# teaghan/sky_embeddings

Measured on AMD Instinct MI355X. Metric: MAE pretrain images/sec (5x64x64, ViT-B), higher is better.
Workload: dtype f16; 1 GPU; mim_32.ini-as-BASELINE configs[1]: MAE ViT-Base/16, 5x64x64, mask_ratio=0.75, bs=256/GPU, AdamW+cosine, norm_pix mse; global_batch=256, parallelism=dp1, rccl_ranks=1, graph=True, adamw_in_wgrad_epilogue=True

## Files before the change

### include/skyemb.h

```cpp
#ifndef SKYEMB_H
#define SKYEMB_H

#include <stdint.h>

#ifdef __cplusplus
extern "C" {
#endif

#define SKYEMB_BF16 0
#define SKYEMB_F32 1
#define SKYEMB_F16 2

#define SKYEMB_KC 0
#define SKYEMB_RC 1

#define SKYEMB_ACT_NONE 0
#define SKYEMB_ACT_GELU 1
#define SKYEMB_ACT_DGELU 2

const char *skyemb_last_error(void);
int skyemb_version(void);
int skyemb_debug_skip(int mask);
#define SKYEMB_GEMM_COUNT_FALLBACK 0
#define SKYEMB_GEMM_COUNT_PIPE 1
#define SKYEMB_GEMM_COUNT_256 2
#define SKYEMB_GEMM_COUNT_GROUP 3
#define SKYEMB_GEMM_COUNT_GROUP256 4
#define SKYEMB_GEMM_COUNT_SPLITK 5
#define SKYEMB_GEMM_COUNT_SLOTS 8
int skyemb_gemm_launch_counts(long long *out, int n, int reset);

typedef struct skyemb_gemm_args {
    const void *A;
    const void *B;
    int64_t lda, ldb;
    int32_t a_layout, b_layout;
    int32_t M, N, K;
    int32_t dtype;
    float alpha;
    const float *bias;
    const float *table;
    const int32_t *tab_row;
    int64_t ldt;
    const int32_t *dst_row;
    const float *resid;
    int64_t ldr;
    const void *aux;
    int64_t ldaux;
    int32_t act;
    float *out_f32;
    int64_t ldo32;
    void *out;
    int64_t ldo;
    void *out2;
    int64_t ldo2;
    int32_t tile;
    float *colsum_a;
    void *ws;
    int64_t ws_bytes;
    int32_t split_k;
    int32_t prefetch_wgs;
    const void *prefetch;
    int64_t prefetch_bytes;
} skyemb_gemm_args;

int skyemb_gemm(const skyemb_gemm_args *args, void *stream);

typedef struct skyemb_gemm_group_info {
    int32_t total_blocks;
    int32_t tile;
    int32_t class_mask;
    int32_t reserved;
} skyemb_gemm_group_info;
int64_t skyemb_gemm_group_blob_bytes(int n);
int skyemb_gemm_group_plan(const skyemb_gemm_args *args, int n, int tile, void *blob_host, int64_t blob_bytes,
                           skyemb_gemm_group_info *info);
int skyemb_gemm_group_launch(const void *blob_dev, const skyemb_gemm_group_info *info, void *stream);
typedef struct skyemb_adamw_desc {
    float *g_base, *p, *m, *v;
    void *p_lp;
    const float *hyper;
    int64_t n_decay;
    float beta1, beta2, eps, weight_decay, grad_scale;
    int32_t enabled;
} skyemb_adamw_desc;
int skyemb_gemm_group_plan_adamw(const skyemb_gemm_args *args, int n, int tile, const skyemb_adamw_desc *adamw, void *blob_host,
                                 int64_t blob_bytes, skyemb_gemm_group_info *info);
int skyemb_gemm_group_plan_side_adamw(const skyemb_gemm_args *args, int n, int tile, const skyemb_adamw_desc *adamw, int own_step,
                                      int64_t side_lo, int64_t side_hi, int side_blocks, void *blob_host, int64_t blob_bytes,
                                      skyemb_gemm_group_info *info);
typedef struct skyemb_ln_bwd_side {
    const void *dy;
    const float *x, *gamma, *mean, *rstd;
    const float *g_in;
    float *g_out;
    void *g_lp;
    float *part;
    int32_t M, D;
} skyemb_ln_bwd_side;
int skyemb_gemm_group_attach_ln_bwd(void *blob_host, int64_t blob_bytes, skyemb_gemm_group_info *info, const skyemb_ln_bwd_side *ln);

int skyemb_colsum(const void *X, int dtype, int64_t ldx, int M, int N, float *out, void *stream);

int skyemb_random_mask_from_noise(const float *noise, int B, int L, int keep, int64_t *ids_restore, float *mask,
                                  int32_t *ids_keep, int32_t *dec_dst, int32_t *dec_tab, int n_extra, void *stream);
int skyemb_simmim_mask_from_noise(const float *noise, const float *ratio_u, double max_ratio, int B, int C, int L, int grid, int p,
                                  float *out_mask, void *stream);

int skyemb_patch_gather(const float *imgs, const float *pmv, const int32_t *ids_keep, void *out, int dtype, int B,
                        int C, int H, int W, int p, int keep, float pixel_mean, float pixel_std, void *stream);

int skyemb_patch_gather_blend(const float *imgs, const float *pmv, const int32_t *ids_keep, const float *pixel_mask, void *out,
                              int dtype, int B, int C, int H, int W, int p, int keep, float pixel_mean, float pixel_std,
                              void *stream);
int skyemb_patch_gather_bwd_pmv_blend(const float *imgs, const int32_t *ids_keep, const float *pixel_mask, const float *drows,
                                      float *partial, float *dpmv, int B, int C, int H, int W, int p, int keep, void *stream);

int skyemb_radec_token_fwd(const float *ra_dec, const float *W0, const float *b0, const float *W1, const float *b1,
                           const float *pos_row, float *x, int64_t row_stride, int B, int D, float *sh, float *z, void *stream);
int skyemb_radec_token_bwd(const float *g, int64_t row_stride, const float *W1, const float *sh, const float *z, float *dz_ws,
                           float *dW0, float *db0, float *dW1, float *db1, int B, int D, void *stream);

int skyemb_patch_gather_bwd_pmv(const float *imgs, const int32_t *ids_keep, const float *drows, float *partial,
                                float *dpmv, int B, int C, int H, int W, int p, int keep, void *stream);

int skyemb_layernorm_fwd(const float *x, const float *gamma, const float *beta, void *y, float *y32, int dtype,
                         float *mean, float *rstd, int M, int D, float eps, void *stream);

int skyemb_layernorm_bwd_blocks(int M);
typedef struct {
    const float *part;
    float *dgamma, *dbeta;
    int32_t nblk, D;
} skyemb_ln_reduce_item;
int skyemb_layernorm_bwd_reduce_batch(const skyemb_ln_reduce_item *items, const int32_t *blocks, int n_blocks, void *stream);
int skyemb_layernorm_bwd(const void *dy, int dy_is_f32, int dtype, const float *x, const float *gamma,
                         const float *mean, const float *rstd, const float *g_in, float *g_out, void *g_lp,
                         float *part, float *dgamma, float *dbeta, int M, int D, void *stream);

#define SKYEMB_MHA_MAX_N 4098
int skyemb_mha_fwd(const void *qkv, void *out, int dtype, int B, int N, int H, int hd, void *stream);
int skyemb_mha_bwd(const void *qkv, const void *dout, void *dqkv, int dtype, int B, int N, int H, int hd,
                   void *stream);

int skyemb_fill_mask_tokens(float *x, const float *mask, const float *mask_token, const float *dec_pos, int B,
                            int L, int Dd, int n_extra, void *stream);
int skyemb_gather_rows(const float *src, const int32_t *idx, float *out, void *out_lp, int dtype, int n_rows,
                       int D, void *stream);
int skyemb_rowsum_select(const float *src, int64_t ld, const float *sel, int row0, int inner, int outer_stride,
                         int n_rows, int D, float *partial, float *out, void *stream);

int skyemb_masked_patch_loss(const float *imgs, const float *pred, const float *mask, float *loss, void *dpred,
                             float *dpred32, int dtype, float *ws, int B, int C, int H, int W, int p, int extra,
                             float pixel_mean, float pixel_std, int norm_pix, int loss_l1, float dscale, void *stream);

int skyemb_simmim_pixel_loss(const float *imgs, const float *pred_tok, const float *pixel_mask, float *loss, void *dpred_tok,
                             int dtype, float *pred_img, float *ws, int B, int C, int H, int W, int p, int extra,
                             float pixel_mean, float pixel_std, int norm_pix, int loss_l1, int pooled, float dscale, void *stream);

int skyemb_set_scalars(float *dst, float a, float b, float c, float d, void *stream);
int skyemb_adamw(float *p, void *g, float *m, float *v, void *p_lp, int dtype, int64_t n, int64_t n_decay,
                 const float *hyper, float lr, float bc1, float bc2, float beta1, float beta2, float eps, float wd,
                 float grad_scale, int zero_grad, int grad_dtype, void *stream);
int skyemb_cast(const float *src, void *dst, int dtype, int64_t n, void *stream);

int skyemb_gather_rows_host(const void *src, int64_t row_bytes, const int64_t *idx, int64_t n, int64_t src_rows, void *dst,
                            int nthreads);
int skyemb_h5_unchunk_host(const void *file_base, int64_t file_bytes, const int64_t *chunk_addr, const int64_t *chunk_off,
                           int64_t nchunks, int rank, const int64_t *chunk_dims, const int64_t *dset_dims, int elem_size, void *dst,
                           int nthreads);
int skyemb_fits_decode_tiles_host(int codec, const void *base, int64_t base_bytes, const int64_t *off, const int64_t *len,
                                  const int64_t *npix, const int64_t *dst_off, int64_t ntiles, int bytepix, int blocksize, void *dst,
                                  int64_t dst_pixels, int nthreads);
int skyemb_fits_dequantise_tiles_host(const int32_t *q, const int64_t *q_off, const int64_t *y0, const int64_t *x0, const int64_t *h,
                                      const int64_t *w, const int64_t *table_row, int64_t ntiles, const double *zscale, const double *zzero,
                                      const int32_t *blank, const uint8_t *has_blank, const float *rand, int method, int zdither0,
                                      float *out, int64_t H, int64_t W, int big_endian_out, int nthreads);
int skyemb_tile_cutouts(const void *tile, const int *big_endian, int C, int H, int W, const int *h0, const int *w0, int n, int S,
                        float lo, float hi, int use_lo, int use_hi, float *out, void *stream);
int skyemb_clip_crop(const float *src, float *dst, int64_t n_planes, int Hs, int Ws, int size, float lo, float hi,
                     int use_lo, int use_hi, void *stream);

int skyemb_augment(const float *imgs, float *out, const float *params, const int32_t *nan_mask, const float *noise, int B, int C,
                   int S, int A, void *stream);

int skyemb_standardise(const float *x, const float *mu, const float *sigma, float *out, int64_t N, int D,
                       void *stream);
int skyemb_weighted_norms(const float *x, const float *w, float *norms, float *xw_out, int64_t N, int D,
                          void *stream);
int skyemb_cosine_topk_chunks(int64_t N, int Q, int D, int k);
int skyemb_cosine_topk(const float *tw, const float *qn, const float *bank, const float *xn, int Q, int64_t N,
                       int D, int k, float eps, int64_t idx_offset, int nchunks, const float *thr0, float *part_s,
                       int64_t *part_i, void *stream);
int skyemb_kth_largest_floor(const float *x, int Q, int S, int k, float *out, void *stream);
int skyemb_cosine_sample_floor(const float *tw, const float *qn, const float *sample, const float *sample_norms, int Q, int64_t S,
                               int D, int k, float eps, float *ws, float *floor_out, void *stream);
int skyemb_cosine_sample_floor_applicable(int Q, int64_t S, int D, int k);
int skyemb_topk_merge(const float *in_s, const int64_t *in_i, int Q, int nlists, int k, float *out_s,
                      int64_t *out_i, void *ws, void *stream);

int skyemb_topk_prefilter_applicable(int Q, int64_t N, int D, int k);
int64_t skyemb_topk_prefilter_ws_bytes(int Q, int D, int k);
int64_t skyemb_bank16_bytes(int64_t N, int D);
int64_t skyemb_bank16_rowp_rows(int64_t N);
int skyemb_bank16_prepare(const float *bank, const float *xn, int64_t N, int D, void *bank16, float *rowp, void *stream);
int skyemb_cosine_topk_prefiltered(const float *tw, const float *qn, int Q, const float *bank, const float *xn, const void *bank16,
                                   const float *rowp, int64_t N, int D, int k, float eps, int64_t idx_offset, const float *thr0,
                                   void *ws, int64_t ws_bytes, float *out_s, int64_t *out_i, int *redo, void *stream);
int skyemb_attnpool_q(const float *latent, const float *Wq, const float *bq, float *q, int D, void *stream);
int skyemb_attnpool_fwd(const float *q, const void *kv, int dtype, void *out, float *prob, int B, int N, int H, int hd, void *stream);
int skyemb_attnpool_bwd(const float *q, const void *kv, int dtype, const void *dout, const float *prob, void *dkv, float *dq_part,
                        int B, int N, int H, int hd, void *stream);
int skyemb_attnpool_fwd_long(const float *q, const void *kv, int dtype, void *out, float *prob, int B, int N, int H, int hd,
                             void *stream);
int skyemb_attnpool_bwd_long(const float *q, const void *kv, int dtype, const void *dout, const float *prob, void *dkv,
                             float *dq_part, int B, int N, int H, int hd, void *stream);
int skyemb_attnpool_q_bwd(const float *dq_part, int B, const float *latent, const float *Wq, float *dWq, float *dbq, float *dlatent,
                          float *ws, int D, void *stream);
int skyemb_cosine_scores(const float *tw, const float *qn, const float *bank, const float *xn, int Q, int64_t N,
                         int D, float eps, float *scores, void *stream);
#define SKYEMB_COMBINE_MIN 0
#define SKYEMB_COMBINE_MEAN 1
#define SKYEMB_COMBINE_MAX 2
int skyemb_cosine_token_applicable(int Q, int P, int D, int k);
int skyemb_cosine_token_topk_chunks(int64_t N, int P, int Q, int D, int k);
int skyemb_cosine_token_scores(const float *tw, const float *qn, const float *bank, const float *xn, int Q, int64_t N, int P, int D,
                               int combine, float eps, float *scores, void *stream);
int skyemb_cosine_token_topk(const float *tw, const float *qn, const float *bank, const float *xn, int Q, int64_t N, int P, int D,
                             int k, int combine, float eps, int64_t idx_offset, int nlists, const float *thr0, float *part_s,
                             int64_t *part_i, void *stream);

#ifdef __cplusplus
}
#endif
#endif
```

### sky_embeddings_amd/_lib.py

```python
from __future__ import annotations

import ctypes
import os
import subprocess

import torch

_HERE = os.path.dirname(os.path.abspath(__file__))
SO_PATH = os.environ.get("SKYEMB_LIB") or os.path.join(_HERE, "libskyemb.so")
CSRC = os.path.join(_HERE, "csrc")

BF16, F32, F16 = 0, 1, 2
ABI_VERSION = 111
KC, RC = 0, 1
ACT_NONE, ACT_GELU, ACT_DGELU = 0, 1, 2
COMBINE_MIN, COMBINE_MEAN, COMBINE_MAX = 0, 1, 2


class SkyembLibraryError(RuntimeError):
    pass


class SkyembError(RuntimeError):
    pass


c_i32, c_i64, c_f32, c_vp = ctypes.c_int32, ctypes.c_int64, ctypes.c_float, ctypes.c_void_p


class GemmArgs(ctypes.Structure):
    _fields_ = [
        ("A", c_vp), ("B", c_vp), ("lda", c_i64), ("ldb", c_i64), ("a_layout", c_i32), ("b_layout", c_i32),
        ("M", c_i32), ("N", c_i32), ("K", c_i32), ("dtype", c_i32), ("alpha", c_f32),
        ("bias", c_vp), ("table", c_vp), ("tab_row", c_vp), ("ldt", c_i64), ("dst_row", c_vp),
        ("resid", c_vp), ("ldr", c_i64), ("aux", c_vp), ("ldaux", c_i64), ("act", c_i32),
        ("out_f32", c_vp), ("ldo32", c_i64), ("out", c_vp), ("ldo", c_i64), ("out2", c_vp), ("ldo2", c_i64),
        ("tile", c_i32), ("colsum_a", c_vp), ("ws", c_vp), ("ws_bytes", c_i64), ("split_k", c_i32), ("prefetch_wgs", c_i32),
        ("prefetch", c_vp), ("prefetch_bytes", c_i64),
    ]


class AdamwDesc(ctypes.Structure):
    _fields_ = [("g_base", c_vp), ("p", c_vp), ("m", c_vp), ("v", c_vp), ("p_lp", c_vp), ("hyper", c_vp), ("n_decay", c_i64),
                ("beta1", c_f32), ("beta2", c_f32), ("eps", c_f32), ("weight_decay", c_f32), ("grad_scale", c_f32), ("enabled", c_i32)]


class LnBwdSide(ctypes.Structure):
    _fields_ = [("dy", c_vp), ("x", c_vp), ("gamma", c_vp), ("mean", c_vp), ("rstd", c_vp), ("g_in", c_vp), ("g_out", c_vp), ("g_lp", c_vp),
                ("part", c_vp), ("M", c_i32), ("D", c_i32)]


class GemmGroupInfo(ctypes.Structure):
    _fields_ = [("total_blocks", c_i32), ("tile", c_i32), ("class_mask", c_i32), ("reserved", c_i32)]


PROTOTYPES = {
    "skyemb_last_error": (ctypes.c_char_p, []),
    "skyemb_version": (c_i32, []),
    "skyemb_debug_skip": (c_i32, [c_i32]),
    "skyemb_gemm_launch_counts": (c_i32, [c_vp, c_i32, c_i32]),
    "skyemb_gemm": (c_i32, [ctypes.POINTER(GemmArgs), c_vp]),
    "skyemb_gemm_group_blob_bytes": (c_i64, [c_i32]),
    "skyemb_gemm_group_plan": (c_i32, [ctypes.POINTER(GemmArgs), c_i32, c_i32, c_vp, c_i64, ctypes.POINTER(GemmGroupInfo)]),
    "skyemb_set_scalars": (c_i32, [c_vp, c_f32, c_f32, c_f32, c_f32, c_vp]),
    "skyemb_gemm_group_plan_adamw": (c_i32, [ctypes.POINTER(GemmArgs), c_i32, c_i32, ctypes.POINTER(AdamwDesc), c_vp, c_i64,
                                             ctypes.POINTER(GemmGroupInfo)]),
    "skyemb_gemm_group_plan_side_adamw": (c_i32, [ctypes.POINTER(GemmArgs), c_i32, c_i32, ctypes.POINTER(AdamwDesc), c_i32, c_i64, c_i64, c_i32,
                                                  c_vp, c_i64, ctypes.POINTER(GemmGroupInfo)]),
    "skyemb_gemm_group_attach_ln_bwd": (c_i32, [c_vp, c_i64, ctypes.POINTER(GemmGroupInfo), ctypes.POINTER(LnBwdSide)]),
    "skyemb_gemm_group_launch": (c_i32, [c_vp, ctypes.POINTER(GemmGroupInfo), c_vp]),
    "skyemb_colsum": (c_i32, [c_vp, c_i32, c_i64, c_i32, c_i32, c_vp, c_vp]),
    "skyemb_random_mask_from_noise": (c_i32, [c_vp, c_i32, c_i32, c_i32, c_vp, c_vp, c_vp, c_vp, c_vp, c_i32, c_vp]),
    "skyemb_simmim_mask_from_noise": (c_i32, [c_vp, c_vp, ctypes.c_double, c_i32, c_i32, c_i32, c_i32, c_i32, c_vp, c_vp]),
    "skyemb_patch_gather": (c_i32, [c_vp, c_vp, c_vp, c_vp, c_i32, c_i32, c_i32, c_i32, c_i32, c_i32, c_i32, c_f32,
                                    c_f32, c_vp]),
    "skyemb_patch_gather_bwd_pmv": (c_i32, [c_vp, c_vp, c_vp, c_vp, c_vp, c_i32, c_i32, c_i32, c_i32, c_i32, c_i32,
                                            c_vp]),
    "skyemb_layernorm_fwd": (c_i32, [c_vp, c_vp, c_vp, c_vp, c_vp, c_i32, c_vp, c_vp, c_i32, c_i32, c_f32, c_vp]),
    "skyemb_patch_gather_blend": (c_i32, [c_vp, c_vp, c_vp, c_vp, c_vp, c_i32, c_i32, c_i32, c_i32, c_i32, c_i32, c_i32, c_f32, c_f32, c_vp]),
    "skyemb_patch_gather_bwd_pmv_blend": (c_i32, [c_vp, c_vp, c_vp, c_vp, c_vp, c_vp, c_i32, c_i32, c_i32, c_i32, c_i32, c_i32, c_vp]),
    "skyemb_radec_token_fwd": (c_i32, [c_vp, c_vp, c_vp, c_vp, c_vp, c_vp, c_vp, c_i64, c_i32, c_i32, c_vp, c_vp, c_vp]),
    "skyemb_radec_token_bwd": (c_i32, [c_vp, c_i64, c_vp, c_vp, c_vp, c_vp, c_vp, c_vp, c_vp, c_vp, c_i32, c_i32, c_vp]),
    "skyemb_simmim_pixel_loss": (c_i32, [c_vp, c_vp, c_vp, c_vp, c_vp, c_i32, c_vp, c_vp, c_i32, c_i32, c_i32, c_i32, c_i32, c_i32,
                                         c_f32, c_f32, c_i32, c_i32, c_i32, c_f32, c_vp]),
    "skyemb_gather_rows_host": (c_i32, [c_vp, c_i64, c_vp, c_i64, c_i64, c_vp, c_i32]),
    "skyemb_h5_unchunk_host": (c_i32, [c_vp, c_i64, c_vp, c_vp, c_i64, c_i32, c_vp, c_vp, c_i32, c_vp, c_i32]),
    "skyemb_fits_decode_tiles_host": (c_i32, [c_i32, c_vp, c_i64, c_vp, c_vp, c_vp, c_vp, c_i64, c_i32, c_i32, c_vp, c_i64, c_i32]),
    "skyemb_fits_dequantise_tiles_host": (c_i32, [c_vp, c_vp, c_vp, c_vp, c_vp, c_vp, c_vp, c_i64, c_vp, c_vp, c_vp, c_vp, c_vp, c_i32, c_i32,
                                                  c_vp, c_i64, c_i64, c_i32, c_i32]),
    "skyemb_augment": (c_i32, [c_vp, c_vp, c_vp, c_vp, c_vp, c_i32, c_i32, c_i32, c_i32, c_vp]),
    "skyemb_attnpool_q": (c_i32, [c_vp, c_vp, c_vp, c_vp, c_i32, c_vp]),
    "skyemb_attnpool_fwd": (c_i32, [c_vp, c_vp, c_i32, c_vp, c_vp, c_i32, c_i32, c_i32, c_i32, c_vp]),
    "skyemb_attnpool_bwd": (c_i32, [c_vp, c_vp, c_i32, c_vp, c_vp, c_vp, c_vp, c_i32, c_i32, c_i32, c_i32, c_vp]),
    "skyemb_attnpool_fwd_long": (c_i32, [c_vp, c_vp, c_i32, c_vp, c_vp, c_i32, c_i32, c_i32, c_i32, c_vp]),
    "skyemb_attnpool_bwd_long": (c_i32, [c_vp, c_vp, c_i32, c_vp, c_vp, c_vp, c_vp, c_i32, c_i32, c_i32, c_i32, c_vp]),
    "skyemb_attnpool_q_bwd": (c_i32, [c_vp, c_i32, c_vp, c_vp, c_vp, c_vp, c_vp, c_vp, c_i32, c_vp]),
    "skyemb_tile_cutouts": (c_i32, [c_vp, c_vp, c_i32, c_i32, c_i32, c_vp, c_vp, c_i32, c_i32, c_f32, c_f32, c_i32, c_i32, c_vp, c_vp]),
    "skyemb_clip_crop": (c_i32, [c_vp, c_vp, c_i64, c_i32, c_i32, c_i32, c_f32, c_f32, c_i32, c_i32, c_vp]),
    "skyemb_layernorm_bwd_blocks": (c_i32, [c_i32]),
    "skyemb_layernorm_bwd_reduce_batch": (c_i32, [c_vp, c_vp, c_i32, c_vp]),
    "skyemb_layernorm_bwd": (c_i32, [c_vp, c_i32, c_i32, c_vp, c_vp, c_vp, c_vp, c_vp, c_vp, c_vp, c_vp, c_vp, c_vp,
                                     c_i32, c_i32, c_vp]),
    "skyemb_mha_fwd": (c_i32, [c_vp, c_vp, c_i32, c_i32, c_i32, c_i32, c_i32, c_vp]),
    "skyemb_mha_bwd": (c_i32, [c_vp, c_vp, c_vp, c_i32, c_i32, c_i32, c_i32, c_i32, c_vp]),
    "skyemb_fill_mask_tokens": (c_i32, [c_vp, c_vp, c_vp, c_vp, c_i32, c_i32, c_i32, c_i32, c_vp]),
    "skyemb_gather_rows": (c_i32, [c_vp, c_vp, c_vp, c_vp, c_i32, c_i32, c_i32, c_vp]),
    "skyemb_rowsum_select": (c_i32, [c_vp, c_i64, c_vp, c_i32, c_i32, c_i32, c_i32, c_i32, c_vp, c_vp, c_vp]),
    "skyemb_masked_patch_loss": (c_i32, [c_vp, c_vp, c_vp, c_vp, c_vp, c_vp, c_i32, c_vp, c_i32, c_i32, c_i32, c_i32,
                                         c_i32, c_i32, c_f32, c_f32, c_i32, c_i32, c_f32, c_vp]),
    "skyemb_adamw": (c_i32, [c_vp, c_vp, c_vp, c_vp, c_vp, c_i32, c_i64, c_i64, c_vp, c_f32, c_f32, c_f32, c_f32,
                             c_f32, c_f32, c_f32, c_f32, c_i32, c_i32, c_vp]),
    "skyemb_cast": (c_i32, [c_vp, c_vp, c_i32, c_i64, c_vp]),
    "skyemb_standardise": (c_i32, [c_vp, c_vp, c_vp, c_vp, c_i64, c_i32, c_vp]),
    "skyemb_weighted_norms": (c_i32, [c_vp, c_vp, c_vp, c_vp, c_i64, c_i32, c_vp]),
    "skyemb_cosine_topk_chunks": (c_i32, [c_i64, c_i32, c_i32, c_i32]),
    "skyemb_cosine_topk": (c_i32, [c_vp, c_vp, c_vp, c_vp, c_i32, c_i64, c_i32, c_i32, c_f32, c_i64, c_i32, c_vp, c_vp,
                                   c_vp, c_vp]),
    "skyemb_kth_largest_floor": (c_i32, [c_vp, c_i32, c_i32, c_i32, c_vp, c_vp]),
    "skyemb_cosine_sample_floor": (c_i32, [c_vp, c_vp, c_vp, c_vp, c_i32, c_i64, c_i32, c_i32, c_f32, c_vp, c_vp, c_vp]),
    "skyemb_cosine_sample_floor_applicable": (c_i32, [c_i32, c_i64, c_i32, c_i32]),
    "skyemb_topk_merge": (c_i32, [c_vp, c_vp, c_i32, c_i32, c_i32, c_vp, c_vp, c_vp, c_vp]),
    "skyemb_topk_prefilter_applicable": (c_i32, [c_i32, c_i64, c_i32, c_i32]),
    "skyemb_topk_prefilter_ws_bytes": (c_i64, [c_i32, c_i32, c_i32]),
    "skyemb_bank16_bytes": (c_i64, [c_i64, c_i32]),
    "skyemb_bank16_rowp_rows": (c_i64, [c_i64]),
    "skyemb_bank16_prepare": (c_i32, [c_vp, c_vp, c_i64, c_i32, c_vp, c_vp, c_vp]),
    "skyemb_cosine_topk_prefiltered": (c_i32, [c_vp, c_vp, c_i32, c_vp, c_vp, c_vp, c_vp, c_i64, c_i32, c_i32, c_f32, c_i64, c_vp,
                                               c_vp, c_i64, c_vp, c_vp, c_vp, c_vp]),
    "skyemb_cosine_scores": (c_i32, [c_vp, c_vp, c_vp, c_vp, c_i32, c_i64, c_i32, c_f32, c_vp, c_vp]),
    "skyemb_cosine_token_applicable": (c_i32, [c_i32, c_i32, c_i32, c_i32]),
    "skyemb_cosine_token_topk_chunks": (c_i32, [c_i64, c_i32, c_i32, c_i32, c_i32]),
    "skyemb_cosine_token_scores": (c_i32, [c_vp, c_vp, c_vp, c_vp, c_i32, c_i64, c_i32, c_i32, c_i32, c_f32, c_vp, c_vp]),
    "skyemb_cosine_token_topk": (c_i32, [c_vp, c_vp, c_vp, c_vp, c_i32, c_i64, c_i32, c_i32, c_i32, c_i32, c_f32, c_i64, c_i32, c_vp,
                                         c_vp, c_vp, c_vp]),
}

_LIB = None


def build(force: bool = False) -> str:
    if force:
        subprocess.check_call(["make", "-C", CSRC, "-s", "clean"])
    subprocess.check_call(["make", "-C", CSRC, "-s", "-j8"])
    return SO_PATH


def lib():
    global _LIB
    if _LIB is None:
        if not os.path.exists(SO_PATH):
            raise SkyembLibraryError(
                f"{SO_PATH} is missing: the HIP hot-path library has not been built "
                "(run `python -c 'import __graft_entry__ as g; g.build()'` or `make -C sky_embeddings_amd/csrc`). "
                "There is no CPU fallback.")
        try:
            L = ctypes.CDLL(SO_PATH)
        except OSError as e:
            raise SkyembLibraryError(f"cannot load {SO_PATH}: {e}") from e
        for name, (res, args) in PROTOTYPES.items():
            try:
                fn = getattr(L, name)
            except AttributeError as e:
                raise SkyembLibraryError(f"{SO_PATH} does not export {name}") from e
            fn.restype, fn.argtypes = res, args
        if L.skyemb_version() != ABI_VERSION:
            raise SkyembLibraryError(f"{SO_PATH} reports ABI version {L.skyemb_version()}, this binding is written against "
                                     f"{ABI_VERSION}: rebuild the library (make -C sky_embeddings_amd/csrc)")
        _LIB = L
    return _LIB


def check(rc: int, what: str = ""):
    if rc != 0:
        msg = lib().skyemb_last_error()
        raise SkyembError(f"{what} failed (rc={rc}): {msg.decode() if msg else ''}")
```

### sky_embeddings_amd/csrc/adamw.hip

```cpp
#include "common.h"
#include "adamw_math.h"

namespace {

template <typename T, bool LP, typename GT>
__global__ __launch_bounds__(256) void adamw_kernel(float *__restrict__ p, GT *__restrict__ g, float *__restrict__ m,
                                                    float *__restrict__ v, T *__restrict__ p_lp, int64_t n4,
                                                    int64_t n_decay, const float *__restrict__ hyper, float lr_arg,
                                                    float bc1_arg, float bc2_arg, float beta1, float beta2, float eps,
                                                    float wd, float grad_scale, int zero_grad) {
    const float lr = hyper ? hyper[0] : lr_arg, bc1 = hyper ? hyper[1] : bc1_arg, bc2 = hyper ? hyper[2] : bc2_arg;
    const SkyAdamScalars sc = sky_adam_scalars(lr, bc1, bc2, beta1, beta2, eps, wd, grad_scale);
    const int64_t stride = (int64_t)gridDim.x * 256;
    for (int64_t i0 = (int64_t)blockIdx.x * 256 + threadIdx.x; i0 < n4; i0 += 2 * stride) {
        f32x4 pv[2], gv[2], mv[2], vv[2];
#pragma unroll
        for (int u = 0; u < 2; ++u) {
            const int64_t i = i0 + u * stride;
            if (i < n4) {
                pv[u] = *(const f32x4 *)(p + 4 * i);
                const float4 gl = load4<GT>(g + 4 * i);
                gv[u] = (f32x4){gl.x, gl.y, gl.z, gl.w};
                mv[u] = *(const f32x4 *)(m + 4 * i);
                vv[u] = *(const f32x4 *)(v + 4 * i);
            }
        }
#pragma unroll
        for (int u = 0; u < 2; ++u) {
            const int64_t i = i0 + u * stride;
            if (i >= n4) break;
#pragma unroll
            for (int j = 0; j < 4; ++j) {
                float pj = pv[u][j], mj = mv[u][j], vj = vv[u][j];
                sky_adamw_update(gv[u][j], pj, mj, vj, 4 * i + j < n_decay, sc);
                pv[u][j] = pj; mv[u][j] = mj; vv[u][j] = vj;
            }
            *(f32x4 *)(p + 4 * i) = pv[u];
            *(f32x4 *)(m + 4 * i) = mv[u];
            *(f32x4 *)(v + 4 * i) = vv[u];
            if (LP) store4<T>(p_lp + 4 * i, pv[u][0], pv[u][1], pv[u][2], pv[u][3]);
            if (zero_grad) store4<GT>(g + 4 * i, 0.f, 0.f, 0.f, 0.f);
        }
    }
}

__global__ void set_scalars_kernel(float *dst, float a, float b, float c, float d) {
    if (threadIdx.x == 0) { dst[0] = a; dst[1] = b; dst[2] = c; dst[3] = d; }
}

}

extern "C" int skyemb_set_scalars(float *dst, float a, float b, float c, float d, void *stream) {
    SKY_CHECK_ARG(dst != nullptr, "skyemb_set_scalars: null destination");
    hipLaunchKernelGGL(set_scalars_kernel, dim3(1), dim3(64), 0, (hipStream_t)stream, dst, a, b, c, d);
    SKY_LAUNCH_CHECK("skyemb_set_scalars");
    return 0;
}

extern "C" int skyemb_adamw(float *p, void *g, float *m, float *v, void *p_lp, int dtype, int64_t n, int64_t n_decay,
                            const float *hyper, float lr, float bc1, float bc2, float beta1, float beta2, float eps,
                            float wd, float grad_scale, int zero_grad, int grad_dtype, void *stream) {
    SKY_CHECK_ARG(n > 0 && n % 4 == 0 && n_decay >= 0 && n_decay <= n, "skyemb_adamw: n must be a positive multiple of 4");
    SKY_CHECK_ARG(aligned16(p) && aligned16(m) && aligned16(v) && (((uintptr_t)g) & 7) == 0, "skyemb_adamw: unaligned buffers");
    SKY_CHECK_ARG(grad_dtype == SKYEMB_F32 || sky_is_lp(grad_dtype), "skyemb_adamw: bad grad_dtype %d", grad_dtype);
    SKY_CHECK_ARG(!sky_is_lp(grad_dtype) || !p_lp || grad_dtype == dtype || dtype == SKYEMB_F32,
                  "skyemb_adamw: a 16-bit gradient buffer and a 16-bit shadow must share their format");
    int64_t blocks = ceil_div64(n / 4, 256);
    if (blocks > 256 * 16) blocks = 256 * 16;
    hipStream_t st = (hipStream_t)stream;
    dim3 grid((unsigned)blocks), block(256);
#define ADAMW_LAUNCH(T, LP, GT, lp_ptr)                                                                                        \
    hipLaunchKernelGGL((adamw_kernel<T, LP, GT>), grid, block, 0, st, p, (GT *)g, m, v, lp_ptr, n / 4, n_decay, hyper, lr, bc1, \
                       bc2, beta1, beta2, eps, wd, grad_scale, zero_grad)
    const bool g16 = grad_dtype == SKYEMB_BF16, gh = grad_dtype == SKYEMB_F16;
    if (!p_lp) {
        if (g16) ADAMW_LAUNCH(float, false, bf16_t, (float *)nullptr);
        else if (gh) ADAMW_LAUNCH(float, false, f16_t, (float *)nullptr);
        else ADAMW_LAUNCH(float, false, float, (float *)nullptr);
    } else if (dtype == SKYEMB_BF16) {
        if (g16) ADAMW_LAUNCH(bf16_t, true, bf16_t, (bf16_t *)p_lp);
        else ADAMW_LAUNCH(bf16_t, true, float, (bf16_t *)p_lp);
    } else if (dtype == SKYEMB_F16) {
        if (gh) ADAMW_LAUNCH(f16_t, true, f16_t, (f16_t *)p_lp);
        else ADAMW_LAUNCH(f16_t, true, float, (f16_t *)p_lp);
    } else {
        if (g16) ADAMW_LAUNCH(float, true, bf16_t, (float *)p_lp);
        else if (gh) ADAMW_LAUNCH(float, true, f16_t, (float *)p_lp);
        else ADAMW_LAUNCH(float, true, float, (float *)p_lp);
    }
#undef ADAMW_LAUNCH
    SKY_LAUNCH_CHECK("skyemb_adamw");
    return 0;
}
```

### sky_embeddings_amd/csrc/frontend.hip

```cpp
#include "common.h"
#include <type_traits>

namespace {

__global__ __launch_bounds__(256) void mask_kernel(const float *__restrict__ noise, int B, int L, int keep,
                                                   int64_t *__restrict__ ids_restore, float *__restrict__ mask,
                                                   int32_t *__restrict__ ids_keep, int32_t *__restrict__ dec_dst,
                                                   int32_t *__restrict__ dec_tab, int E) {
    extern __shared__ float sn[];
    const int lane = threadIdx.x & 63, wave = threadIdx.x >> 6;
    const int b = blockIdx.x * 4 + wave;
    if (b >= B) return;
    float *row = sn + wave * L;
    for (int i = lane; i < L; i += 64) row[i] = noise[(int64_t)b * L + i];
    __builtin_amdgcn_wave_barrier();
    for (int i = lane; i < L; i += 64) {
        const float v = row[i];
        int rank = 0;
        for (int j = 0; j < L; ++j) {
            const float u = row[j];
            rank += (u < v || (u == v && j < i)) ? 1 : 0;
        }
        ids_restore[(int64_t)b * L + i] = rank;
        mask[(int64_t)b * L + i] = rank >= keep ? 1.0f : 0.0f;
        if (rank < keep) {
            ids_keep[(int64_t)b * keep + rank] = i;
            if (dec_dst) {
                dec_dst[(int64_t)b * (keep + E) + E + rank] = b * (L + E) + E + i;
                dec_tab[(int64_t)b * (keep + E) + E + rank] = E + i;
            }
        }
    }
    if (dec_dst && lane < E) {
        dec_dst[(int64_t)b * (keep + E) + lane] = b * (L + E) + lane;
        dec_tab[(int64_t)b * (keep + E) + lane] = lane;
    }
}


__global__ __launch_bounds__(256) void simmim_mask_kernel(const float *__restrict__ noise, const float *__restrict__ ratio_u,
                                                          double max_ratio, int BC, int C, int L, int grid, int p,
                                                          float *__restrict__ out) {
    extern __shared__ float sn[];
    const int lane = threadIdx.x & 63, wave = threadIdx.x >> 6;
    const int bc = blockIdx.x * 4 + wave;
    if (bc >= BC) return;
    float *row = sn + wave * 2 * L, *mk = row + L;
    for (int i = lane; i < L; i += 64) row[i] = noise[(int64_t)bc * L + i];
    __builtin_amdgcn_wave_barrier();
    const int b = bc / C;
    const int count = (int)ceilf((float)((double)L * ((double)ratio_u[b] * max_ratio)));
    for (int i = lane; i < L; i += 64) {
        const float v = row[i];
        int rank = 0;
        for (int j = 0; j < L; ++j) {
            const float u = row[j];
            rank += (u < v || (u == v && j < i)) ? 1 : 0;
        }
        mk[i] = rank < count ? 1.0f : 0.0f;
    }
    __builtin_amdgcn_wave_barrier();
    const int H = grid * p;
    float *o = out + (int64_t)bc * H * H;
    for (int e = lane * 4; e < H * H; e += 256) {
        const int y = e / H, x = e - y * H;
        const float m = mk[(y / p) * grid + x / p];
        *(float4 *)(o + e) = make_float4(m, m, m, m);
    }
}

template <typename T>
__global__ __launch_bounds__(256) void patch_gather_kernel(const float *__restrict__ imgs, const float *__restrict__ pmv,
                                                           const int32_t *__restrict__ ids_keep, T *__restrict__ out,
                                                           int C, int H, int W, int p, int keep, float mean, float stdv,
                                                           const float *__restrict__ pmask) {
    const int row = blockIdx.x;
    const int b = row / keep;
    const int l = ids_keep ? ids_keep[row] : (row - b * keep);
    const int gw = W / p;
    const int y0 = (l / gw) * p, x0 = (l % gw) * p;
    const int pv4 = C * p * p / 4, p4 = p / 4;
    for (int e = threadIdx.x; e < pv4; e += 256) {
        const int px4 = e % p4, py = (e / p4) % p, c = e / (p4 * p);
        const float4 x = *(const float4 *)(imgs + (((int64_t)b * C + c) * H + y0 + py) * W + x0 + 4 * px4);
        const float4 m = *(const float4 *)(pmv + (c * p + py) * p + 4 * px4);
        float4 o;
        o.x = x.x != x.x ? m.x : (x.x - mean) / stdv;
        o.y = x.y != x.y ? m.y : (x.y - mean) / stdv;
        o.z = x.z != x.z ? m.z : (x.z - mean) / stdv;
        o.w = x.w != x.w ? m.w : (x.w - mean) / stdv;
        if (pmask) {
            const float4 k = *(const float4 *)(pmask + (((int64_t)b * C + c) * H + y0 + py) * W + x0 + 4 * px4);
            o.x = o.x * (1.0f - k.x) + m.x * k.x;
            o.y = o.y * (1.0f - k.y) + m.y * k.y;
            o.z = o.z * (1.0f - k.z) + m.z * k.z;
            o.w = o.w * (1.0f - k.w) + m.w * k.w;
        }
        if constexpr (std::is_same<T, f16_t>::value) {
            o.x = fminf(fmaxf(o.x, -65504.f), 65504.f);
            o.y = fminf(fmaxf(o.y, -65504.f), 65504.f);
            o.z = fminf(fmaxf(o.z, -65504.f), 65504.f);
            o.w = fminf(fmaxf(o.w, -65504.f), 65504.f);
        }
        store4<T>(out + (int64_t)row * (C * p * p) + 4 * e, o.x, o.y, o.z, o.w);
    }
}

__global__ __launch_bounds__(256) void pmv_partial_kernel(const float *__restrict__ imgs, const int32_t *__restrict__ ids_keep,
                                                          const float *__restrict__ drows, float *__restrict__ partial,
                                                          int C, int H, int W, int p, int keep, const float *__restrict__ pmask) {
    const int b = blockIdx.x;
    const int gw = W / p, pv = C * p * p;
    const int e = blockIdx.y * 256 + threadIdx.x;
    if (e >= pv) return;
    const int px = e % p, py = (e / p) % p, c = e / (p * p);
    float acc = 0.f;
    for (int j0 = 0; j0 < keep; j0 += 4) {
        float wgt[4], d[4];
#pragma unroll
        for (int u = 0; u < 4; ++u) {
            const int j = j0 + u < keep ? j0 + u : keep - 1;
            const int l = ids_keep ? ids_keep[b * keep + j] : j;
            const int y = (l / gw) * p + py, x = (l % gw) * p + px;
            const int64_t pix = (((int64_t)b * C + c) * H + y) * W + x;
            const float v = imgs[pix];
            wgt[u] = j0 + u >= keep ? 0.0f : v != v ? 1.0f : (pmask ? pmask[pix] : 0.0f);
            d[u] = drows[((int64_t)b * keep + j) * pv + e];
        }
#pragma unroll
        for (int u = 0; u < 4; ++u)
            if (wgt[u] != 0.0f) acc += wgt[u] * d[u];
    }
    partial[(int64_t)b * pv + e] = acc;
}

template <typename T>
__global__ __launch_bounds__(256) void colsum_kernel(const T *__restrict__ X, int64_t ldx, int M, int N,
                                                     float *__restrict__ out) {
    __shared__ float red[4][64];
    const int lane = threadIdx.x & 63, wave = threadIdx.x >> 6;
    const int n = blockIdx.x * 64 + lane;
    float acc = 0.f;
    if (n < N) {
#pragma unroll 8
        for (int m = wave; m < M; m += 4) acc += to_f32<T>(X[(int64_t)m * ldx + n]);
    }
    red[wave][lane] = acc;
    __syncthreads();
    if (wave == 0 && n < N) out[n] = (red[0][lane] + red[1][lane]) + (red[2][lane] + red[3][lane]);
}

__global__ __launch_bounds__(256) void fill_mask_tokens_kernel(float *__restrict__ x, const float *__restrict__ mask,
                                                               const float *__restrict__ mask_token,
                                                               const float *__restrict__ dec_pos, int L, int Dd, int E) {
    const int b = blockIdx.x / L, l = blockIdx.x % L;
    if (mask[(int64_t)b * L + l] == 0.0f) return;
    float *dst = x + ((int64_t)b * (L + E) + E + l) * Dd;
    const float *pos = dec_pos + (int64_t)(E + l) * Dd;
    for (int d = threadIdx.x * 4; d < Dd; d += 1024) {
        const float4 t = *(const float4 *)(mask_token + d), q = *(const float4 *)(pos + d);
        *(float4 *)(dst + d) = make_float4(t.x + q.x, t.y + q.y, t.z + q.z, t.w + q.w);
    }
}

template <typename T>
__global__ __launch_bounds__(256) void gather_rows_kernel(const float *__restrict__ src, const int32_t *__restrict__ idx,
                                                          float *__restrict__ out, T *__restrict__ out_lp, int D) {
    const int r = blockIdx.x;
    const float *s = src + (int64_t)idx[r] * D;
    for (int d = threadIdx.x * 4; d < D; d += 1024) {
        const float4 v = *(const float4 *)(s + d);
        if (out) *(float4 *)(out + (int64_t)r * D + d) = v;
        if (out_lp) store4<T>(out_lp + (int64_t)r * D + d, v.x, v.y, v.z, v.w);
    }
}

__global__ __launch_bounds__(256) void rowsum_select_kernel(const float *__restrict__ src, int64_t ld,
                                                            const float *__restrict__ sel, int row0, int inner,
                                                            int outer_stride, int n_rows, int D,
                                                            float *__restrict__ partial) {
    const int nblk = gridDim.x;
    for (int d = threadIdx.x; d < D; d += 256) {
        float acc = 0.f;
        for (int i0 = blockIdx.x; i0 < n_rows; i0 += 4 * nblk) {
            float x[4];
#pragma unroll
            for (int u = 0; u < 4; ++u) {
                const int i = i0 + u * nblk;
                const bool take = i < n_rows && !(sel && sel[i] == 0.0f);
                const int ii = take ? i : 0;
                const int64_t r = (int64_t)row0 + (int64_t)(ii / inner) * outer_stride + (ii % inner);
                x[u] = take ? src[r * ld + d] : 0.f;
            }
#pragma unroll
            for (int u = 0; u < 4; ++u)
                if (i0 + u * nblk < n_rows && !(sel && sel[i0 + u * nblk] == 0.0f)) acc += x[u];
        }
        partial[(int64_t)blockIdx.x * D + d] = acc;
    }
}

template <typename T>
__global__ __launch_bounds__(256) void cast_kernel(const float *__restrict__ src, T *__restrict__ dst, int64_t n4) {
    for (int64_t i = (int64_t)blockIdx.x * 256 + threadIdx.x; i < n4; i += (int64_t)gridDim.x * 256) {
        const float4 v = *(const float4 *)(src + 4 * i);
        store4<T>(dst + 4 * i, v.x, v.y, v.z, v.w);
    }
}

__global__ __launch_bounds__(256) void clip_crop_kernel(const float *__restrict__ src, float *__restrict__ dst, int64_t n_out,
                                                        int Hs, int Ws, int size, int top, int left, float lo, float hi,
                                                        int use_lo, int use_hi) {
    for (int64_t i = (int64_t)blockIdx.x * 256 + threadIdx.x; i < n_out; i += (int64_t)gridDim.x * 256) {
        const int x = (int)(i % size);
        const int64_t t = i / size;
        const int y = (int)(t % size);
        const int64_t plane = t / size;
        float v = src[(plane * Hs + top + y) * Ws + left + x];
        if (use_lo && v < lo) v = lo;
        if (use_hi && v > hi) v = hi;
        dst[i] = v;
    }
}

__global__ __launch_bounds__(256) void tile_cutouts_kernel(const unsigned int *__restrict__ tile, const int *__restrict__ be, int C,
                                                           int H, int W, const int *__restrict__ h0, const int *__restrict__ w0,
                                                           int64_t n_out, int S, float lo, float hi, int use_lo, int use_hi,
                                                           float *__restrict__ out) {
    for (int64_t i = (int64_t)blockIdx.x * 256 + threadIdx.x; i < n_out; i += (int64_t)gridDim.x * 256) {
        const int x = (int)(i % S);
        int64_t t = i / S;
        const int y = (int)(t % S);
        t /= S;
        const int c = (int)(t % C);
        const int64_t k = t / C;
        unsigned int u = tile[((int64_t)c * H + h0[k] + y) * W + w0[k] + x];
        if (be[c]) u = __builtin_bswap32(u);
        float v = __uint_as_float(u);
        if (use_lo && v < lo) v = lo;
        if (use_hi && v > hi) v = hi;
        out[i] = v;
    }
}

}

extern "C" int skyemb_clip_crop(const float *src, float *dst, int64_t n_planes, int Hs, int Ws, int size, float lo, float hi,
                                int use_lo, int use_hi, void *stream) {
    SKY_CHECK_ARG(src && dst && n_planes > 0 && size > 0 && Hs >= size && Ws >= size, "skyemb_clip_crop: bad shape");
    const int64_t n_out = n_planes * size * size;
    int64_t blocks = ceil_div64(n_out, 256);
    if (blocks > 8192) blocks = 8192;
    hipLaunchKernelGGL(clip_crop_kernel, dim3((unsigned)blocks), dim3(256), 0, (hipStream_t)stream, src, dst, n_out, Hs, Ws, size,
                       (Hs - size) / 2, (Ws - size) / 2, lo, hi, use_lo, use_hi);
    SKY_LAUNCH_CHECK("skyemb_clip_crop");
    return 0;
}

extern "C" int skyemb_tile_cutouts(const void *tile, const int *big_endian, int C, int H, int W, const int *h0, const int *w0, int n,
                                   int S, float lo, float hi, int use_lo, int use_hi, float *out, void *stream) {
    SKY_CHECK_ARG(tile && big_endian && h0 && w0 && out && C > 0 && n > 0 && S > 0 && H >= S && W >= S,
                  "skyemb_tile_cutouts: bad shape C=%d H=%d W=%d n=%d S=%d", C, H, W, n, S);
    const int64_t n_out = (int64_t)n * C * S * S;
    int64_t blocks = ceil_div64(n_out, 256);
    if (blocks > 16384) blocks = 16384;
    hipLaunchKernelGGL(tile_cutouts_kernel, dim3((unsigned)blocks), dim3(256), 0, (hipStream_t)stream, (const unsigned int *)tile,
                       big_endian, C, H, W, h0, w0, n_out, S, lo, hi, use_lo, use_hi, out);
    SKY_LAUNCH_CHECK("skyemb_tile_cutouts");
    return 0;
}

extern "C" int skyemb_random_mask_from_noise(const float *noise, int B, int L, int keep, int64_t *ids_restore,
                                             float *mask, int32_t *ids_keep, int32_t *dec_dst, int32_t *dec_tab,
                                             int n_extra, void *stream) {
    SKY_CHECK_ARG(B > 0 && L > 0 && keep >= 0 && keep <= L && L <= 4096 && n_extra >= 1 && n_extra <= 2,
                  "skyemb_random_mask_from_noise: bad shape B=%d L=%d keep=%d extra=%d", B, L, keep, n_extra);
    hipLaunchKernelGGL(mask_kernel, dim3((B + 3) / 4), dim3(256), (size_t)4 * L * sizeof(float), (hipStream_t)stream, noise,
                       B, L, keep, ids_restore, mask, ids_keep, dec_dst, dec_tab, n_extra);
    SKY_LAUNCH_CHECK("skyemb_random_mask_from_noise");
    return 0;
}


extern "C" int skyemb_simmim_mask_from_noise(const float *noise, const float *ratio_u, double max_ratio, int B, int C, int L, int grid,
                                             int p, float *out_mask, void *stream) {
    SKY_CHECK_ARG(noise && ratio_u && out_mask && B > 0 && C > 0 && L == grid * grid && L <= 4096 && p > 0 && p % 4 == 0 &&
                  max_ratio >= 0.0 && max_ratio <= 1.0, "skyemb_simmim_mask_from_noise: bad arguments (L=%d grid=%d p=%d)", L, grid, p);
    hipLaunchKernelGGL(simmim_mask_kernel, dim3((B * C + 3) / 4), dim3(256), (size_t)8 * L * sizeof(float), (hipStream_t)stream, noise,
                       ratio_u, max_ratio, B * C, C, L, grid, p, out_mask);
    SKY_LAUNCH_CHECK("skyemb_simmim_mask_from_noise");
    return 0;
}

static int patch_gather_launch(const float *imgs, const float *pmv, const int32_t *ids_keep, const float *pixel_mask, void *out,
                               int dtype, int B, int C, int H, int W, int p, int keep, float pixel_mean, float pixel_std,
                               void *stream) {
    SKY_CHECK_ARG(B > 0 && C > 0 && p > 0 && p % 4 == 0 && H % p == 0 && W % p == 0 && keep > 0,
                  "skyemb_patch_gather: bad geometry C=%d H=%d W=%d p=%d keep=%d", C, H, W, p, keep);
    SKY_CHECK_ARG(ids_keep || keep == (H / p) * (W / p), "skyemb_patch_gather: ids_keep == NULL needs keep == L");
    hipStream_t st = (hipStream_t)stream;
    if (dtype == SKYEMB_BF16)
        hipLaunchKernelGGL(patch_gather_kernel<bf16_t>, dim3(B * keep), dim3(256), 0, st, imgs, pmv, ids_keep, (bf16_t *)out,
                           C, H, W, p, keep, pixel_mean, pixel_std, pixel_mask);
    else if (dtype == SKYEMB_F16)
        hipLaunchKernelGGL(patch_gather_kernel<f16_t>, dim3(B * keep), dim3(256), 0, st, imgs, pmv, ids_keep, (f16_t *)out,
                           C, H, W, p, keep, pixel_mean, pixel_std, pixel_mask);
    else
        hipLaunchKernelGGL(patch_gather_kernel<float>, dim3(B * keep), dim3(256), 0, st, imgs, pmv, ids_keep, (float *)out, C,
                           H, W, p, keep, pixel_mean, pixel_std, pixel_mask);
    SKY_LAUNCH_CHECK("skyemb_patch_gather");
    return 0;
}

extern "C" int skyemb_patch_gather(const float *imgs, const float *pmv, const int32_t *ids_keep, void *out, int dtype,
                                   int B, int C, int H, int W, int p, int keep, float pixel_mean, float pixel_std,
                                   void *stream) {
    return patch_gather_launch(imgs, pmv, ids_keep, nullptr, out, dtype, B, C, H, W, p, keep, pixel_mean, pixel_std, stream);
}

extern "C" int skyemb_patch_gather_blend(const float *imgs, const float *pmv, const int32_t *ids_keep, const float *pixel_mask,
                                         void *out, int dtype, int B, int C, int H, int W, int p, int keep, float pixel_mean,
                                         float pixel_std, void *stream) {
    return patch_gather_launch(imgs, pmv, ids_keep, pixel_mask, out, dtype, B, C, H, W, p, keep, pixel_mean, pixel_std, stream);
}

extern "C" int skyemb_colsum(const void *X, int dtype, int64_t ldx, int M, int N, float *out, void *stream) {
    SKY_CHECK_ARG(M > 0 && N > 0, "skyemb_colsum: bad shape");
    hipStream_t st = (hipStream_t)stream;
    if (dtype == SKYEMB_BF16)
        hipLaunchKernelGGL(colsum_kernel<bf16_t>, dim3((N + 63) / 64), dim3(256), 0, st, (const bf16_t *)X, ldx, M, N, out);
    else if (dtype == SKYEMB_F16)
        hipLaunchKernelGGL(colsum_kernel<f16_t>, dim3((N + 63) / 64), dim3(256), 0, st, (const f16_t *)X, ldx, M, N, out);
    else
        hipLaunchKernelGGL(colsum_kernel<float>, dim3((N + 63) / 64), dim3(256), 0, st, (const float *)X, ldx, M, N, out);
    SKY_LAUNCH_CHECK("skyemb_colsum");
    return 0;
}

extern "C" int skyemb_patch_gather_bwd_pmv_blend(const float *imgs, const int32_t *ids_keep, const float *pixel_mask,
                                                 const float *drows, float *partial, float *dpmv, int B, int C, int H, int W,
                                                 int p, int keep, void *stream) {
    SKY_CHECK_ARG(B > 0 && C > 0 && p > 0 && keep > 0, "skyemb_patch_gather_bwd_pmv: bad geometry");
    hipLaunchKernelGGL(pmv_partial_kernel, dim3(B, (C * p * p + 255) / 256), dim3(256), 0, (hipStream_t)stream, imgs, ids_keep, drows, partial, C, H,
                       W, p, keep, pixel_mask);
    SKY_LAUNCH_CHECK("skyemb_patch_gather_bwd_pmv");
    return skyemb_colsum(partial, SKYEMB_F32, (int64_t)C * p * p, B, C * p * p, dpmv, stream);
}

extern "C" int skyemb_patch_gather_bwd_pmv(const float *imgs, const int32_t *ids_keep, const float *drows, float *partial,
                                           float *dpmv, int B, int C, int H, int W, int p, int keep, void *stream) {
    return skyemb_patch_gather_bwd_pmv_blend(imgs, ids_keep, nullptr, drows, partial, dpmv, B, C, H, W, p, keep, stream);
}

extern "C" int skyemb_fill_mask_tokens(float *x, const float *mask, const float *mask_token, const float *dec_pos, int B,
                                       int L, int Dd, int n_extra, void *stream) {
    SKY_CHECK_ARG(B > 0 && L > 0 && Dd % 4 == 0 && n_extra >= 1, "skyemb_fill_mask_tokens: bad shape");
    hipLaunchKernelGGL(fill_mask_tokens_kernel, dim3(B * L), dim3(256), 0, (hipStream_t)stream, x, mask, mask_token, dec_pos,
                       L, Dd, n_extra);
    SKY_LAUNCH_CHECK("skyemb_fill_mask_tokens");
    return 0;
}

extern "C" int skyemb_gather_rows(const float *src, const int32_t *idx, float *out, void *out_lp, int dtype, int n_rows,
                                  int D, void *stream) {
    SKY_CHECK_ARG(n_rows > 0 && D % 4 == 0, "skyemb_gather_rows: bad shape");
    hipStream_t st = (hipStream_t)stream;
    if (dtype == SKYEMB_BF16)
        hipLaunchKernelGGL(gather_rows_kernel<bf16_t>, dim3(n_rows), dim3(256), 0, st, src, idx, out, (bf16_t *)out_lp, D);
    else if (dtype == SKYEMB_F16)
        hipLaunchKernelGGL(gather_rows_kernel<f16_t>, dim3(n_rows), dim3(256), 0, st, src, idx, out, (f16_t *)out_lp, D);
    else
        hipLaunchKernelGGL(gather_rows_kernel<float>, dim3(n_rows), dim3(256), 0, st, src, idx, out, (float *)out_lp, D);
    SKY_LAUNCH_CHECK("skyemb_gather_rows");
    return 0;
}

extern "C" int skyemb_rowsum_select(const float *src, int64_t ld, const float *sel, int row0, int inner, int outer_stride,
                                    int n_rows, int D, float *partial, float *out, void *stream) {
    SKY_CHECK_ARG(n_rows > 0 && D > 0 && inner > 0, "skyemb_rowsum_select: bad shape");
    const int nblk = 256;
    hipLaunchKernelGGL(rowsum_select_kernel, dim3(nblk), dim3(256), 0, (hipStream_t)stream, src, ld, sel, row0, inner,
                       outer_stride, n_rows, D, partial);
    SKY_LAUNCH_CHECK("skyemb_rowsum_select");
    return skyemb_colsum(partial, SKYEMB_F32, D, nblk, D, out, stream);
}

extern "C" int skyemb_cast(const float *src, void *dst, int dtype, int64_t n, void *stream) {
    SKY_CHECK_ARG(n > 0 && n % 4 == 0, "skyemb_cast: n must be a positive multiple of 4");
    int64_t blocks = ceil_div64(n / 4, 256);
    if (blocks > 4096) blocks = 4096;
    hipStream_t st = (hipStream_t)stream;
    if (dtype == SKYEMB_BF16)
        hipLaunchKernelGGL(cast_kernel<bf16_t>, dim3((unsigned)blocks), dim3(256), 0, st, src, (bf16_t *)dst, n / 4);
    else if (dtype == SKYEMB_F16)
        hipLaunchKernelGGL(cast_kernel<f16_t>, dim3((unsigned)blocks), dim3(256), 0, st, src, (f16_t *)dst, n / 4);
    else
        hipLaunchKernelGGL(cast_kernel<float>, dim3((unsigned)blocks), dim3(256), 0, st, src, (float *)dst, n / 4);
    SKY_LAUNCH_CHECK("skyemb_cast");
    return 0;
}
```

### sky_embeddings_amd/csrc/layernorm.hip

```cpp
#include "common.h"
#include "ln_bwd_body.h"

namespace {

constexpr int MAXV = 8;

template <typename T, int NV>
__global__ __launch_bounds__(256) void ln_fwd_kernel(const float *__restrict__ x, const float *__restrict__ gamma,
                                                     const float *__restrict__ beta, T *__restrict__ y,
                                                     float *__restrict__ y32, float *__restrict__ mean_o,
                                                     float *__restrict__ rstd_o, int M, int D, float eps) {
    const int lane = threadIdx.x & 63;
    const int row = blockIdx.x * 4 + (threadIdx.x >> 6);
    if (row >= M) return;
    const int nv = D >> 2;
    const float *xr = x + (int64_t)row * D;
    float4 v[NV], gm[NV], bt[NV];
#pragma unroll
    for (int i = 0; i < NV; ++i) {
        const int c = lane + i * 64, cc = c < nv ? c : nv - 1;
        v[i] = *(const float4 *)(xr + 4 * cc);
        gm[i] = *(const float4 *)(gamma + 4 * cc);
        bt[i] = *(const float4 *)(beta + 4 * cc);
    }
    float s = 0.f;
#pragma unroll
    for (int i = 0; i < NV; ++i)
        if (lane + i * 64 < nv) s += (v[i].x + v[i].y) + (v[i].z + v[i].w);
    const float mean = wave_sum(s) / (float)D;
    float q = 0.f;
#pragma unroll
    for (int i = 0; i < NV; ++i) {
        if (lane + i * 64 < nv) {
            const float a = v[i].x - mean, b = v[i].y - mean, cc = v[i].z - mean, d = v[i].w - mean;
            q += (a * a + b * b) + (cc * cc + d * d);
        }
    }
    const float rstd = rsqrtf(wave_sum(q) / (float)D + eps);
    if (lane == 0) {
        mean_o[row] = mean;
        rstd_o[row] = rstd;
    }
#pragma unroll
    for (int i = 0; i < NV; ++i) {
        const int c = lane + i * 64;
        if (c < nv) {
            const float4 g = gm[i], b = bt[i];
            const float o0 = (v[i].x - mean) * rstd * g.x + b.x, o1 = (v[i].y - mean) * rstd * g.y + b.y;
            const float o2 = (v[i].z - mean) * rstd * g.z + b.z, o3 = (v[i].w - mean) * rstd * g.w + b.w;
            if (y) store4<T>(y + (int64_t)row * D + 4 * c, o0, o1, o2, o3);
            if (y32) *(float4 *)(y32 + (int64_t)row * D + 4 * c) = make_float4(o0, o1, o2, o3);
        }
    }
}

template <typename TD, typename T, int NV>
__global__ __launch_bounds__(256) void ln_bwd_kernel(const TD *__restrict__ dy, const float *__restrict__ x,
                                                     const float *__restrict__ gamma, const float *__restrict__ mean,
                                                     const float *__restrict__ rstd, const float *g_in, float *g_out,
                                                     T *__restrict__ g_lp, float *__restrict__ part, int M, int D,
                                                     int nblk) {
    __shared__ float red[4 * 256];
    sky_ln_bwd_rows<TD, T, NV>(dy, x, gamma, mean, rstd, g_in, g_out, g_lp, part, M, D, nblk, (int)blockIdx.x, (int)(threadIdx.x >> 6),
                               (int)(threadIdx.x & 63), red);
}

__global__ __launch_bounds__(1024) void ln_bwd_reduce_kernel(const float *__restrict__ part, float *__restrict__ dgamma,
                                                             float *__restrict__ dbeta, int nblk, int D) {
    __shared__ float red[32][33];
    const int col = threadIdx.x & 31, rg = threadIdx.x >> 5;
    const int d = blockIdx.x * 32 + col;
    const float *src = part + (int64_t)blockIdx.y * nblk * D;
    float acc = 0.f;
    if (d < D)
#pragma unroll 8
        for (int b = rg; b < nblk; b += 32) acc += src[(int64_t)b * D + d];
    red[rg][col] = acc;
    __syncthreads();
    if (rg == 0 && d < D) {
        float t = 0.f;
#pragma unroll
        for (int r = 0; r < 32; ++r) t += red[r][col];
        (blockIdx.y == 0 ? dgamma : dbeta)[d] = t;
    }
}

__global__ __launch_bounds__(1024) void ln_bwd_reduce_batch_kernel(const skyemb_ln_reduce_item *__restrict__ items,
                                                                   const int2 *__restrict__ blocks) {
    __shared__ float red[32][33];
    const int2 blk = blocks[blockIdx.x];
    const skyemb_ln_reduce_item it = items[blk.x];
    const int bx = blk.y & 0xffff, by = blk.y >> 16;
    const int col = threadIdx.x & 31, rg = threadIdx.x >> 5;
    const int d = bx * 32 + col;
    const float *src = it.part + (int64_t)by * it.nblk * it.D;
    float acc = 0.f;
    if (d < it.D) {
#pragma unroll 8
        for (int b = rg; b < it.nblk; b += 32) acc += src[(int64_t)b * it.D + d];
    }
    red[rg][col] = acc;
    __syncthreads();
    if (rg == 0 && d < it.D) {
        float t = 0.f;
#pragma unroll
        for (int r = 0; r < 32; ++r) t += red[r][col];
        (by == 0 ? it.dgamma : it.dbeta)[d] = t;
    }
}

}

extern "C" int skyemb_layernorm_bwd_reduce_batch(const skyemb_ln_reduce_item *items, const int32_t *blocks, int n_blocks, void *stream) {
    SKY_CHECK_ARG(items && blocks && n_blocks > 0, "skyemb_layernorm_bwd_reduce_batch: bad arguments");
    hipLaunchKernelGGL(ln_bwd_reduce_batch_kernel, dim3((unsigned)n_blocks), dim3(1024), 0, (hipStream_t)stream, items, (const int2 *)blocks);
    SKY_LAUNCH_CHECK("skyemb_layernorm_bwd_reduce_batch");
    return 0;
}

extern "C" int skyemb_layernorm_fwd(const float *x, const float *gamma, const float *beta, void *y, float *y32,
                                    int dtype, float *mean, float *rstd, int M, int D, float eps, void *stream) {
    SKY_CHECK_ARG(M > 0 && D > 0 && D % 4 == 0 && D <= MAXV * 256, "skyemb_layernorm_fwd: bad shape M=%d D=%d", M, D);
    SKY_CHECK_ARG(aligned16(x) && aligned16(gamma) && aligned16(beta), "skyemb_layernorm_fwd: unaligned input");
    hipStream_t st = (hipStream_t)stream;
    dim3 grid((M + 3) / 4), block(256);
#define LN_FWD(NV)                                                                                                   \
    if (dtype == SKYEMB_BF16)                                                                                        \
        hipLaunchKernelGGL((ln_fwd_kernel<bf16_t, NV>), grid, block, 0, st, x, gamma, beta, (bf16_t *)y, y32, mean,   \
                           rstd, M, D, eps);                                                                         \
    else if (dtype == SKYEMB_F16)                                                                                    \
        hipLaunchKernelGGL((ln_fwd_kernel<f16_t, NV>), grid, block, 0, st, x, gamma, beta, (f16_t *)y, y32, mean,     \
                           rstd, M, D, eps);                                                                         \
    else                                                                                                             \
        hipLaunchKernelGGL((ln_fwd_kernel<float, NV>), grid, block, 0, st, x, gamma, beta, (float *)y, y32, mean,     \
                           rstd, M, D, eps);
    switch ((D + 255) / 256) {
        case 1: LN_FWD(1) break;
        case 2: LN_FWD(2) break;
        case 3: LN_FWD(3) break;
        case 4: LN_FWD(4) break;
        case 5: LN_FWD(5) break;
        case 6: LN_FWD(6) break;
        case 7: LN_FWD(7) break;
        default: LN_FWD(8) break;
    }
#undef LN_FWD
    SKY_LAUNCH_CHECK("skyemb_layernorm_fwd");
    return 0;
}

extern "C" int skyemb_layernorm_bwd_blocks(int M) {
    int nb = (M + 3) / 4;
    if (nb < 1) nb = 1;
    const int rounds = (nb + SKY_LN_BWD_CAP - 1) / SKY_LN_BWD_CAP;
    return (nb + rounds - 1) / rounds;
}

extern "C" int skyemb_layernorm_bwd(const void *dy, int dy_is_f32, int dtype, const float *x, const float *gamma,
                                    const float *mean, const float *rstd, const float *g_in, float *g_out, void *g_lp,
                                    float *part, float *dgamma, float *dbeta, int M, int D, void *stream) {
    SKY_CHECK_ARG(M > 0 && D > 0 && D % 4 == 0 && D <= MAXV * 256, "skyemb_layernorm_bwd: bad shape M=%d D=%d", M, D);
    hipStream_t st = (hipStream_t)stream;
    const int nblk = skyemb_layernorm_bwd_blocks(M);
    dim3 grid(nblk), block(256);
#define LN_BWD(NV)                                                                                                   \
    if (dtype == SKYEMB_BF16) {                                                                                      \
        if (dy_is_f32)                                                                                               \
            hipLaunchKernelGGL((ln_bwd_kernel<float, bf16_t, NV>), grid, block, 0, st, (const float *)dy, x, gamma,   \
                               mean, rstd, g_in, g_out, (bf16_t *)g_lp, part, M, D, nblk);                           \
        else                                                                                                         \
            hipLaunchKernelGGL((ln_bwd_kernel<bf16_t, bf16_t, NV>), grid, block, 0, st, (const bf16_t *)dy, x, gamma, \
                               mean, rstd, g_in, g_out, (bf16_t *)g_lp, part, M, D, nblk);                           \
    } else if (dtype == SKYEMB_F16) {                                                                                \
        if (dy_is_f32)                                                                                               \
            hipLaunchKernelGGL((ln_bwd_kernel<float, f16_t, NV>), grid, block, 0, st, (const float *)dy, x, gamma,    \
                               mean, rstd, g_in, g_out, (f16_t *)g_lp, part, M, D, nblk);                            \
        else                                                                                                         \
            hipLaunchKernelGGL((ln_bwd_kernel<f16_t, f16_t, NV>), grid, block, 0, st, (const f16_t *)dy, x, gamma,    \
                               mean, rstd, g_in, g_out, (f16_t *)g_lp, part, M, D, nblk);                            \
    } else {                                                                                                         \
        hipLaunchKernelGGL((ln_bwd_kernel<float, float, NV>), grid, block, 0, st, (const float *)dy, x, gamma, mean,  \
                           rstd, g_in, g_out, (float *)g_lp, part, M, D, nblk);                                      \
    }
    switch ((D + 255) / 256) {
        case 1: LN_BWD(1) break;
        case 2: LN_BWD(2) break;
        case 3: LN_BWD(3) break;
        case 4: LN_BWD(4) break;
        case 5: LN_BWD(5) break;
        case 6: LN_BWD(6) break;
        case 7: LN_BWD(7) break;
        default: LN_BWD(8) break;
    }
#undef LN_BWD
    if (dgamma && dbeta)
        hipLaunchKernelGGL(ln_bwd_reduce_kernel, dim3((D + 31) / 32, 2), dim3(1024), 0, st, part, dgamma, dbeta, nblk, D);
    SKY_LAUNCH_CHECK("skyemb_layernorm_bwd");
    return 0;
}
```

### sky_embeddings_amd/engine.py

```python
from __future__ import annotations

import math
import os
from collections import OrderedDict
from contextlib import contextmanager

import numpy as np
import torch

from . import ops
from ._lib import ACT_DGELU, ACT_GELU, BF16, F32, KC, RC, AdamwDesc
from .model_config import (FROZEN, SH_FEATURES, SIREN_HIDDEN, MAEConfig, not_optimised, sincos_pos_embed, state_layout,
                           weight_decay_split, xavier_bound)


def _pad8(n):
    return (n + 7) // 8 * 8


def merge_spans(spans):
    out = []
    for lo, hi in sorted(spans):
        if out and out[-1][1] == lo:
            out[-1] = (out[-1][0], hi)
        else:
            out.append((lo, hi))
    return out


def subtract_spans(spans, holes):
    out = []
    for s, e in spans:
        cur = s
        for hs, he in holes:
            if he <= cur or hs >= e:
                continue
            if hs > cur:
                out.append((cur, hs))
            cur = max(cur, he)
        if cur < e:
            out.append((cur, e))
    return out


WGRAD_SLOTS_PER_CU = {256256: 1, 128128: 2, 9128128: 1, 128064: 2, 64064: 3}
SIDE_CARRIER_MAX_FILL = 0.76
ADAMW_SIDE_MODES = ("auto", "0", "1", "dec", "enc")
WGRAD_GROUPS_KEY = {"plain": "wgrad_groups", "adamw": "wgrad_groups_adamw", "g16": "wgrad_groups_g16"}


def plan_wgrad_schedule(prefixes, tiles, ncu, mode):
    assert mode in ADAMW_SIDE_MODES, mode
    carry = [False] * len(prefixes)
    for k in range(1, len(prefixes)):
        tile, count = tiles[k]
        slots = ncu * WGRAD_SLOTS_PER_CU.get(tile, 1)
        carry[k] = (mode == "1" or (mode == "auto" and count <= SIDE_CARRIER_MAX_FILL * slots) or
                    (mode == "dec" and prefixes[k].startswith("decoder_blocks")) or (mode == "enc" and prefixes[k].startswith("blocks")))
    return [(carry[k], k + 1 < len(carry) and carry[k + 1]) for k in range(len(carry))]


class ParamStore:

    def __init__(self, cfg: MAEConfig, device, lp_dtype):
        self.cfg = cfg
        shapes = dict(state_layout(cfg))
        decay, no_decay = weight_decay_split(cfg)
        self.decay, self.no_decay = decay, no_decay
        self.order = decay + no_decay
        self.offsets = {}
        off = 0
        for name in decay:
            self.offsets[name] = off
            off += _pad8(int(np.prod(shapes[name])))
        self.n_decay = off
        for name in no_decay:
            self.offsets[name] = off
            off += _pad8(int(np.prod(shapes[name])))
        self.n = off
        self.shapes = shapes
        self.p = torch.zeros(self.n, device=device, dtype=torch.float32)
        self.g = torch.zeros(self.n, device=device, dtype=torch.float32)
        self.m = torch.zeros(self.n, device=device, dtype=torch.float32)
        self.v = torch.zeros(self.n, device=device, dtype=torch.float32)
        self.p_lp = torch.zeros(self.n, device=device, dtype=lp_dtype)
        self.frozen = {k: torch.zeros(shapes[k], device=device, dtype=torch.float32) for k in not_optimised(cfg) if k in shapes}

    def _view(self, buf, name):
        o = self.offsets[name]
        return buf[o:o + int(np.prod(self.shapes[name]))].view(self.shapes[name])

    def span(self, name):
        o = self.offsets[name]
        return o, o + _pad8(int(np.prod(self.shapes[name])))

    def param(self, name):
        return self.frozen[name] if name in self.frozen else self._view(self.p, name)

    def grad(self, name):
        return self._view(self.g, name)

    def lp(self, name):
        return self._view(self.p_lp, name)

    def refresh_lp(self):
        ops.cast(self.p, self.p_lp, self.n)


def stage_gradient_ranges(store: ParamStore, cfg: MAEConfig, n_encoder_groups: int = 3):
    off = store.offsets
    dec0 = store.span("decoder_embed.weight")[1]
    ranges = [[(dec0, store.n_decay)]]
    bounds = sorted({round(cfg.depth * k / n_encoder_groups) for k in range(n_encoder_groups + 1)}, reverse=True)
    groups = []
    for hi, lo in zip(bounds[:-1], bounds[1:]):
        groups.append((hi, lo))
        end = dec0 if hi == cfg.depth else off[f"blocks.{hi}.attn.qkv.weight"]
        ranges.append([(off[f"blocks.{lo}.attn.qkv.weight"], end)])
    ranges.append([(0, off["blocks.0.attn.qkv.weight"]), (store.n_decay, store.n)])
    return groups, ranges


class MAEEngine:
    _modes = "mae"

    def __init__(self, cfg: MAEConfig, device="cuda", compute_dtype=torch.bfloat16, seed=None):
        if cfg.attn_pool and not cfg.simmim:
            raise ValueError("attn_pool exists in SimMIM mode only (utils/mim_vit.py:244-254, :282)")
        if cfg.simmim and self._modes == "mae":
            raise NotImplementedError("simmim=True is served by sky_embeddings_amd.simmim_engine.SimMIMEngine")
        assert cfg.embed_dim % cfg.num_heads == 0 and cfg.decoder_embed_dim % cfg.decoder_num_heads == 0
        assert cfg.embed_dim % 8 == 0 and cfg.decoder_embed_dim % 8 == 0 and cfg.patch_size % 4 == 0
        self.cfg = cfg
        self.device = torch.device(device)
        self.dtype = compute_dtype
        self.code = ops.dtype_code(compute_dtype)
        env = os.environ.get("SKYEMB_LOSS_SCALE")
        self._loss_scale_auto = compute_dtype == torch.float16 and env is None
        self._loss_scale = float(env) if (env is not None and compute_dtype == torch.float16) else (65536.0 if compute_dtype == torch.float16 else 1.0)
        assert self._loss_scale > 0 and math.log2(self._loss_scale).is_integer(), "loss_scale must be a power of two"
        self.fold_decoder_wgrads = True
        self.store = ParamStore(cfg, self.device, compute_dtype)
        self._ws = {}
        self._last = None
        self.splitk_ws = torch.zeros(8 * 1024 * 1024, device=self.device, dtype=torch.float32)
        self._side, self._pending, self._group_done = None, {}, None
        self._splitk_ws_side = None
        self._ln_first = self._ln_count = 0
        self._pf_maps = None
        self._graph_captures = 0
        self._variant_args = {"adamw": None, "g16": None}
        self._variant = "plain"
        self._adamw_side, self._adamw_side_blocks = "0", 0
        self.initialize_weights(seed)

    def initialize_weights(self, seed=None):
        cfg, st = self.cfg, self.store
        gen = torch.Generator().manual_seed(seed if seed is not None else int(torch.initial_seed() % (2 ** 31)))
        for name in st.order:
            shape = st.shapes[name]
            if name in ("cls_token", "mask_token"):
                t = torch.randn(shape, generator=gen) * 0.02
            elif name == "attn_pool.latent":
                sd_ = shape[-1] ** -0.5
                t = (torch.randn(shape, generator=gen) * sd_).clamp_(-2 * sd_, 2 * sd_)
            elif name == "patch_mask_values":
                t = torch.zeros(shape)
            elif name == "patch_embed.proj.bias" or name.startswith("decoder.0."):
                b = 1.0 / math.sqrt(cfg.patch_dim if name.startswith("patch_embed") else cfg.embed_dim)
                t = (torch.rand(shape, generator=gen) * 2 - 1) * b
            elif name.startswith("ra_dec_embed."):
                first = ".layers.0." in name
                w_std = (1.0 / SH_FEATURES) if first else math.sqrt(6.0 / SIREN_HIDDEN)
                t = (torch.rand(shape, generator=gen) * 2 - 1) * w_std
            elif name.endswith("norm1.weight") or name.endswith("norm2.weight") or name.endswith("norm.weight"):
                t = torch.ones(shape)
            elif name.endswith(".bias"):
                t = torch.zeros(shape)
            else:
                t = (torch.rand(shape, generator=gen) * 2 - 1) * xavier_bound(shape)
            st.param(name).copy_(t)
        for k in st.frozen:
            if k in FROZEN:
                tab = sincos_pos_embed(st.shapes[k][-1], cfg.grid, True, cfg.ra_dec)
                st.frozen[k].copy_(torch.from_numpy(tab).float().unsqueeze(0))
            else:
                st.frozen[k].copy_(torch.randn(st.shapes[k], generator=gen) * 0.02)
        st.refresh_lp()

    @property
    def loss_scale(self):
        return self._loss_scale

    @loss_scale.setter
    def loss_scale(self, v):
        assert v > 0 and math.log2(v).is_integer(), "loss_scale must be a power of two"
        self._loss_scale, self._loss_scale_auto = float(v), False

    def plan_loss_scale(self, masked_elements):
        if self._loss_scale_auto:
            e = round(math.log2(max(float(masked_elements), 64.0) / 64.0))
            self._loss_scale = float(2 ** min(max(e, 0), 16))
        return self._loss_scale

    def expected_masked_elements(self, B, mask_ratio):
        cfg = self.cfg
        return B * (cfg.num_patches - int(cfg.num_patches * (1 - mask_ratio))) * cfg.patch_dim

    def grad(self, name):
        g = self.store.grad(name)
        return g if self.loss_scale == 1.0 else g / self.loss_scale

    def state_dict(self):
        out = OrderedDict()
        for name, _ in state_layout(self.cfg):
            out[name] = self.store.param(name)
        return out

    def load_state_dict(self, sd, strict=True):
        names = [n for n, _ in state_layout(self.cfg)]
        missing = [n for n in names if n not in sd]
        unexpected = [k for k in sd if k not in names]
        if strict and (missing or unexpected):
            raise RuntimeError(f"load_state_dict: missing {missing[:5]} unexpected {unexpected[:5]}")
        for n in names:
            if n in sd:
                self.store.param(n).copy_(torch.as_tensor(sd[n]).to(torch.float32).reshape(self.store.shapes[n]))
        self.store.refresh_lp()

    def _workspace(self, B, keep, train):
        key = (B, keep, train)
        if key in self._ws:
            return self._ws[key]
        cfg, dev, T = self.cfg, self.device, self.dtype
        L, D, Dd, pv, E = cfg.num_patches, cfg.embed_dim, cfg.decoder_embed_dim, cfg.patch_dim, cfg.num_extra_tokens
        Ne, Nd = E + keep, E + L
        Me, Md = B * Ne, B * Nd
        f32 = dict(device=dev, dtype=torch.float32)
        lp = dict(device=dev, dtype=T)
        i32 = dict(device=dev, dtype=torch.int32)
        w = {}
        w["sh"], w["z"], w["dz"] = torch.empty(B, 25, **f32), torch.empty(B, 8, **f32), torch.empty(B, 8, **f32)
        w["ids_restore"] = torch.empty(B, L, device=dev, dtype=torch.int64)
        w["mask"] = torch.empty(B, L, **f32)
        w["ids_keep"] = torch.empty(B, keep, **i32)
        w["dec_dst"] = torch.empty(B, Ne, **i32)
        w["dec_tab"] = torch.empty(B, Ne, **i32)
        w["pe_dst"] = (torch.arange(B, device=dev)[:, None] * Ne + E + torch.arange(keep, device=dev)[None, :]).to(torch.int32).contiguous()
        w["patches"] = torch.empty(B * keep, pv, **lp)
        w["latent32"] = torch.empty(Me, D, **f32)
        n_enc_sets = cfg.depth if train else 1
        w["enc"] = [self._block_bufs(Me, D) for _ in range(n_enc_sets)]
        w["xs"] = [torch.empty(Me, D, **f32) for _ in range((cfg.depth + 1) if train else 2)]
        w["lat_lp"] = torch.empty(Me, D, **lp)
        w["lat_mean"], w["lat_rstd"] = torch.empty(Me, **f32), torch.empty(Me, **f32)
        if train:
            w["dec"] = [self._block_bufs(Md, Dd) for _ in range(cfg.decoder_depth)]
            w["xd"] = [torch.empty(Md, Dd, **f32) for _ in range(cfg.decoder_depth + 1)]
            w["dlat_lp"] = torch.empty(Md, Dd, **lp)
            w["dlat_mean"], w["dlat_rstd"] = torch.empty(Md, **f32), torch.empty(Md, **f32)
            w["pred"] = torch.empty(B, Nd, pv, **f32)
            w["loss"] = torch.zeros(1, **f32)
            w["loss_ws"] = torch.empty(4 * B * L + 4, **f32)
            w["dpred"] = torch.empty(Md, pv, **lp)
            self._bwd_scratch(w, max(Me, Md) * max(D, Dd), max(Me * int(D * cfg.mlp_ratio), Md * int(Dd * cfg.mlp_ratio)))
            order = [("ln", "decoder_norm", Md, Dd)]
            for i in reversed(range(cfg.decoder_depth)):
                order.append(("block", f"decoder_blocks.{i}", w["dec"][i], Md, Dd))
            order.append(("ln", "norm", Me, D))
            for i in reversed(range(cfg.depth)):
                order.append(("block", f"blocks.{i}", w["enc"][i], Me, D))
            self._build_reduce_table(w, order)
            w["dE"] = torch.empty(Me, Dd, **lp)
            self._build_wgrad_groups(w, (("blocks", w["enc"], Me, D), ("decoder_blocks", w["dec"], Md, Dd)))
            w["dT"] = torch.empty(B * keep, D, **lp)
            w["drows"] = torch.empty(B * keep, pv, **f32)
            w["pmv_part"] = torch.empty(B, pv, **f32)
            w["rs_part"] = torch.empty(256, max(D, Dd), **f32)
        self._ws[key] = w
        return w

    def _block_bufs(self, M, dim):
        f32, lp = dict(device=self.device, dtype=torch.float32), dict(device=self.device, dtype=self.dtype)
        hidden = int(dim * self.cfg.mlp_ratio)
        return dict(ln1=torch.empty(M, dim, **lp), mean1=torch.empty(M, **f32), rstd1=torch.empty(M, **f32),
                    qkv=torch.empty(M, 3 * dim, **lp), att=torch.empty(M, dim, **lp), xmid=torch.empty(M, dim, **f32),
                    ln2=torch.empty(M, dim, **lp), mean2=torch.empty(M, **f32), rstd2=torch.empty(M, **f32),
                    hpre=torch.empty(M, hidden, **lp), hact=torch.empty(M, hidden, **lp))

    def _bwd_scratch(self, w, n, n_hidden):
        f32, lp = dict(device=self.device, dtype=torch.float32), dict(device=self.device, dtype=self.dtype)
        w["g"] = torch.empty(n, **f32)
        w["g_lp"] = torch.empty(n, **lp)
        w["g_lp2"] = torch.empty(n, **lp)
        w["g_lp_b"], w["g_lp2_b"] = torch.empty(n, **lp), torch.empty(n, **lp)
        w["dh_b"], w["dqkv_b"] = torch.empty(n_hidden, **lp), torch.empty(3 * n, **lp)
        w["dln"] = torch.empty(n, **lp)
        w["datt"] = torch.empty(n, **lp)
        w["dh"] = torch.empty(n_hidden, **lp)
        w["dqkv"] = torch.empty(3 * n, **lp)

    def _build_wgrad_groups(self, w, stacks):
        w["splitk_ws"] = self.splitk_ws
        plain = w["wgrad_groups"] = {}
        if self.dtype in ops.LP_DTYPES:
            for tag, blocks, M, dim in stacks:
                for i, bufs in enumerate(blocks):
                    plain[f"{tag}.{i}"] = self._make_wgrad_group(f"{tag}.{i}", bufs, M, dim, w)
        for kind, arg in self._variant_args.items():
            if arg is not None and plain:
                self._build_variant_groups(w, kind)

    def _build_reduce_table(self, w, order):
        f32 = dict(device=self.device, dtype=torch.float32)
        entries = []
        w["ln_index"], w["ln_parts"] = {}, {}

        def ln(name, M_, D_):
            nb = ops.layernorm_bwd_blocks(M_)
            part = torch.empty(2, nb, D_, **f32)
            w["ln_index"][name] = len(entries)
            w["ln_parts"][name] = part
            entries.append((part, self.store.grad(f"{name}.weight"), self.store.grad(f"{name}.bias"), nb, D_))
        for item in order:
            if item[0] == "ln":
                ln(*item[1:])
                continue
            _, prefix, bufs, M_, dim = item
            ln(f"{prefix}.norm2", M_, dim)
            ln(f"{prefix}.norm1", M_, dim)
        w["ln_items"] = ops.ln_reduce_items(entries, self.device)

    def _weight_chain(self):
        cfg = self.cfg
        blk = lambda p: [f"{p}.attn.qkv.weight", f"{p}.attn.proj.weight", f"{p}.mlp.fc1.weight", f"{p}.mlp.fc2.weight"]
        names = ["patch_embed.proj.weight"]
        for i in range(cfg.depth):
            names += blk(f"blocks.{i}")
        names += self._decoder_weight_chain()
        return [n for n in names if n in self.store.offsets]

    def _decoder_weight_chain(self):
        cfg = self.cfg
        names = ["decoder_embed.weight"]
        for i in range(cfg.decoder_depth):
            names += [f"decoder_blocks.{i}.attn.qkv.weight", f"decoder_blocks.{i}.attn.proj.weight", f"decoder_blocks.{i}.mlp.fc1.weight",
                      f"decoder_blocks.{i}.mlp.fc2.weight"]
        return names + ["decoder_pred.weight"]

    PF_MAX_ROWS = 8192

    def _pf(self, direction, wname, rows=0):
        if rows >= int(os.environ.get("SKYEMB_PF_MAX_ROWS", self.PF_MAX_ROWS)):
            return None
        if self._pf_maps is None:
            chain = self._weight_chain()
            self._pf_maps = {"fwd": dict(zip(chain[:-1], chain[1:])), "bwd": dict(zip(chain[1:], chain[:-1]))}
        if self.dtype not in ops.LP_DTYPES:
            return None
        only = os.environ.get("SKYEMB_PF_ONLY", "")
        if only and only != direction:
            return None
        nxt = self._pf_maps[direction].get(wname)
        return None if nxt is None else self.store.lp(nxt)

    def _embed(self, imgs, noise, keep, w, ra_dec=None):
        cfg, st = self.cfg, self.store
        B = imgs.shape[0]
        L, D, pv, E = cfg.num_patches, cfg.embed_dim, cfg.patch_dim, cfg.num_extra_tokens
        Ne = E + keep
        ops.random_mask_from_noise(noise, keep, w["ids_restore"], w["mask"], w["ids_keep"], w["dec_dst"], w["dec_tab"], n_extra=E)
        ops.patch_gather(imgs, st.param("patch_mask_values"), w["ids_keep"], w["patches"], cfg.patch_size, keep,
                         cfg.pixel_mean, cfg.pixel_std)
        x0 = w["xs"][0]
        pos = st.frozen["pos_embed"].view(-1, D)
        ops.gemm(w["patches"], st.lp("patch_embed.proj.weight"), M=B * keep, N=D, K=pv,
                 bias=st.param("patch_embed.proj.bias"), table=pos[E:], tab_row=w["ids_keep"], ldt=D,
                 dst_row=w["pe_dst"], out_f32=x0, ldo32=D, prefetch=self._pf("fwd", "patch_embed.proj.weight", B * keep))
        self._extra_tokens_fwd(x0, pos, B, Ne, ra_dec, w)
        return x0

    def _extra_tokens_fwd(self, x0, pos, B, Ne, ra_dec, w):
        cfg, st = self.cfg, self.store
        D = cfg.embed_dim
        x0.view(B, Ne, D)[:, 0, :] = st.param("cls_token").view(D) + pos[0]
        if cfg.ra_dec:
            P = st.param
            ops.radec_token_fwd(ra_dec, P("ra_dec_embed.neural_network.layers.0.weight"),
                                P("ra_dec_embed.neural_network.layers.0.bias"), P("ra_dec_embed.neural_network.last_layer.weight"),
                                P("ra_dec_embed.neural_network.last_layer.bias"), pos[1], x0.view(-1)[D:], Ne * D, B, D,
                                w["sh"], w["z"])

    def _block_fwd(self, x_in, x_out, bufs, prefix, M, dim, heads, Bsz, N):
        st, eps = self.store, self.cfg.ln_eps
        hd = dim // heads
        hidden = bufs["hpre"].shape[1]
        P, LP = st.param, st.lp
        ops.layernorm_fwd(x_in, P(f"{prefix}.norm1.weight"), P(f"{prefix}.norm1.bias"), bufs["ln1"], bufs["mean1"],
                          bufs["rstd1"], M, dim, eps)
        PF = lambda name: self._pf("fwd", f"{prefix}.{name}.weight", M)
        ops.gemm(bufs["ln1"], LP(f"{prefix}.attn.qkv.weight"), M=M, N=3 * dim, K=dim, bias=P(f"{prefix}.attn.qkv.bias"),
                 out=bufs["qkv"], prefetch=PF("attn.qkv"))
        ops.mha_fwd(bufs["qkv"], bufs["att"], Bsz, N, heads, hd)
        ops.gemm(bufs["att"], LP(f"{prefix}.attn.proj.weight"), M=M, N=dim, K=dim, bias=P(f"{prefix}.attn.proj.bias"),
                 resid=x_in, ldr=dim, out_f32=bufs["xmid"], ws=self.splitk_ws, prefetch=PF("attn.proj"))
        ops.layernorm_fwd(bufs["xmid"], P(f"{prefix}.norm2.weight"), P(f"{prefix}.norm2.bias"), bufs["ln2"],
                          bufs["mean2"], bufs["rstd2"], M, dim, eps)
        ops.gemm(bufs["ln2"], LP(f"{prefix}.mlp.fc1.weight"), M=M, N=hidden, K=dim, bias=P(f"{prefix}.mlp.fc1.bias"),
                 act=ACT_GELU, out=bufs["hact"], out2=bufs["hpre"], prefetch=PF("mlp.fc1"))
        ops.gemm(bufs["hact"], LP(f"{prefix}.mlp.fc2.weight"), M=M, N=dim, K=hidden, bias=P(f"{prefix}.mlp.fc2.bias"),
                 resid=bufs["xmid"], ldr=dim, out_f32=x_out, ws=self.splitk_ws, prefetch=PF("mlp.fc2"))

    def _blocks_fwd(self, w, B, Ne, train):
        cfg, xs = self.cfg, w["xs"]
        M, D = B * Ne, cfg.embed_dim
        for i in range(cfg.depth):
            if train:
                self._block_fwd(xs[i], xs[i + 1], w["enc"][i], f"blocks.{i}", M, D, cfg.num_heads, B, Ne)
            else:
                self._block_fwd(xs[i % 2], xs[(i + 1) % 2], w["enc"][0], f"blocks.{i}", M, D, cfg.num_heads, B, Ne)
        return xs[cfg.depth] if train else xs[cfg.depth % 2]

    def _encoder_fwd(self, imgs, noise, keep, w, train, ra_dec=None):
        cfg, st = self.cfg, self.store
        B = imgs.shape[0]
        D, Ne = cfg.embed_dim, cfg.num_extra_tokens + keep
        Me = B * Ne
        self._embed(imgs, noise, keep, w, ra_dec)
        x_last = self._blocks_fwd(w, B, Ne, train)
        ops.layernorm_fwd(x_last, st.param("norm.weight"), st.param("norm.bias"), w["lat_lp"], w["lat_mean"],
                          w["lat_rstd"], Me, D, cfg.ln_eps, y32=w["latent32"])
        return x_last

    def check_ra_dec(self, imgs, ra_dec):
        if not self.cfg.ra_dec:
            return None
        assert ra_dec is not None and tuple(ra_dec.shape) == (imgs.shape[0], 2), "ra_dec=True models need ra_dec [B,2] (degrees)"
        return ra_dec.to(device=imgs.device, dtype=torch.float32).contiguous()

    def _check_cutouts(self, imgs):
        cfg = self.cfg
        assert imgs.is_cuda and imgs.dtype == torch.float32 and imgs.is_contiguous()
        B, C, H, W = imgs.shape
        assert (C, H, W) == (cfg.in_chans, cfg.img_size, cfg.img_size), f"bad cutout shape {tuple(imgs.shape)}"
        return B

    def _check_inputs(self, imgs, noise):
        cfg = self.cfg
        B = self._check_cutouts(imgs)
        if noise is None:
            noise = torch.rand(B, cfg.num_patches, device=imgs.device)
        assert noise.shape == (B, cfg.num_patches) and noise.is_cuda and noise.dtype == torch.float32
        return noise.contiguous()

    def forward_features(self, imgs, mask_ratio=0.0, noise=None, ra_dec=None):
        cfg = self.cfg
        noise = self._check_inputs(imgs, noise)
        ra_dec = self.check_ra_dec(imgs, ra_dec)
        B = imgs.shape[0]
        keep = int(cfg.num_patches * (1 - mask_ratio))
        w = self._workspace(B, keep, False)
        self._encoder_fwd(imgs, noise, keep, w, False, ra_dec)
        return w["latent32"].view(B, cfg.num_extra_tokens + keep, cfg.embed_dim), w["mask"], w["ids_restore"]

    def encoder_forward_train(self, imgs, noise, keep, ra_dec=None):
        w = self._workspace(imgs.shape[0], keep, True)
        self._encoder_fwd(imgs, noise, keep, w, True, ra_dec)
        self._last = (imgs, imgs.shape[0], keep)
        return w

    def forward_train(self, imgs, mask_ratio=0.75, noise=None, ra_dec=None):
        cfg, st = self.cfg, self.store
        noise = self._check_inputs(imgs, noise)
        ra_dec = self.check_ra_dec(imgs, ra_dec)
        B = imgs.shape[0]
        L, D, Dd, pv, E = cfg.num_patches, cfg.embed_dim, cfg.decoder_embed_dim, cfg.patch_dim, cfg.num_extra_tokens
        keep = int(L * (1 - mask_ratio))
        assert keep >= 1, "mask_ratio leaves no visible patch"
        Ne, Nd = E + keep, E + L
        Me, Md = B * Ne, B * Nd
        w = self._workspace(B, keep, True)
        self.plan_loss_scale(B * (L - keep) * pv)
        self._encoder_fwd(imgs, noise, keep, w, True, ra_dec)
        xd = w["xd"]
        dpos = st.frozen["decoder_pos_embed"].view(-1, Dd)
        ops.gemm(w["lat_lp"], st.lp("decoder_embed.weight"), M=Me, N=Dd, K=D, bias=st.param("decoder_embed.bias"),
                 table=dpos, tab_row=w["dec_tab"], ldt=Dd, dst_row=w["dec_dst"], out_f32=xd[0], ldo32=Dd,
                 prefetch=self._pf("fwd", "decoder_embed.weight", Me))
        ops.fill_mask_tokens(xd[0], w["mask"], st.param("mask_token"), dpos, B, L, Dd, n_extra=E)
        for i in range(cfg.decoder_depth):
            self._block_fwd(xd[i], xd[i + 1], w["dec"][i], f"decoder_blocks.{i}", Md, Dd, cfg.decoder_num_heads, B, Nd)
        ops.layernorm_fwd(xd[-1], st.param("decoder_norm.weight"), st.param("decoder_norm.bias"), w["dlat_lp"],
                          w["dlat_mean"], w["dlat_rstd"], Md, Dd, cfg.ln_eps)
        ops.gemm(w["dlat_lp"], st.lp("decoder_pred.weight"), M=Md, N=pv, K=Dd, bias=st.param("decoder_pred.bias"),
                 out_f32=w["pred"])
        ops.masked_patch_loss(imgs, w["pred"], w["mask"], w["loss"], w["dpred"], None, self.code, w["loss_ws"],
                              cfg.patch_size, E, cfg.pixel_mean, cfg.pixel_std, cfg.norm_pix_loss, cfg.loss_fn != "mse",
                              dscale=self.loss_scale)
        self._last = (imgs, B, keep)
        return w["loss"], w["pred"][:, E:, :], w["mask"]

    def _linear_bwd(self, dy, x_in, wname, bname, M, N, K, w, dx_out=None, dx_act=0, dx_aux=None, wgrad=True, prefetch="chain"):
        st = self.store
        if wgrad:
            self._wgrad(dy, x_in, N, K, M, st.grad(wname), st.grad(bname), w)
        if dx_out is not None:
            self._before_write(dx_out)
            ops.gemm(dy, st.lp(wname), M=M, N=K, K=N, a_layout=KC, b_layout=RC, lda=N, ldb=K, act=dx_act, aux=dx_aux,
                     ldaux=K, out=dx_out, ws=w["splitk_ws"], prefetch=self._pf("bwd", wname, M) if isinstance(prefetch, str) else prefetch)

    def enable_wgrad_overlap(self, on=True):
        if bool(on) != (self._side is not None):
            if self._ws and self._graph_captures:
                raise RuntimeError("enable_wgrad_overlap: the weight-gradient schedule cannot change while HIP graphs captured on this "
                                   "engine's workspaces exist (build a new engine, or construct every TrainStep with the same wgrad_overlap)")
            self._ws, self._last = {}, None
        if on and self._side is None:
            self._side = torch.cuda.Stream(device=self.device)
            self._splitk_ws_side = torch.zeros_like(self.splitk_ws)
        elif not on:
            self._side = None
        self._pending = {}

    def note_graph_capture(self):
        self._graph_captures += 1

    def _wgrad(self, dy, x_in, M, N, K, dW, db, w):
        def launch(ws):
            ops.gemm(dy, x_in, M=M, N=N, K=K, a_layout=RC, b_layout=RC, lda=M, ldb=N, out_f32=dW, colsum_a=db, ws=ws)
        if self._side is None:
            launch(w["splitk_ws"])
        else:
            self._pending[dy.data_ptr()] = self._on_side(lambda: launch(self._splitk_ws_side))

    def _on_side(self, launch):
        ready = torch.cuda.Event()
        ready.record()
        self._side.wait_event(ready)
        with torch.cuda.stream(self._side):
            launch()
            done = torch.cuda.Event()
            done.record()
        return done

    def _before_write(self, buf):
        if self._side is not None:
            ev = self._pending.pop(buf.data_ptr(), None)
            if ev is not None:
                torch.cuda.current_stream().wait_event(ev)

    def _end_stage(self, w, last=False):
        if self._side is not None:
            torch.cuda.current_stream().wait_stream(self._side)
            self._pending.clear()
            self._group_done = None
        if self._ln_count:
            ops.layernorm_bwd_reduce_batch(w["ln_items"], self._ln_first, self._ln_count)
        self._ln_first, self._ln_count = (0, 0) if last else (self._ln_first + self._ln_count, 0)

    def _ln_bwd(self, dy, x, prefix, mean, rstd, g_in, g, g_lp, M, dim, w):
        st = self.store
        k = w["ln_index"][prefix]
        assert k == self._ln_first + self._ln_count, "LayerNorm backward visited out of table order"
        self._ln_count += 1
        self._before_write(g_lp)
        ops.layernorm_bwd(dy, x, st.param(f"{prefix}.weight"), mean, rstd, g_in, g, g_lp, w["ln_parts"][prefix], None, None,
                          M, dim, self.code)

    def _bwd_set(self, prefix):
        stack, i = prefix.rsplit(".", 1)
        depth = self.cfg.depth if stack == "blocks" else self.cfg.decoder_depth
        return (depth - 1 - int(i)) & 1

    @staticmethod
    def _scratch(w, key, s, n):
        return (w[key] if s == 0 or (key + "_b") not in w else w[key + "_b"])[:n]

    def _wgrad_layers(self, prefix, bufs, M, dim, w):
        hidden = bufs["hpre"].shape[1]
        s = self._bwd_set(prefix)
        g_lp = self._scratch(w, "g_lp", s, M * dim).view(M, dim)
        g_lp2 = self._scratch(w, "g_lp2", s, M * dim).view(M, dim)
        dh = self._scratch(w, "dh", s, M * hidden).view(M, hidden)
        dqkv = self._scratch(w, "dqkv", s, 3 * M * dim).view(M, 3 * dim)
        return [(g_lp, bufs["hact"], f"{prefix}.mlp.fc2", dim, hidden), (dh, bufs["ln2"], f"{prefix}.mlp.fc1", hidden, dim),
                (g_lp2, bufs["att"], f"{prefix}.attn.proj", dim, dim), (dqkv, bufs["ln1"], f"{prefix}.attn.qkv", 3 * dim, dim)]

    def _make_wgrad_group(self, prefix, bufs, M, dim, w, adamw=None, g16=None, side=None):
        st = self.store

        def dst(name, n_out, k_in):
            if g16 is None:
                return dict(out_f32=st.grad(f"{name}.weight"))
            o = st.offsets[f"{name}.weight"]
            return dict(out=g16[o:o + n_out * k_in].view(n_out, k_in))
        layers = self._wgrad_layers(prefix, bufs, M, dim, w) + self._extra_wgrad_layers(prefix, M, w)
        tile = int(os.environ.get("SKYEMB_WGRAD_TILE_DEC" if prefix.startswith("decoder") else "SKYEMB_WGRAD_TILE_ENC", "0"))
        hint = self._pf("bwd", f"{prefix}.attn.qkv.weight", M)
        args = [ops.gemm_args(dy, x_in, M=n_out, N=k_in, K=M, a_layout=RC, b_layout=RC, lda=n_out, ldb=k_in,
                              colsum_a=st.grad(f"{name}.bias"), prefetch=hint if j == 0 else None, **dst(name, n_out, k_in))
                for j, (dy, x_in, name, n_out, k_in) in enumerate(layers)]
        grp = ops.GemmGroup(args, self.device, tile=tile, adamw=adamw, side=side, ln_bwd=self._norm1_side_record(prefix, bufs, M, dim, w))
        if grp.ok:
            grp.extra_layers = [name for _, _, name, _, _ in layers[4:]]
            if adamw is None and g16 is None:
                w.setdefault("folded_wgrads", set()).update(grp.extra_layers)
        return grp if grp.ok else None

    def _extra_wgrad_layers(self, prefix, M, w):
        if (os.environ.get("SKYEMB_FOLD_WGRADS", "1") == "0" or self._side is not None or "dpred" not in w
                or not self.fold_decoder_wgrads):
            return []
        cfg = self.cfg
        out = []
        if prefix == f"decoder_blocks.{cfg.decoder_depth - 1}" and w["dpred"].shape[0] == M:
            out.append((w["dpred"], w["dlat_lp"], "decoder_pred", cfg.patch_dim, cfg.decoder_embed_dim))
        if prefix == f"blocks.{cfg.depth - 1}" and "dE" in w and w["dE"].shape[0] == M:
            out.append((w["dE"], w["lat_lp"], "decoder_embed", cfg.decoder_embed_dim, cfg.embed_dim))
        return out

    def _block_input(self, prefix, w):
        tag, i = prefix.rsplit(".", 1)
        return (w["xs"] if tag == "blocks" else w["xd"])[int(i)]

    def _norm1_side_record(self, prefix, bufs, M, dim, w):
        if self._side is not None or os.environ.get("SKYEMB_LN_SIDE", "1") == "0" or "ln_parts" not in w:
            return None
        s = self._bwd_set(prefix)
        g = w["g"][:M * dim].view(M, dim)
        return dict(dy=w["dln"][:M * dim].view(M, dim), x=self._block_input(prefix, w), gamma=self.store.param(f"{prefix}.norm1.weight"),
                    mean=bufs["mean1"], rstd=bufs["rstd1"], g_in=g, g_out=g, g_lp=self._scratch(w, "g_lp", s ^ 1, M * dim).view(M, dim),
                    part=w["ln_parts"][f"{prefix}.norm1"], M=M, D=dim)

    def enable_fused_adamw(self, optimizer, on=True, side=None):
        self._variant_args["adamw"] = None
        if not on:
            return
        self._adamw_side = os.environ.get("SKYEMB_ADAMW_SIDE", "auto") if side is None else ("1" if side is True else "0" if side is False else str(side))
        assert self._adamw_side in ADAMW_SIDE_MODES, self._adamw_side
        self._adamw_side_blocks = int(os.environ.get("SKYEMB_SIDE_BLOCKS", "256"))
        assert self.dtype in ops.LP_DTYPES, "the fused optimiser step exists on the 16-bit paths (grouped weight gradients)"
        st = self.store
        b1, b2 = optimizer.defaults["betas"]
        d = AdamwDesc()
        d.g_base, d.p, d.m, d.v, d.p_lp = (t.data_ptr() for t in (st.g, st.p, st.m, st.v, st.p_lp))
        d.hyper = optimizer.hyper_device.data_ptr()
        d.n_decay = st.n_decay
        d.beta1, d.beta2, d.eps = b1, b2, optimizer.defaults["eps"]
        d.weight_decay, d.grad_scale = optimizer.param_groups[1]["weight_decay"], optimizer.grad_scale
        self._enable_variant("adamw", d)

    def _enable_variant(self, kind, arg):
        self._variant_args[kind] = arg
        for w in self._ws.values():
            if "wgrad_groups" in w:
                self._build_variant_groups(w, kind)

    @property
    def adamw_side(self):
        return self._adamw_side

    @property
    def fused_adamw_desc(self):
        return self._variant_args["adamw"]

    @contextmanager
    def wgrad_variant(self, kind):
        assert kind in WGRAD_GROUPS_KEY, kind
        prev, self._variant = self._variant, kind
        try:
            yield
        finally:
            self._variant = prev

    def enable_grad_mirror(self, g16):
        self._enable_variant("g16", g16)

    def grad_mirror_ranges(self, w):
        return list(w.get("g16_ranges", []))

    def fused_adamw_ranges(self, w):
        return list(w.get("fused_ranges", []))

    def _wgrad_launch_order(self, w):
        order = [f"decoder_blocks.{i}" for i in reversed(range(len(w.get("dec", []))))]
        return order + [f"blocks.{i}" for i in reversed(range(self.cfg.depth))]

    def _block_weight_span(self, prefix):
        spans = merge_spans(self.store.span(f"{prefix}.{n}.weight") for n in ("attn.qkv", "attn.proj", "mlp.fc1", "mlp.fc2"))
        assert len(spans) == 1, "a block's weight matrices are not contiguous in the flat buffers"
        return spans[0]

    def _build_variant_groups(self, w, kind):
        st, arg = self.store, self._variant_args[kind]
        plain = w["wgrad_groups"]
        groups, spans = {}, []
        order = [p for p in self._wgrad_launch_order(w) if plain.get(p) is not None]
        plan = [(False, False)] * len(order)
        if kind == "adamw":
            ncu = torch.cuda.get_device_properties(self.device).multi_processor_count
            plan = plan_wgrad_schedule(order, [(plain[p].info.tile, plain[p].tile_blocks) for p in order], ncu, self._adamw_side)
            w["adamw_side_launches"] = sum(carries for carries, _ in plan)
        for k, (prefix, (carries, stores)) in enumerate(zip(order, plan)):
            tag, i = prefix.rsplit(".", 1)
            bufs = (w["enc"] if tag == "blocks" else w["dec"])[int(i)]
            M, dim = bufs["ln1"].shape
            side = None
            if carries or stores:
                lo, hi = self._block_weight_span(order[k - 1]) if carries else (0, 0)
                side = (not stores, lo, hi, self._adamw_side_blocks if hi > lo else 0)
            grp = self._make_wgrad_group(prefix, bufs, M, dim, w, side=side, **{kind: arg})
            if grp is None:
                assert side is None, f"side optimiser jobs: the grouped launch of {prefix} could not be planned"
                continue
            groups[prefix] = grp
            spans += [st.span(f"{prefix}.{name}.weight") for name in ("attn.qkv", "attn.proj", "mlp.fc1", "mlp.fc2")]
            if not stores:
                spans += [st.span(f"{name}.weight") for name in grp.extra_layers]
        w[WGRAD_GROUPS_KEY[kind]] = groups
        w["fused_ranges" if kind == "adamw" else "g16_ranges"] = merge_spans(spans)

    def _block_bwd(self, x_in, bufs, prefix, M, dim, heads, Bsz, N, g, g_lp, w):
        hd = dim // heads
        hidden = bufs["hpre"].shape[1]
        s = self._bwd_set(prefix)
        g_lp = self._scratch(w, "g_lp", s, M * dim).view(M, dim)
        g_lp_next = self._scratch(w, "g_lp", s ^ 1, M * dim).view(M, dim)
        dh = self._scratch(w, "dh", s, M * hidden).view(M, hidden)
        dqkv = self._scratch(w, "dqkv", s, 3 * M * dim).view(M, 3 * dim)
        dln = w["dln"][:M * dim].view(M, dim)
        datt = w["datt"][:M * dim].view(M, dim)
        group = w["wgrad_groups"].get(prefix)
        if self._variant_args.get(self._variant) is not None:
            group = w.get(WGRAD_GROUPS_KEY[self._variant], {}).get(prefix, group)
        single = group is None
        g_mid = g_lp if single else self._scratch(w, "g_lp2", s, M * dim).view(M, dim)
        self._linear_bwd(g_lp, bufs["hact"], f"{prefix}.mlp.fc2.weight", f"{prefix}.mlp.fc2.bias", M, dim, hidden, w,
                         dx_out=dh, dx_act=ACT_DGELU, dx_aux=bufs["hpre"], wgrad=single)
        self._linear_bwd(dh, bufs["ln2"], f"{prefix}.mlp.fc1.weight", f"{prefix}.mlp.fc1.bias", M, hidden, dim, w,
                         dx_out=dln, wgrad=single)
        self._ln_bwd(dln, bufs["xmid"], f"{prefix}.norm2", bufs["mean2"], bufs["rstd2"], g, g, g_mid, M, dim, w)
        self._linear_bwd(g_mid, bufs["att"], f"{prefix}.attn.proj.weight", f"{prefix}.attn.proj.bias", M, dim, dim, w,
                         dx_out=datt, wgrad=single)
        self._before_write(dqkv)
        ops.mha_bwd(bufs["qkv"], datt, dqkv, Bsz, N, heads, hd)
        self._linear_bwd(dqkv, bufs["ln1"], f"{prefix}.attn.qkv.weight", f"{prefix}.attn.qkv.bias", M, 3 * dim, dim, w,
                         dx_out=dln, wgrad=single, prefetch="chain" if group is None else None)
        prev_done = self._group_done
        if group is not None:
            if self._side is None:
                group.launch()
            else:
                self._group_done = self._on_side(group.launch)
        if prev_done is not None:
            torch.cuda.current_stream().wait_event(prev_done)
        if group is not None and group.ln_side:
            assert w["ln_index"][f"{prefix}.norm1"] == self._ln_first + self._ln_count, "LayerNorm backward visited out of table order"
            assert x_in.data_ptr() == self._block_input(prefix, w).data_ptr()
            self._ln_count += 1
        else:
            self._ln_bwd(dln, x_in, f"{prefix}.norm1", bufs["mean1"], bufs["rstd1"], g, g, g_lp_next, M, dim, w)

    def last_key(self):
        assert self._last is not None, "no forward_train() yet"
        return (self._last[1], self._last[2], True)

    def last_workspace(self):
        return self._ws[self.last_key()]

    def start_backward_at(self, ln_name):
        self._ln_first, self._ln_count = self.last_workspace()["ln_index"][ln_name], 0

    def _bwd_ctx(self):
        assert self._last is not None, "backward() without forward_train()"
        imgs, B, keep = self._last
        cfg = self.cfg
        L, E = cfg.num_patches, cfg.num_extra_tokens
        return imgs, B, keep, E + keep, E + L, self._ws[(B, keep, True)]

    def backward_decoder(self):
        imgs, B, keep, Ne, Nd, w = self._bwd_ctx()
        cfg, st = self.cfg, self.store
        L, D, Dd, pv = cfg.num_patches, cfg.embed_dim, cfg.decoder_embed_dim, cfg.patch_dim
        Me, Md = B * Ne, B * Nd
        self._ln_first = self._ln_count = 0
        dln = w["dln"][:Md * Dd].view(Md, Dd)
        self._linear_bwd(w["dpred"], w["dlat_lp"], "decoder_pred.weight", "decoder_pred.bias", Md, pv, Dd, w, dx_out=dln,
                         wgrad="decoder_pred" not in w.get("folded_wgrads", ()))
        g = w["g"][:Md * Dd].view(Md, Dd)
        g_lp = w["g_lp"][:Md * Dd].view(Md, Dd)
        self._ln_bwd(dln, w["xd"][-1], "decoder_norm", w["dlat_mean"], w["dlat_rstd"], None, g, g_lp, Md, Dd, w)
        for i in reversed(range(cfg.decoder_depth)):
            self._block_bwd(w["xd"][i], w["dec"][i], f"decoder_blocks.{i}", Md, Dd, cfg.decoder_num_heads, B, Nd, g,
                            g_lp, w)
        ops.rowsum_select(g, Dd, w["mask"], cfg.num_extra_tokens, L, Nd, B * L, Dd, w["rs_part"], st.grad("mask_token").view(Dd))
        ops.gather_rows(g, w["dec_dst"], None, w["dE"], Me, Dd)
        dln_e = w["dln"][:Me * D].view(Me, D)
        self._linear_bwd(w["dE"], w["lat_lp"], "decoder_embed.weight", "decoder_embed.bias", Me, Dd, D, w, dx_out=dln_e,
                         wgrad="decoder_embed" not in w.get("folded_wgrads", ()))
        self._end_stage(w)

    def backward_encoder(self, hi=None, lo=0):
        imgs, B, keep, Ne, Nd, w = self._bwd_ctx()
        cfg = self.cfg
        D = cfg.embed_dim
        Me = B * Ne
        g = w["g"][:Me * D].view(Me, D)
        g_lp = w["g_lp"][:Me * D].view(Me, D)
        if hi is None:
            hi = cfg.depth
            dln_e = w["dln"][:Me * D].view(Me, D)
            self._ln_bwd(dln_e, w["xs"][cfg.depth], "norm", w["lat_mean"], w["lat_rstd"], None, g, g_lp, Me, D, w)
        for i in reversed(range(lo, hi)):
            self._block_bwd(w["xs"][i], w["enc"][i], f"blocks.{i}", Me, D, cfg.num_heads, B, Ne, g, g_lp, w)
        self._end_stage(w)

    def backward_embed(self):
        imgs, B, keep, Ne, Nd, w = self._bwd_ctx()
        self._embed_bwd(B, Ne, keep, w)
        ops.patch_gather_bwd_pmv(imgs, w["ids_keep"], w["drows"], w["pmv_part"], self.store.grad("patch_mask_values"),
                                 self.cfg.patch_size, keep)
        self._end_stage(w, last=True)

    def _embed_bwd(self, B, Ne, n_patch, w):
        cfg, st = self.cfg, self.store
        D, pv = cfg.embed_dim, cfg.patch_dim
        g = w["g"][:B * Ne * D].view(B * Ne, D)
        ops.rowsum_select(g, D, None, 0, 1, Ne, B, D, w["rs_part"], st.grad("cls_token").view(D))
        if cfg.ra_dec:
            G = st.grad
            ops.radec_token_bwd(g.view(-1)[D:], Ne * D, st.param("ra_dec_embed.neural_network.last_layer.weight"), w["sh"],
                                w["z"], w["dz"], G("ra_dec_embed.neural_network.layers.0.weight"),
                                G("ra_dec_embed.neural_network.layers.0.bias"), G("ra_dec_embed.neural_network.last_layer.weight"),
                                G("ra_dec_embed.neural_network.last_layer.bias"), B, D)
        ops.gather_rows(g, w["pe_dst"], None, w["dT"], B * n_patch, D)
        self._wgrad(w["dT"], w["patches"], D, pv, B * n_patch, st.grad("patch_embed.proj.weight"),
                    st.grad("patch_embed.proj.bias"), w)
        ops.gemm(w["dT"], st.lp("patch_embed.proj.weight"), M=B * n_patch, N=pv, K=D, a_layout=KC, b_layout=RC, lda=D,
                 ldb=pv, out_f32=w["drows"])

    def backward(self):
        self.backward_decoder()
        self.backward_encoder()
        self.backward_embed()

    def backward_stages(self, n_encoder_groups=3):
        groups, ranges = self._stage_ranges(n_encoder_groups)
        stages = [(self.backward_decoder, ranges[0])]
        for k, (hi, lo) in enumerate(groups):
            stages.append(((lambda h=hi, l=lo, top=(k == 0): self.backward_encoder(None if top else h, l)), ranges[1 + k]))
        stages.append((self.backward_embed, ranges[-1]))
        return stages

    def _stage_ranges(self, n_encoder_groups):
        return stage_gradient_ranges(self.store, self.cfg, n_encoder_groups)

    def flops_per_image(self, mask_ratio=0.75):
        cfg = self.cfg
        L, D, Dd, pv = cfg.num_patches, cfg.embed_dim, cfg.decoder_embed_dim, cfg.patch_dim
        keep = int(L * (1 - mask_ratio))
        Ne, Nd = cfg.num_extra_tokens + keep, cfg.num_extra_tokens + L
        r = cfg.mlp_ratio

        def blocks(n, d, depth, heads):
            lin = 2 * n * d * (3 * d + d + 2 * r * d)
            att = 2 * 2 * n * n * d
            return depth * (lin + att)
        common = blocks(Ne, D, cfg.depth, cfg.num_heads) + 2 * Ne * D * Dd + blocks(Nd, Dd, cfg.decoder_depth,
                                                                                  cfg.decoder_num_heads) + 2 * Nd * Dd * pv
        executed = 3 * (common + 2 * keep * pv * D)
        algorithmic = 3 * (common + 2 * L * pv * D)
        return executed, algorithmic
```

### sky_embeddings_amd/ops.py

```python
from __future__ import annotations

import ctypes
import os

import torch

from . import _lib
from ._lib import (ACT_DGELU, ACT_GELU, ACT_NONE, BF16, COMBINE_MAX, COMBINE_MEAN, COMBINE_MIN, F16, F32, KC, RC, AdamwDesc,
                   GemmArgs, GemmGroupInfo, LnBwdSide, check, lib)

TORCH_DTYPE = {BF16: torch.bfloat16, F32: torch.float32, F16: torch.float16}
LP_DTYPES = (torch.bfloat16, torch.float16)


def dtype_code(t: torch.dtype) -> int:
    if t == torch.bfloat16:
        return BF16
    if t == torch.float32:
        return F32
    if t == torch.float16:
        return F16
    raise TypeError(f"unsupported activation dtype {t}")


def _stream():
    return torch.cuda.current_stream().cuda_stream


def _p(t):
    if t is None:
        return None
    assert t.is_cuda, "libskyemb ops need device tensors (there is no CPU fallback)"
    return t.data_ptr()


def _prefetch_on():
    import os
    return os.environ.get("SKYEMB_PREFETCH", "1") != "0"


def gemm_args(A, B, *, M, N, K, a_layout=KC, b_layout=KC, lda=None, ldb=None, alpha=1.0, bias=None, table=None,
              tab_row=None, ldt=0, dst_row=None, resid=None, ldr=0, aux=None, ldaux=0, act=ACT_NONE, out_f32=None, ldo32=0,
              out=None, ldo=0, out2=None, ldo2=0, tile=0, colsum_a=None, ws=None, split_k=0, prefetch=None):
    g = GemmArgs()
    g.A, g.B = _p(A), _p(B)
    g.lda = lda if lda is not None else (K if a_layout == KC else M)
    g.ldb = ldb if ldb is not None else (K if b_layout == KC else N)
    g.a_layout, g.b_layout = a_layout, b_layout
    g.M, g.N, g.K = M, N, K
    g.dtype = dtype_code(A.dtype)
    assert B.dtype == A.dtype
    g.alpha = alpha
    g.bias, g.table, g.tab_row, g.ldt, g.dst_row = _p(bias), _p(table), _p(tab_row), ldt, _p(dst_row)
    g.resid, g.ldr, g.aux, g.ldaux, g.act = _p(resid), ldr, _p(aux), ldaux, act
    g.out_f32, g.ldo32, g.out, g.ldo, g.out2, g.ldo2 = _p(out_f32), ldo32 or N, _p(out), ldo or N, _p(out2), ldo2 or N
    g.tile = tile
    g.colsum_a = _p(colsum_a)
    g.ws, g.ws_bytes, g.split_k = _p(ws), (ws.numel() * ws.element_size() if ws is not None else 0), split_k
    if prefetch is not None and _prefetch_on():
        g.prefetch, g.prefetch_bytes = _p(prefetch), prefetch.numel() * prefetch.element_size() // 4 * 4
    return g


def gemm(A, B, **kw):
    g = gemm_args(A, B, **kw)
    check(lib().skyemb_gemm(ctypes.byref(g), _stream()), "skyemb_gemm")


class GemmGroup:

    def __init__(self, args, device, tile=0, adamw=None, side=None, ln_bwd=None):
        n = len(args)
        arr = (GemmArgs * n)(*args)
        nbytes = lib().skyemb_gemm_group_blob_bytes(n)
        host = torch.zeros(nbytes, dtype=torch.uint8)
        self.info = GemmGroupInfo()
        if side is not None:
            own, lo, hi, blocks = side
            rc = lib().skyemb_gemm_group_plan_side_adamw(arr, n, tile, ctypes.byref(adamw), int(bool(own)), int(lo), int(hi), int(blocks),
                                                         host.data_ptr(), nbytes, ctypes.byref(self.info))
        elif adamw is not None:
            rc = lib().skyemb_gemm_group_plan_adamw(arr, n, tile, ctypes.byref(adamw), host.data_ptr(), nbytes, ctypes.byref(self.info))
        else:
            rc = lib().skyemb_gemm_group_plan(arr, n, tile, host.data_ptr(), nbytes, ctypes.byref(self.info))
        self.ok = rc == 0
        if rc > 0:
            check(rc, "skyemb_gemm_group_plan")
        self.tile_blocks = self.info.total_blocks - (int(side[3]) if side is not None else 0)
        self.ln_side = False
        if self.ok and ln_bwd is not None and ln_bwd["dy"].dtype in LP_DTYPES:
            rec = LnBwdSide()
            for k in ("dy", "x", "gamma", "mean", "rstd", "g_in", "g_out", "g_lp", "part"):
                setattr(rec, k, _p(ln_bwd[k]))
            rec.M, rec.D = ln_bwd["M"], ln_bwd["D"]
            rc2 = lib().skyemb_gemm_group_attach_ln_bwd(host.data_ptr(), nbytes, ctypes.byref(self.info), ctypes.byref(rec))
            if rc2 > 0:
                check(rc2, "skyemb_gemm_group_attach_ln_bwd")
            self.ln_side = rc2 == 0
        self.total_blocks = self.info.total_blocks
        self.blob = host.to(device) if self.ok else None

    def launch(self):
        check(lib().skyemb_gemm_group_launch(self.blob.data_ptr(), ctypes.byref(self.info), _stream()), "skyemb_gemm_group_launch")


GEMM_COUNT_NAMES = ("fallback", "pipe", "tile256", "group", "group256", "splitk")


def gemm_launch_counts(reset=False):
    buf = (ctypes.c_longlong * 8)()
    check(lib().skyemb_gemm_launch_counts(ctypes.cast(buf, ctypes.c_void_p), 8, int(reset)), "skyemb_gemm_launch_counts")
    return dict(zip(GEMM_COUNT_NAMES, list(buf)))


def colsum(X, M, N, out, ldx=None):
    code = dtype_code(X.dtype)
    check(lib().skyemb_colsum(_p(X), code, ldx if ldx is not None else N, M, N, _p(out), _stream()), "skyemb_colsum")


def random_mask_from_noise(noise, keep, ids_restore, mask, ids_keep, dec_dst=None, dec_tab=None, n_extra=1):
    B, L = noise.shape
    check(lib().skyemb_random_mask_from_noise(_p(noise), B, L, keep, _p(ids_restore), _p(mask), _p(ids_keep),
                                              _p(dec_dst), _p(dec_tab), n_extra, _stream()), "skyemb_random_mask_from_noise")


def augment(imgs, out, params, nan_mask, noise, A):
    B, C, S, _ = imgs.shape
    check(lib().skyemb_augment(_p(imgs), _p(out), _p(params), _p(nan_mask), _p(noise), B, C, S, A, _stream()), "skyemb_augment")


def tile_cutouts(tile, big_endian, h0, w0, S, out, lo=None, hi=None):
    C, H, W = tile.shape
    check(lib().skyemb_tile_cutouts(_p(tile), _p(big_endian), C, H, W, _p(h0), _p(w0), h0.numel(), S,
                                    0.0 if lo is None else float(lo), 0.0 if hi is None else float(hi), int(lo is not None),
                                    int(hi is not None), _p(out), _stream()), "skyemb_tile_cutouts")


def attnpool_q(latent, Wq, bq, q):
    check(lib().skyemb_attnpool_q(_p(latent), _p(Wq), _p(bq), _p(q), q.numel(), _stream()), "skyemb_attnpool_q")


def attnpool_fwd(q, kv, out, prob, B, N, H, hd):
    check(lib().skyemb_attnpool_fwd(_p(q), _p(kv), dtype_code(kv.dtype), _p(out), _p(prob), B, N, H, hd, _stream()), "skyemb_attnpool_fwd")


def attnpool_bwd(q, kv, dout, prob, dkv, dq_part, B, N, H, hd):
    check(lib().skyemb_attnpool_bwd(_p(q), _p(kv), dtype_code(kv.dtype), _p(dout), _p(prob), _p(dkv), _p(dq_part), B, N, H, hd,
                                    _stream()), "skyemb_attnpool_bwd")


def attnpool_fwd_long(q, kv, out, prob, B, N, H, hd):
    check(lib().skyemb_attnpool_fwd_long(_p(q), _p(kv), dtype_code(kv.dtype), _p(out), _p(prob), B, N, H, hd, _stream()),
          "skyemb_attnpool_fwd_long")


def attnpool_bwd_long(q, kv, dout, prob, dkv, dq_part, B, N, H, hd):
    check(lib().skyemb_attnpool_bwd_long(_p(q), _p(kv), dtype_code(kv.dtype), _p(dout), _p(prob), _p(dkv), _p(dq_part), B, N, H, hd,
                                         _stream()), "skyemb_attnpool_bwd_long")


def attnpool_q_bwd(dq_part, latent, Wq, dWq, dbq, dlatent, ws):
    B, D = dq_part.shape
    check(lib().skyemb_attnpool_q_bwd(_p(dq_part), B, _p(latent), _p(Wq), _p(dWq), _p(dbq), _p(dlatent), _p(ws), D, _stream()),
          "skyemb_attnpool_q_bwd")


def simmim_mask_from_noise(noise, ratio_u, max_ratio, grid, p, out_mask):
    B, C, L = noise.shape
    check(lib().skyemb_simmim_mask_from_noise(_p(noise), _p(ratio_u), max_ratio, B, C, L, grid, p, _p(out_mask), _stream()),
          "skyemb_simmim_mask_from_noise")


def patch_gather(imgs, pmv, ids_keep, out, p, keep, pixel_mean, pixel_std):
    B, C, H, W = imgs.shape
    check(lib().skyemb_patch_gather(_p(imgs), _p(pmv), _p(ids_keep), _p(out), dtype_code(out.dtype), B, C, H, W, p,
                                    keep, pixel_mean, pixel_std, _stream()), "skyemb_patch_gather")


def patch_gather_bwd_pmv(imgs, ids_keep, drows, partial, dpmv, p, keep):
    B, C, H, W = imgs.shape
    check(lib().skyemb_patch_gather_bwd_pmv(_p(imgs), _p(ids_keep), _p(drows), _p(partial), _p(dpmv), B, C, H, W, p,
                                            keep, _stream()), "skyemb_patch_gather_bwd_pmv")


def patch_gather_blend(imgs, pmv, ids_keep, pixel_mask, out, p, keep, pixel_mean, pixel_std):
    B, C, H, W = imgs.shape
    check(lib().skyemb_patch_gather_blend(_p(imgs), _p(pmv), _p(ids_keep), _p(pixel_mask), _p(out), dtype_code(out.dtype), B, C,
                                          H, W, p, keep, pixel_mean, pixel_std, _stream()), "skyemb_patch_gather_blend")


def patch_gather_bwd_pmv_blend(imgs, ids_keep, pixel_mask, drows, partial, dpmv, p, keep):
    B, C, H, W = imgs.shape
    check(lib().skyemb_patch_gather_bwd_pmv_blend(_p(imgs), _p(ids_keep), _p(pixel_mask), _p(drows), _p(partial), _p(dpmv), B,
                                                  C, H, W, p, keep, _stream()), "skyemb_patch_gather_bwd_pmv_blend")


def radec_token_fwd(ra_dec, W0, b0, W1, b1, pos_row, x_rows, row_stride, B, D, sh, z):
    check(lib().skyemb_radec_token_fwd(_p(ra_dec), _p(W0), _p(b0), _p(W1), _p(b1), _p(pos_row), _p(x_rows), row_stride, B, D,
                                       _p(sh), _p(z), _stream()), "skyemb_radec_token_fwd")


def radec_token_bwd(g_rows, row_stride, W1, sh, z, dz_ws, dW0, db0, dW1, db1, B, D):
    check(lib().skyemb_radec_token_bwd(_p(g_rows), row_stride, _p(W1), _p(sh), _p(z), _p(dz_ws), _p(dW0), _p(db0), _p(dW1),
                                       _p(db1), B, D, _stream()), "skyemb_radec_token_bwd")


def simmim_pixel_loss(imgs, pred_tok, pixel_mask, loss, dpred_tok, dtype, pred_img, ws, p, extra, pixel_mean, pixel_std,
                      norm_pix, loss_l1, pooled=False, dscale=1.0):
    B, C, H, W = imgs.shape
    check(lib().skyemb_simmim_pixel_loss(_p(imgs), _p(pred_tok), _p(pixel_mask), _p(loss), _p(dpred_tok), dtype, _p(pred_img),
                                         _p(ws), B, C, H, W, p, extra, pixel_mean, pixel_std, int(norm_pix), int(loss_l1),
                                         int(pooled), float(dscale), _stream()), "skyemb_simmim_pixel_loss")


def layernorm_fwd(x, gamma, beta, y, mean, rstd, M, D, eps, y32=None, dtype=None):
    code = dtype if dtype is not None else dtype_code(y.dtype)
    check(lib().skyemb_layernorm_fwd(_p(x), _p(gamma), _p(beta), _p(y), _p(y32), code, _p(mean), _p(rstd), M, D, eps,
                                     _stream()), "skyemb_layernorm_fwd")


def layernorm_bwd_blocks(M):
    return lib().skyemb_layernorm_bwd_blocks(M)


def layernorm_bwd(dy, x, gamma, mean, rstd, g_in, g_out, g_lp, part, dgamma, dbeta, M, D, dtype):
    dy_f32 = 1 if (dy.dtype == torch.float32 and dtype in (BF16, F16)) else 0
    check(lib().skyemb_layernorm_bwd(_p(dy), dy_f32, dtype, _p(x), _p(gamma), _p(mean), _p(rstd), _p(g_in), _p(g_out),
                                     _p(g_lp), _p(part), _p(dgamma), _p(dbeta), M, D, _stream()), "skyemb_layernorm_bwd")


def ln_reduce_items(entries, device):
    rows = [[part.data_ptr(), dg.data_ptr(), db.data_ptr() if db is not None else 0, nblk + (D << 32)] for part, dg, db, nblk, D in entries]
    blocks, first = [], [0]
    for k, (part, dg, db, nblk, D) in enumerate(entries):
        for y in range(2 if db is not None else 1):
            blocks += [[k, x | (y << 16)] for x in range((D + 31) // 32)]
        first.append(len(blocks))
    return (torch.tensor(rows, dtype=torch.int64).to(device), torch.tensor(blocks, dtype=torch.int32).to(device), first)


def layernorm_bwd_reduce_batch(table, first, count):
    items, blocks, first_block = table
    b0, b1 = first_block[first], first_block[first + count]
    check(lib().skyemb_layernorm_bwd_reduce_batch(items.data_ptr(), blocks.data_ptr() + 8 * b0, b1 - b0, _stream()),
          "skyemb_layernorm_bwd_reduce_batch")


def mha_fwd(qkv, out, B, N, H, hd):
    check(lib().skyemb_mha_fwd(_p(qkv), _p(out), dtype_code(qkv.dtype), B, N, H, hd, _stream()), "skyemb_mha_fwd")


def mha_bwd(qkv, dout, dqkv, B, N, H, hd):
    check(lib().skyemb_mha_bwd(_p(qkv), _p(dout), _p(dqkv), dtype_code(qkv.dtype), B, N, H, hd, _stream()),
          "skyemb_mha_bwd")


def fill_mask_tokens(x, mask, mask_token, dec_pos, B, L, Dd, n_extra=1):
    check(lib().skyemb_fill_mask_tokens(_p(x), _p(mask), _p(mask_token), _p(dec_pos), B, L, Dd, n_extra, _stream()),
          "skyemb_fill_mask_tokens")


def gather_rows(src, idx, out, out_lp, n_rows, D):
    code = dtype_code(out_lp.dtype) if out_lp is not None else F32
    check(lib().skyemb_gather_rows(_p(src), _p(idx), _p(out), _p(out_lp), code, n_rows, D, _stream()),
          "skyemb_gather_rows")


def rowsum_select(src, ld, sel, row0, inner, outer_stride, n_rows, D, partial, out):
    check(lib().skyemb_rowsum_select(_p(src), ld, _p(sel), row0, inner, outer_stride, n_rows, D, _p(partial), _p(out),
                                     _stream()), "skyemb_rowsum_select")


def masked_patch_loss(imgs, pred, mask, loss, dpred, dpred32, dtype, ws, p, extra, pixel_mean, pixel_std, norm_pix,
                      loss_l1, dscale=1.0):
    B, C, H, W = imgs.shape
    check(lib().skyemb_masked_patch_loss(_p(imgs), _p(pred), _p(mask), _p(loss), _p(dpred), _p(dpred32), dtype, _p(ws),
                                         B, C, H, W, p, extra, pixel_mean, pixel_std, int(norm_pix), int(loss_l1),
                                         float(dscale), _stream()), "skyemb_masked_patch_loss")


def adamw(p, g, m, v, p_lp, n, n_decay, hyper, beta1, beta2, eps, wd, grad_scale=1.0, zero_grad=False, lr=0.0, bc1=1.0,
          bc2=1.0):
    code = dtype_code(p_lp.dtype) if p_lp is not None else F32
    check(lib().skyemb_adamw(_p(p), _p(g), _p(m), _p(v), _p(p_lp), code, n, n_decay, _p(hyper), lr, bc1, bc2, beta1,
                             beta2, eps, wd, grad_scale, int(zero_grad), dtype_code(g.dtype), _stream()), "skyemb_adamw")


def set_scalars(dst, a, b=0.0, c=0.0, d=0.0):
    check(lib().skyemb_set_scalars(_p(dst), a, b, c, d, _stream()), "skyemb_set_scalars")


def cast(src, dst, n):
    check(lib().skyemb_cast(_p(src), _p(dst), dtype_code(dst.dtype), n, _stream()), "skyemb_cast")


def standardise(x, mu, sigma, out):
    N, D = x.shape
    check(lib().skyemb_standardise(_p(x), _p(mu), _p(sigma), _p(out), N, D, _stream()), "skyemb_standardise")


def weighted_norms(x, w, norms, xw_out=None):
    N, D = x.shape
    check(lib().skyemb_weighted_norms(_p(x), _p(w), _p(norms), _p(xw_out), N, D, _stream()), "skyemb_weighted_norms")


def cosine_topk_chunks(N, Q, D, k):
    return lib().skyemb_cosine_topk_chunks(N, Q, D, k)


def cosine_topk(tw, qn, bank, xn, k, eps, idx_offset, nchunks, part_s, part_i, thr0=None):
    Q, D = tw.shape
    N = bank.shape[0]
    check(lib().skyemb_cosine_topk(_p(tw), _p(qn), _p(bank), _p(xn), Q, N, D, k, eps, idx_offset, nchunks, _p(thr0),
                                   _p(part_s), _p(part_i), _stream()), "skyemb_cosine_topk")


def kth_largest_floor(x, k, out):
    Q, S = x.shape
    check(lib().skyemb_kth_largest_floor(_p(x), Q, S, k, _p(out), _stream()), "skyemb_kth_largest_floor")


def sample_floor_applicable(Q, S, D, k, *tensors):
    return bool(lib().skyemb_cosine_sample_floor_applicable(Q, S, D, k)) and all(t.data_ptr() % 16 == 0 for t in tensors)


def cosine_sample_floor(tw, qn, sample, sample_norms, k, eps, ws, out):
    Q, D = tw.shape
    S = sample.shape[0]
    check(lib().skyemb_cosine_sample_floor(_p(tw), _p(qn), _p(sample), _p(sample_norms), Q, S, D, k, eps, _p(ws), _p(out), _stream()),
          "skyemb_cosine_sample_floor")


def topk_prefilter_applicable(Q, N, D, k):
    return bool(lib().skyemb_topk_prefilter_applicable(Q, N, D, k))


def bank16_prepare(bank, xn):
    N, D = bank.shape
    rows = lib().skyemb_bank16_rowp_rows(N)
    assert lib().skyemb_bank16_bytes(N, D) == rows * D * 2
    bank16 = torch.empty(rows, D, device=bank.device, dtype=torch.float16)
    rowp = torch.empty(rows, 4, device=bank.device, dtype=torch.float32)
    check(lib().skyemb_bank16_prepare(_p(bank), _p(xn), N, D, _p(bank16), _p(rowp), _stream()), "skyemb_bank16_prepare")
    return bank16, rowp


def cosine_topk_prefiltered(tw, qn, bank, xn, bank16, rowp, k, eps, idx_offset, out_s, out_i, redo, thr0=None, ws=None):
    Q, D = tw.shape
    N = bank.shape[0]
    need = lib().skyemb_topk_prefilter_ws_bytes(Q, D, k)
    if ws is None or ws.numel() < need:
        ws = torch.empty(need, device=tw.device, dtype=torch.uint8)
    check(lib().skyemb_cosine_topk_prefiltered(_p(tw), _p(qn), Q, _p(bank), _p(xn), _p(bank16), _p(rowp), N, D, k, eps, idx_offset,
                                               _p(thr0), _p(ws), ws.numel(), _p(out_s), _p(out_i), _p(redo), _stream()),
          "skyemb_cosine_topk_prefiltered")
    return ws


def topk_merge(in_s, in_i, Q, nlists, k, out_s, out_i, ws=None):
    check(lib().skyemb_topk_merge(_p(in_s), _p(in_i), Q, nlists, k, _p(out_s), _p(out_i), _p(ws), _stream()),
          "skyemb_topk_merge")


def cosine_scores(tw, qn, bank, xn, eps, scores):
    Q, D = tw.shape
    N = bank.shape[0]
    check(lib().skyemb_cosine_scores(_p(tw), _p(qn), _p(bank), _p(xn), Q, N, D, eps, _p(scores), _stream()),
          "skyemb_cosine_scores")


COMBINE_CODES = {"min": COMBINE_MIN, "mean": COMBINE_MEAN, "max": COMBINE_MAX}


def cosine_token_applicable(Q, P, D, k):
    return bool(lib().skyemb_cosine_token_applicable(Q, P, D, k))


def cosine_token_refusal(Q, P, D, k):
    L = lib()
    return None if L.skyemb_cosine_token_applicable(Q, P, D, k) else L.skyemb_last_error().decode()


def cosine_token_topk_chunks(N, P, Q, D, k):
    return lib().skyemb_cosine_token_topk_chunks(N, P, Q, D, k)


def cosine_token_scores(tw, qn, bank, xn, combine, eps, scores):
    Q, D = tw.shape
    N, P = bank.shape[0], bank.shape[1]
    check(lib().skyemb_cosine_token_scores(_p(tw), _p(qn), _p(bank), _p(xn), Q, N, P, D, combine, eps, _p(scores), _stream()),
          "skyemb_cosine_token_scores")


def cosine_token_topk(tw, qn, bank, xn, k, combine, eps, idx_offset, nlists, part_s, part_i, thr0=None):
    Q, D = tw.shape
    N, P = bank.shape[0], bank.shape[1]
    check(lib().skyemb_cosine_token_topk(_p(tw), _p(qn), _p(bank), _p(xn), Q, N, P, D, k, combine, eps, idx_offset, nlists, _p(thr0),
                                         _p(part_s), _p(part_i), _stream()), "skyemb_cosine_token_topk")
```

### sky_embeddings_amd/optim.py

```python
from __future__ import annotations

import math

import numpy as np
import torch

from . import ops


class FusedAdamW:
    def __init__(self, engine, lr=1e-4, betas=(0.9, 0.95), eps=1e-8, weight_decay=0.05, process_group=None):
        self.engine = engine
        self.store = engine.store
        self.defaults = dict(lr=lr, betas=tuple(betas), eps=eps, weight_decay=weight_decay)
        self.param_groups = [dict(lr=lr, initial_lr=lr, betas=tuple(betas), eps=eps, weight_decay=0.0),
                             dict(lr=lr, initial_lr=lr, betas=tuple(betas), eps=eps, weight_decay=weight_decay)]
        self.step_count = 0
        self.base_grad_scale = 1.0
        self.hyper_device = None
        self.process_group = process_group
        self.grad_buffer = None

    @property
    def grad_scale(self):
        return self.base_grad_scale / getattr(self.engine, "loss_scale", 1.0)

    @grad_scale.setter
    def grad_scale(self, v):
        self.base_grad_scale = float(v) * getattr(self.engine, "loss_scale", 1.0)

    @property
    def lr(self):
        return self.param_groups[0]["lr"]

    def set_lr(self, lr):
        for g in self.param_groups:
            g["lr"] = lr

    def zero_grad(self, set_to_none=True):
        return None

    def step(self):
        self.begin_step()
        self.apply_range(0, self.store.n)

    def use_device_scalars(self, device):
        if self.hyper_device is None:
            self.hyper_device = torch.zeros(4, device=device, dtype=torch.float32)
        self.write_scalars(max(self.step_count, 1))
        return self.hyper_device

    def write_scalars(self, t):
        lr, bc1, bc2 = self.step_scalars(t)
        ops.set_scalars(self.hyper_device, lr, bc1, bc2)

    def begin_step(self):
        self.step_count += 1
        if self.hyper_device is not None:
            self.write_scalars(self.step_count)

    def apply_range(self, start, end, grad=None):
        b1, b2 = self.defaults["betas"]
        t = self.step_count
        st = self.store
        n = end - start
        if n <= 0:
            return
        n_decay = min(max(st.n_decay - start, 0), n)
        sl = slice(start, end)
        g = st.g if self.grad_buffer is None else self.grad_buffer
        if grad is not None:
            g, sl_g = grad, slice(0, n)
        else:
            sl_g = sl
        ops.adamw(st.p[sl], g[sl_g], st.m[sl], st.v[sl], st.p_lp[sl], n, n_decay, self.hyper_device, b1, b2,
                  self.defaults["eps"], self.param_groups[1]["weight_decay"], grad_scale=self.grad_scale, zero_grad=False,
                  lr=self.lr, bc1=1.0 - b1 ** t, bc2=1.0 - b2 ** t)

    def step_scalars(self, t=None):
        b1, b2 = self.defaults["betas"]
        t = self.step_count + 1 if t is None else t
        return self.lr, 1.0 - b1 ** t, 1.0 - b2 ** t

    def _index(self):
        from .model_config import FROZEN, state_layout
        st = self.store
        stateless = {n for n in st.frozen if n not in FROZEN}
        if not stateless:
            return list(st.no_decay), list(st.decay)
        no_decay, decay = [], []
        have = set(st.no_decay) | set(st.decay)
        for name, shape in state_layout(st.cfg):
            if name in have:
                (no_decay if name in st.no_decay else decay).append(name)
            elif name in stateless:
                (no_decay if (len(shape) <= 1 or name.endswith(".bias")) else decay).append(None)
        return no_decay, decay

    def state_dict(self):
        st = self.store
        no_decay, decay = self._index()
        names = no_decay + decay
        state = {}
        if self.step_count > 0:
            for i, n in enumerate(names):
                if n is None:
                    continue
                state[i] = {"step": torch.tensor(float(self.step_count)),
                            "exp_avg": st._view(st.m, n).detach().clone(),
                            "exp_avg_sq": st._view(st.v, n).detach().clone()}
        nd = len(no_decay)
        groups = []
        for gi, ids in enumerate((list(range(nd)), list(range(nd, len(names))))):
            g = dict(self.param_groups[gi])
            g.update(amsgrad=False, foreach=None, maximize=False, capturable=False, differentiable=False, fused=None,
                     params=ids)
            groups.append(g)
        return {"state": state, "param_groups": groups}

    def load_state_dict(self, sd):
        st = self.store
        no_decay, decay = self._index()
        names = no_decay + decay
        groups = sd["param_groups"]
        assert [len(g["params"]) for g in groups] == [len(no_decay), len(decay)], \
            "optimizer state does not match this model (parameter counts per weight-decay group differ)"
        for g_new, g_old in zip(self.param_groups, groups):
            for k in ("lr", "initial_lr", "weight_decay", "eps"):
                if k in g_old:
                    g_new[k] = g_old[k]
            if "betas" in g_old:
                g_new["betas"] = tuple(g_old["betas"])
        self.defaults["betas"] = self.param_groups[0]["betas"]
        steps = set()
        for i, n in enumerate(names):
            s = sd["state"].get(i)
            if s is None or n is None:
                continue
            st._view(st.m, n).copy_(s["exp_avg"].to(torch.float32))
            st._view(st.v, n).copy_(s["exp_avg_sq"].to(torch.float32))
            steps.add(int(float(s["step"])))
        assert len(steps) <= 1, "per-parameter step counts differ; unsupported"
        self.step_count = steps.pop() if steps else 0


class CosineLR:

    def __init__(self, optimizer, T_max, eta_min=0.0):
        self.optimizer = optimizer
        self.T_max = int(T_max)
        self.eta_min = float(eta_min)
        self.base_lr = float(optimizer.param_groups[0].get("initial_lr", optimizer.lr))
        self.last_epoch = 0
        self._apply()

    def _lr_at(self, t):
        return self.eta_min + (self.base_lr - self.eta_min) * (1 + math.cos(math.pi * t / self.T_max)) / 2

    def _apply(self):
        self.optimizer.set_lr(self._lr_at(self.last_epoch))

    def step(self):
        self.last_epoch += 1
        self._apply()

    def get_last_lr(self):
        return [self.optimizer.lr for _ in self.optimizer.param_groups]

    def state_dict(self):
        return {"T_max": self.T_max, "eta_min": self.eta_min, "base_lrs": [self.base_lr] * 2,
                "last_epoch": self.last_epoch, "_step_count": self.last_epoch + 1, "_last_lr": self.get_last_lr()}

    def load_state_dict(self, sd):
        self.T_max = int(sd.get("T_max", self.T_max))
        self.eta_min = float(sd.get("eta_min", self.eta_min))
        if "base_lrs" in sd:
            self.base_lr = float(sd["base_lrs"][0])
        self.last_epoch = int(sd["last_epoch"])
        self._apply()
```

### sky_embeddings_amd/train_step.py

```python
from __future__ import annotations

import os

import torch

from . import ops
from .distributed import all_gather_range, bucket_bounds, reduce_scatter_range, shard_chunk
from .engine import subtract_spans
from .optim import CosineLR, FusedAdamW


class TrainStep:
    def __init__(self, engine, optimizer: FusedAdamW, scheduler: CosineLR, batch_size: int, mask_ratio: float = 0.75,
                 use_graph: bool = True, process_group=None, world_size: int = 1, warmup_iters: int = 2,
                 staged: bool | None = None, n_encoder_groups: int | None = None, bucket_elems: int = 32 * 1024 * 1024,
                 wgrad_overlap: bool | None = None, optimizer_overlap: bool | None = None, grad_comm: str | None = None,
                 external_noise: bool = False, max_mask_ratio: float | None = None, fused_adamw: bool | None = None,
                 adamw_side: bool | None = None, shard_optimizer: bool | None = None, shard_emulate: tuple | None = None):
        self.engine, self.optimizer, self.scheduler = engine, optimizer, scheduler
        self.mask_ratio = mask_ratio
        self.world_size = world_size
        self.process_group = process_group
        self.collectives = world_size > 1 or (os.environ.get("SKYEMB_DIST_FORCE", "0") == "1" and torch.distributed.is_available()
                                              and torch.distributed.is_initialized())
        self.bucket_elems = bucket_elems
        cfg = engine.cfg
        dev = engine.device
        self.imgs = torch.zeros(batch_size, cfg.in_chans, cfg.img_size, cfg.img_size, device=dev)
        self.noise = torch.zeros(batch_size, cfg.num_patches, device=dev)
        self.simmim = bool(cfg.simmim)
        self.pixel_mask = torch.zeros_like(self.imgs) if self.simmim else None
        self.max_mask_ratio = max_mask_ratio if self.simmim else None
        if self.max_mask_ratio is not None:
            self.mask_noise = torch.zeros(batch_size, cfg.in_chans, cfg.num_patches, device=dev)
            self.ratio_u = torch.zeros(batch_size, device=dev)
        self.ra_dec = torch.zeros(batch_size, 2, device=dev) if cfg.ra_dec else None
        self.loss = None
        self.external_noise = external_noise
        explicit_comm = grad_comm is not None
        if grad_comm is None:
            grad_comm = os.environ.get("SKYEMB_GRAD_COMM", "bf16")
        assert grad_comm in ("bf16", "f32"), grad_comm
        self.grad_comm = grad_comm if (world_size > 1 or (staged and explicit_comm)) else "f32"
        self.g16 = None
        if self.grad_comm == "bf16":
            self.g16 = torch.zeros(engine.store.n, device=dev, dtype=engine.dtype if engine.dtype in ops.LP_DTYPES else torch.bfloat16)
        if staged is None:
            env = os.environ.get("SKYEMB_STAGED")
            staged = (world_size > 1) if env is None else env == "1"
        self.staged = staged
        if wgrad_overlap is None:
            wgrad_overlap = os.environ.get("SKYEMB_WGRAD_OVERLAP", "0") == "1"
        engine.enable_wgrad_overlap(wgrad_overlap)
        engine.loss_scale = engine.plan_loss_scale(engine.expected_masked_elements(batch_size, mask_ratio))
        optimizer.base_grad_scale = 1.0 / world_size
        if n_encoder_groups is None:
            n_encoder_groups = 6 if world_size > 1 else 3
        if self.staged:
            stages = engine.backward_stages(min(n_encoder_groups, cfg.depth))
            first_fn, first_ranges = stages[0]
            self.stages = [((lambda: (self._forward(), first_fn())), first_ranges)] + stages[1:]
        else:
            self.stages = [((lambda: (self._forward(), engine.backward())), [(0, engine.store.n)])]
        if self.g16 is not None:
            direct = os.environ.get("SKYEMB_G16_DIRECT", "1") == "1"
            if direct:
                engine.enable_grad_mirror(self.g16)

            def with_cast(fn, ranges):
                todo = []

                def run():
                    with engine.wgrad_variant("g16" if direct else "plain"):
                        fn()
                    if not todo:
                        holes = []
                        if direct:
                            holes = engine.grad_mirror_ranges(engine.last_workspace())
                        todo.append(subtract_spans(ranges, holes))
                    for (s, e) in todo[0]:
                        ops.cast(engine.store.g[s:e], self.g16[s:e], e - s)
                return run
            self.stages = [(with_cast(fn, ranges), ranges) for fn, ranges in self.stages]
        if optimizer_overlap is None:
            optimizer_overlap = self.staged and os.environ.get("SKYEMB_OPT_OVERLAP", "0") == "1"
        self.optimizer_overlap = bool(optimizer_overlap and self.staged)
        if self.optimizer_overlap:
            covered = sorted(r for _, rs in self.stages for r in rs)
            assert covered[0][0] == 0 and covered[-1][1] == engine.store.n and all(a[1] == b[0] for a, b in zip(covered, covered[1:])), \
                "backward stages must partition the flat parameter buffer"
            self.opt_stream = torch.cuda.Stream(device=dev)
        if shard_optimizer is None:
            env = os.environ.get("SKYEMB_SHARD_OPT", "auto")
            shard_optimizer = (world_size > 1) if env == "auto" else env == "1"
        self.shard_rank, self.shard_world = (shard_emulate if shard_emulate is not None else
                                             ((torch.distributed.get_rank(process_group), world_size) if self.collectives and world_size > 1 else (0, 1)))
        self.shard_emulated = shard_emulate is not None
        forced_one = self.collectives and self.shard_world == 1 and shard_optimizer is True and os.environ.get("SKYEMB_SHARD_OPT", "auto") != "0"
        self.shard_optimizer = bool(shard_optimizer and self.staged and (self.shard_world > 1 or forced_one) and not self.optimizer_overlap)
        self._own = {}
        if self.shard_optimizer:
            gdt = engine.store.g.dtype if self.g16 is None else self.g16.dtype
            for k, (_, ranges) in enumerate(self.stages[:-1]):
                for (s_, e_) in ranges:
                    self._own[(s_, e_)] = torch.zeros(max(shard_chunk(e_ - s_, self.shard_world), 8), device=dev, dtype=gdt)
        if fused_adamw is None:
            fused_adamw = os.environ.get("SKYEMB_FUSED_ADAMW", "1") == "1"
        self.fused_adamw = bool(fused_adamw and world_size == 1 and not self.staged and not self.optimizer_overlap
                                and engine.dtype in ops.LP_DTYPES)
        self._rest_ranges = None
        snap = None
        if self.fused_adamw:
            optimizer.use_device_scalars(dev)
            engine.enable_fused_adamw(optimizer, side=adamw_side)
            self.adamw_side = engine.adamw_side
            st = engine.store
            snap = [t.clone() for t in (st.p, st.m, st.v, st.p_lp)]

            self._fused_consts = self._optimizer_consts()

            def owning(fn):
                def run():
                    with engine.wgrad_variant("adamw"):
                        fn()
                    for (s_, e_) in self._rest():
                        optimizer.apply_range(s_, e_)
                return run
            self.stages = [(owning(fn), ranges) for fn, ranges in self.stages]
        self.graphs = None
        if use_graph:
            s = torch.cuda.Stream(device=dev)
            s.wait_stream(torch.cuda.current_stream(dev))
            with torch.cuda.stream(s):
                for _ in range(warmup_iters):
                    for fn, _ in self.stages:
                        fn()
            torch.cuda.current_stream(dev).wait_stream(s)
            torch.cuda.synchronize(dev)
            self.graphs = []
            pool = None
            for fn, _ in self.stages:
                g = torch.cuda.CUDAGraph()
                with torch.cuda.graph(g, pool=pool):
                    fn()
                pool = g.pool()
                self.graphs.append(g)
            engine.note_graph_capture()
        if snap is not None:
            if not use_graph:
                self.stages[0][0]()
            torch.cuda.synchronize(dev)
            for dst, src in zip((engine.store.p, engine.store.m, engine.store.v, engine.store.p_lp), snap):
                dst.copy_(src)

    def _sharded_update(self):
        opt, st = self.optimizer, self.engine.store
        r, W = self.shard_rank, self.shard_world
        opt.begin_step()
        gathers = []
        for k, (_, ranges) in enumerate(self.stages):
            for (s, e) in ranges:
                if k + 1 == len(self.stages):
                    opt.apply_range(s, e)
                    continue
                c = shard_chunk(e - s, W)
                if c > 0:
                    own = self._own[(s, e)]
                    if self.shard_emulated:
                        opt.apply_range(s + r * c, s + (r + 1) * c)
                    else:
                        opt.apply_range(s + r * c, s + (r + 1) * c, grad=own[:c])
                opt.apply_range(s + W * c, e)
                if self.collectives and c > 0:
                    gathers.append(all_gather_range(st.p_lp, s, e, r, W, self.process_group))
        for w in gathers:
            if w is not None:
                w.wait()

    def gather_full_state(self):
        if not (self.shard_optimizer and self.collectives) or self.shard_emulated:
            return
        st = self.engine.store
        works = []
        for k, (_, ranges) in enumerate(self.stages[:-1]):
            for (s, e) in ranges:
                for buf in (st.p, st.m, st.v):
                    works.append(all_gather_range(buf, s, e, self.shard_rank, self.shard_world, self.process_group))
        for w in works:
            if w is not None:
                w.wait()
        torch.cuda.synchronize(self.engine.device)

    def _optimizer_consts(self):
        o = self.optimizer
        return (tuple(o.defaults["betas"]), o.defaults["eps"], o.param_groups[1]["weight_decay"], o.grad_scale)

    def _rest(self):
        if self._rest_ranges is None:
            eng = self.engine
            assert eng.last_key() == self._ws_key
            self._rest_ranges = subtract_spans([(0, eng.store.n)], eng.fused_adamw_ranges(eng.last_workspace()))
            self._rest_key = self._ws_key
        assert self._rest_key == self._ws_key, "TrainStep: the batch shape changed under a fused optimiser step"
        return self._rest_ranges

    def _forward(self):
        if self.simmim:
            if self.max_mask_ratio is not None:
                if not self.external_noise:
                    self.mask_noise.uniform_()
                    self.ratio_u.uniform_()
                cfg = self.engine.cfg
                ops.simmim_mask_from_noise(self.mask_noise, self.ratio_u, float(self.max_mask_ratio), cfg.grid, cfg.patch_size,
                                           self.pixel_mask)
            self.loss, self.pred, self.mask = self.engine.forward_train(self.imgs, mask=self.pixel_mask, ra_dec=self.ra_dec)
            self._ws_key = self.engine.last_key()
            return
        if not self.external_noise:
            self.noise.uniform_()
        self.loss, self.pred, self.mask = self.engine.forward_train(self.imgs, self.mask_ratio, self.noise, ra_dec=self.ra_dec)
        self._ws_key = self.engine.last_key()

    def load_batch(self, imgs, mask=None, ra_dec=None):
        self.imgs.copy_(imgs, non_blocking=True)
        if self.simmim:
            if self.max_mask_ratio is None:
                assert mask is not None, "SimMIM steps need the per-pixel mask (or TrainStep(max_mask_ratio=...))"
                self.pixel_mask.copy_(mask, non_blocking=True)
        if self.ra_dec is not None:
            self.ra_dec.copy_(ra_dec, non_blocking=True)

    def __call__(self, imgs=None, mask=None, ra_dec=None):
        if imgs is not None:
            self.load_batch(imgs, mask, ra_dec)
        if self.fused_adamw:
            if self._optimizer_consts() != self._fused_consts:
                raise RuntimeError("TrainStep: betas / eps / weight_decay / grad_scale of the optimiser changed after the fused "
                                   "weight-gradient launches were built (load the checkpoint BEFORE constructing TrainStep, or rebuild it)")
            self.optimizer.begin_step()
            if self.graphs is not None:
                self.graphs[0].replay()
            else:
                self.stages[0][0]()
            self.scheduler.step()
            return self.loss
        works = []
        g = self.engine.store.g if self.g16 is None else self.g16
        self.optimizer.grad_buffer = self.g16
        overlap = self.optimizer_overlap
        main = torch.cuda.current_stream(self.engine.device)
        if overlap:
            self.optimizer.begin_step()
            self.opt_stream.wait_stream(main)
        for k, (fn, ranges) in enumerate(self.stages):
            if self.graphs is not None:
                self.graphs[k].replay()
            else:
                fn()
            stage_works = []
            sharded = self.shard_optimizer and k + 1 < len(self.stages)
            if self.collectives and sharded:
                for (s, e) in ranges:
                    stage_works += reduce_scatter_range(g, s, e, self.shard_rank, self.shard_world, self._own[(s, e)], self.process_group)
            elif self.collectives:
                for (s, e) in ranges:
                    for (bs, be) in bucket_bounds(e - s, self.bucket_elems):
                        stage_works.append(torch.distributed.all_reduce(g[s + bs:s + be], group=self.process_group,
                                                                        async_op=True))
            if overlap:
                done = torch.cuda.Event()
                done.record(main)
                with torch.cuda.stream(self.opt_stream):
                    self.opt_stream.wait_event(done)
                    for w in stage_works:
                        w.wait()
                    for (s, e) in ranges:
                        self.optimizer.apply_range(s, e)
            else:
                works += stage_works
        if overlap:
            main.wait_stream(self.opt_stream)
        else:
            for w in works:
                w.wait()
            if self.shard_optimizer:
                self._sharded_update()
            else:
                self.optimizer.step()
        self.optimizer.grad_buffer = None
        self.scheduler.step()
        return self.loss
```

Measured before the change: 52810 images/sec.

## Fold small seam kernels into fused gather, rowsum-gather and multi-range AdamW launches

Merges the patch gather, cls+pos token write and decoder mask-token fill into one kernel launch. In backward it fuses the cls rowsum with the patch-row gather and defers some small reductions into the batched LN reduce. It also replaces the per-range AdamW launches for leftover parameters with a single multi-range kernel. The aim is fewer tiny kernel launches and graph nodes per step. The cost is more complex kernel dispatch by block index, behind an env flag that is on by default.

After: 53170 images/sec (median of 6 runs). No clear change (+0.7%).

```diff
diff --git a/include/skyemb.h b/include/skyemb.h
--- a/include/skyemb.h
+++ b/include/skyemb.h
@@ -124,6 +124,11 @@
 int skyemb_patch_gather_bwd_pmv(const float *imgs, const int32_t *ids_keep, const float *drows, float *partial,
                                 float *dpmv, int B, int C, int H, int W, int p, int keep, void *stream);
 
+int skyemb_patch_gather_seams(const float *imgs, const float *pmv, const int32_t *ids_keep, void *out, int dtype, int B, int C, int H,
+                              int W, int p, int keep, float pixel_mean, float pixel_std, const float *cls, const float *pos0, float *x0,
+                              int64_t x0_stride, int D, float *xd, const float *mask, const float *mask_token, const float *dec_pos,
+                              int L, int Dd, int n_extra, void *stream);
+
 int skyemb_layernorm_fwd(const float *x, const float *gamma, const float *beta, void *y, float *y32, int dtype,
                          float *mean, float *rstd, int M, int D, float eps, void *stream);
 
@@ -150,6 +155,9 @@
 int skyemb_rowsum_select(const float *src, int64_t ld, const float *sel, int row0, int inner, int outer_stride,
                          int n_rows, int D, float *partial, float *out, void *stream);
 
+int skyemb_rowsum_gather(const float *src, const float *sel, int row0, int inner, int outer_stride, int n_rows, int D, float *partial,
+                         float *out_sum, const int32_t *idx, float *out, void *out_lp, int dtype, int n_gather, void *stream);
+
 int skyemb_masked_patch_loss(const float *imgs, const float *pred, const float *mask, float *loss, void *dpred,
                              float *dpred32, int dtype, float *ws, int B, int C, int H, int W, int p, int extra,
                              float pixel_mean, float pixel_std, int norm_pix, int loss_l1, float dscale, void *stream);
@@ -162,6 +170,10 @@
 int skyemb_adamw(float *p, void *g, float *m, float *v, void *p_lp, int dtype, int64_t n, int64_t n_decay,
                  const float *hyper, float lr, float bc1, float bc2, float beta1, float beta2, float eps, float wd,
                  float grad_scale, int zero_grad, int grad_dtype, void *stream);
+#define SKYEMB_ADAMW_MAX_RANGES 8
+int skyemb_adamw_ranges(float *p, const float *g, float *m, float *v, void *p_lp, int dtype, const int64_t *lo, const int64_t *hi,
+                        int n_ranges, int64_t n_decay, const float *hyper, float beta1, float beta2, float eps, float wd,
+                        float grad_scale, void *stream);
 int skyemb_cast(const float *src, void *dst, int dtype, int64_t n, void *stream);
 
 int skyemb_gather_rows_host(const void *src, int64_t row_bytes, const int64_t *idx, int64_t n, int64_t src_rows, void *dst,
diff --git a/sky_embeddings_amd/_lib.py b/sky_embeddings_amd/_lib.py
--- a/sky_embeddings_amd/_lib.py
+++ b/sky_embeddings_amd/_lib.py
@@ -110,6 +110,11 @@
                                          c_i32, c_i32, c_f32, c_f32, c_i32, c_i32, c_f32, c_vp]),
     "skyemb_adamw": (c_i32, [c_vp, c_vp, c_vp, c_vp, c_vp, c_i32, c_i64, c_i64, c_vp, c_f32, c_f32, c_f32, c_f32,
                              c_f32, c_f32, c_f32, c_f32, c_i32, c_i32, c_vp]),
+    "skyemb_adamw_ranges": (c_i32, [c_vp, c_vp, c_vp, c_vp, c_vp, c_i32, c_vp, c_vp, c_i32, c_i64, c_vp, c_f32, c_f32, c_f32, c_f32, c_f32,
+                                    c_vp]),
+    "skyemb_patch_gather_seams": (c_i32, [c_vp, c_vp, c_vp, c_vp, c_i32, c_i32, c_i32, c_i32, c_i32, c_i32, c_i32, c_f32, c_f32, c_vp, c_vp,
+                                          c_vp, c_i64, c_i32, c_vp, c_vp, c_vp, c_vp, c_i32, c_i32, c_i32, c_vp]),
+    "skyemb_rowsum_gather": (c_i32, [c_vp, c_vp, c_i32, c_i32, c_i32, c_i32, c_i32, c_vp, c_vp, c_vp, c_vp, c_vp, c_i32, c_i32, c_vp]),
     "skyemb_cast": (c_i32, [c_vp, c_vp, c_i32, c_i64, c_vp]),
     "skyemb_standardise": (c_i32, [c_vp, c_vp, c_vp, c_vp, c_i64, c_i32, c_vp]),
     "skyemb_weighted_norms": (c_i32, [c_vp, c_vp, c_vp, c_vp, c_i64, c_i32, c_vp]),
diff --git a/sky_embeddings_amd/csrc/adamw.hip b/sky_embeddings_amd/csrc/adamw.hip
--- a/sky_embeddings_amd/csrc/adamw.hip
+++ b/sky_embeddings_amd/csrc/adamw.hip
@@ -40,6 +40,53 @@
             *(f32x4 *)(v + 4 * i) = vv[u];
             if (LP) store4<T>(p_lp + 4 * i, pv[u][0], pv[u][1], pv[u][2], pv[u][3]);
             if (zero_grad) store4<GT>(g + 4 * i, 0.f, 0.f, 0.f, 0.f);
+        }
+    }
+}
+
+struct AdamwRanges {
+    int n;
+    int first[SKYEMB_ADAMW_MAX_RANGES + 1];
+    int64_t lo4[SKYEMB_ADAMW_MAX_RANGES];
+    int64_t n4[SKYEMB_ADAMW_MAX_RANGES];
+};
+
+template <typename T, bool LP>
+__global__ __launch_bounds__(256) void adamw_ranges_kernel(float *__restrict__ p, const float *__restrict__ g, float *__restrict__ m,
+                                                           float *__restrict__ v, T *__restrict__ p_lp, const AdamwRanges rs,
+                                                           int64_t n_decay, const float *__restrict__ hyper, float beta1, float beta2,
+                                                           float eps, float wd, float grad_scale) {
+    const SkyAdamScalars sc = sky_adam_scalars(hyper[0], hyper[1], hyper[2], beta1, beta2, eps, wd, grad_scale);
+    int r = 0;
+    while (r + 1 < rs.n && (int)blockIdx.x >= rs.first[r + 1]) ++r;
+    const int64_t base = rs.lo4[r], n4 = rs.n4[r];
+    const int64_t stride = (int64_t)(rs.first[r + 1] - rs.first[r]) * 256;
+    for (int64_t i0 = (int64_t)((int)blockIdx.x - rs.first[r]) * 256 + threadIdx.x; i0 < n4; i0 += 2 * stride) {
+        f32x4 pv[2], gv[2], mv[2], vv[2];
+#pragma unroll
+        for (int u = 0; u < 2; ++u) {
+            const int64_t i = base + i0 + u * stride;
+            if (i0 + u * stride < n4) {
+                pv[u] = *(const f32x4 *)(p + 4 * i);
+                gv[u] = *(const f32x4 *)(g + 4 * i);
+                mv[u] = *(const f32x4 *)(m + 4 * i);
+                vv[u] = *(const f32x4 *)(v + 4 * i);
+            }
+        }
+#pragma unroll
+        for (int u = 0; u < 2; ++u) {
+            const int64_t i = base + i0 + u * stride;
+            if (i0 + u * stride >= n4) break;
+#pragma unroll
+            for (int j = 0; j < 4; ++j) {
+                float pj = pv[u][j], mj = mv[u][j], vj = vv[u][j];
+                sky_adamw_update(gv[u][j], pj, mj, vj, 4 * i + j < n_decay, sc);
+                pv[u][j] = pj; mv[u][j] = mj; vv[u][j] = vj;
+            }
+            *(f32x4 *)(p + 4 * i) = pv[u];
+            *(f32x4 *)(m + 4 * i) = mv[u];
+            *(f32x4 *)(v + 4 * i) = vv[u];
+            if (LP) store4<T>(p_lp + 4 * i, pv[u][0], pv[u][1], pv[u][2], pv[u][3]);
         }
     }
 }
@@ -92,3 +139,41 @@
     SKY_LAUNCH_CHECK("skyemb_adamw");
     return 0;
 }
+
+extern "C" int skyemb_adamw_ranges(float *p, const float *g, float *m, float *v, void *p_lp, int dtype, const int64_t *lo,
+                                   const int64_t *hi, int n_ranges, int64_t n_decay, const float *hyper, float beta1, float beta2,
+                                   float eps, float wd, float grad_scale, void *stream) {
+    SKY_CHECK_ARG(p && g && m && v && lo && hi && hyper && n_ranges > 0 && n_ranges <= SKYEMB_ADAMW_MAX_RANGES && n_decay >= 0,
+                  "skyemb_adamw_ranges: bad arguments (n_ranges=%d, at most %d)", n_ranges, SKYEMB_ADAMW_MAX_RANGES);
+    SKY_CHECK_ARG(aligned16(p) && aligned16(g) && aligned16(m) && aligned16(v) && (((uintptr_t)p_lp) & 7) == 0,
+                  "skyemb_adamw_ranges: unaligned buffers");
+    AdamwRanges rs;
+    rs.n = n_ranges;
+    rs.first[0] = 0;
+    for (int r = 0; r < n_ranges; ++r) {
+        SKY_CHECK_ARG(lo[r] >= 0 && hi[r] > lo[r] && lo[r] % 4 == 0 && hi[r] % 4 == 0 && (r == 0 || lo[r] >= hi[r - 1]),
+                      "skyemb_adamw_ranges: range %d must be non-empty, a multiple of 4 at both ends and behind the one before it", r);
+        int64_t blocks = ceil_div64((hi[r] - lo[r]) / 4, 256);
+        if (blocks > 256 * 16) blocks = 256 * 16;
+        rs.lo4[r] = lo[r] / 4;
+        rs.n4[r] = (hi[r] - lo[r]) / 4;
+        rs.first[r + 1] = rs.first[r] + (int)blocks;
+    }
+    for (int r = n_ranges; r < SKYEMB_ADAMW_MAX_RANGES; ++r) rs.lo4[r] = rs.n4[r] = 0, rs.first[r + 1] = rs.first[n_ranges];
+    hipStream_t st = (hipStream_t)stream;
+    dim3 grid((unsigned)rs.first[n_ranges]), block(256);
+    if (!p_lp)
+        hipLaunchKernelGGL((adamw_ranges_kernel<float, false>), grid, block, 0, st, p, g, m, v, (float *)nullptr, rs, n_decay, hyper, beta1,
+                           beta2, eps, wd, grad_scale);
+    else if (dtype == SKYEMB_BF16)
+        hipLaunchKernelGGL((adamw_ranges_kernel<bf16_t, true>), grid, block, 0, st, p, g, m, v, (bf16_t *)p_lp, rs, n_decay, hyper, beta1,
+                           beta2, eps, wd, grad_scale);
+    else if (dtype == SKYEMB_F16)
+        hipLaunchKernelGGL((adamw_ranges_kernel<f16_t, true>), grid, block, 0, st, p, g, m, v, (f16_t *)p_lp, rs, n_decay, hyper, beta1,
+                           beta2, eps, wd, grad_scale);
+    else
+        hipLaunchKernelGGL((adamw_ranges_kernel<float, true>), grid, block, 0, st, p, g, m, v, (float *)p_lp, rs, n_decay, hyper, beta1,
+                           beta2, eps, wd, grad_scale);
+    SKY_LAUNCH_CHECK("skyemb_adamw_ranges");
+    return 0;
+}
diff --git a/sky_embeddings_amd/csrc/frontend.hip b/sky_embeddings_amd/csrc/frontend.hip
--- a/sky_embeddings_amd/csrc/frontend.hip
+++ b/sky_embeddings_amd/csrc/frontend.hip
@@ -70,11 +70,10 @@
 }
 
 template <typename T>
-__global__ __launch_bounds__(256) void patch_gather_kernel(const float *__restrict__ imgs, const float *__restrict__ pmv,
-                                                           const int32_t *__restrict__ ids_keep, T *__restrict__ out,
-                                                           int C, int H, int W, int p, int keep, float mean, float stdv,
-                                                           const float *__restrict__ pmask) {
-    const int row = blockIdx.x;
+__device__ __forceinline__ void patch_gather_row(const float *__restrict__ imgs, const float *__restrict__ pmv,
+                                                 const int32_t *__restrict__ ids_keep, T *__restrict__ out,
+                                                 int C, int H, int W, int p, int keep, float mean, float stdv,
+                                                 const float *__restrict__ pmask, const int row) {
     const int b = row / keep;
     const int l = ids_keep ? ids_keep[row] : (row - b * keep);
     const int gw = W / p;
@@ -106,6 +105,14 @@
     }
 }
 
+template <typename T>
+__global__ __launch_bounds__(256) void patch_gather_kernel(const float *__restrict__ imgs, const float *__restrict__ pmv,
+                                                           const int32_t *__restrict__ ids_keep, T *__restrict__ out,
+                                                           int C, int H, int W, int p, int keep, float mean, float stdv,
+                                                           const float *__restrict__ pmask) {
+    patch_gather_row<T>(imgs, pmv, ids_keep, out, C, H, W, p, keep, mean, stdv, pmask, (int)blockIdx.x);
+}
+
 __global__ __launch_bounds__(256) void pmv_partial_kernel(const float *__restrict__ imgs, const int32_t *__restrict__ ids_keep,
                                                           const float *__restrict__ drows, float *__restrict__ partial,
                                                           int C, int H, int W, int p, int keep, const float *__restrict__ pmask) {
@@ -150,10 +157,10 @@
     if (wave == 0 && n < N) out[n] = (red[0][lane] + red[1][lane]) + (red[2][lane] + red[3][lane]);
 }
 
-__global__ __launch_bounds__(256) void fill_mask_tokens_kernel(float *__restrict__ x, const float *__restrict__ mask,
-                                                               const float *__restrict__ mask_token,
-                                                               const float *__restrict__ dec_pos, int L, int Dd, int E) {
-    const int b = blockIdx.x / L, l = blockIdx.x % L;
+__device__ __forceinline__ void fill_mask_token_row(float *__restrict__ x, const float *__restrict__ mask,
+                                                    const float *__restrict__ mask_token, const float *__restrict__ dec_pos,
+                                                    int L, int Dd, int E, const int row) {
+    const int b = row / L, l = row % L;
     if (mask[(int64_t)b * L + l] == 0.0f) return;
     float *dst = x + ((int64_t)b * (L + E) + E + l) * Dd;
     const float *pos = dec_pos + (int64_t)(E + l) * Dd;
@@ -163,10 +170,45 @@
     }
 }
 
-template <typename T>
-__global__ __launch_bounds__(256) void gather_rows_kernel(const float *__restrict__ src, const int32_t *__restrict__ idx,
-                                                          float *__restrict__ out, T *__restrict__ out_lp, int D) {
-    const int r = blockIdx.x;
+__global__ __launch_bounds__(256) void fill_mask_tokens_kernel(float *__restrict__ x, const float *__restrict__ mask,
+                                                               const float *__restrict__ mask_token,
+                                                               const float *__restrict__ dec_pos, int L, int Dd, int E) {
+    fill_mask_token_row(x, mask, mask_token, dec_pos, L, Dd, E, (int)blockIdx.x);
+}
+
+struct FwdSeams {
+    const float *cls, *pos0;
+    float *x0;
+    int64_t x0_stride;
+    int D, n_cls;
+    float *xd;
+    const float *mask, *mask_token, *dec_pos;
+    int L, Dd, E, n_fill;
+};
+
+template <typename T>
+__global__ __launch_bounds__(256) void patch_gather_seams_kernel(const float *__restrict__ imgs, const float *__restrict__ pmv,
+                                                                 const int32_t *__restrict__ ids_keep, T *__restrict__ out,
+                                                                 int C, int H, int W, int p, int keep, float mean, float stdv,
+                                                                 int n_gather, const FwdSeams s) {
+    int blk = (int)blockIdx.x;
+    if (blk < n_gather) return patch_gather_row<T>(imgs, pmv, ids_keep, out, C, H, W, p, keep, mean, stdv, nullptr, blk);
+    blk -= n_gather;
+    if (blk < s.n_cls) {
+        float *dst = s.x0 + (int64_t)blk * s.x0_stride;
+        for (int d = threadIdx.x * 4; d < s.D; d += 1024) {
+            const float4 t = *(const float4 *)(s.cls + d), q = *(const float4 *)(s.pos0 + d);
+            *(float4 *)(dst + d) = make_float4(t.x + q.x, t.y + q.y, t.z + q.z, t.w + q.w);
+        }
+        return;
+    }
+    blk -= s.n_cls;
+    if (blk < s.n_fill) fill_mask_token_row(s.xd, s.mask, s.mask_token, s.dec_pos, s.L, s.Dd, s.E, blk);
+}
+
+template <typename T>
+__device__ __forceinline__ void gather_row(const float *__restrict__ src, const int32_t *__restrict__ idx,
+                                           float *__restrict__ out, T *__restrict__ out_lp, int D, const int r) {
     const float *s = src + (int64_t)idx[r] * D;
     for (int d = threadIdx.x * 4; d < D; d += 1024) {
         const float4 v = *(const float4 *)(s + d);
@@ -175,14 +217,18 @@
     }
 }
 
-__global__ __launch_bounds__(256) void rowsum_select_kernel(const float *__restrict__ src, int64_t ld,
-                                                            const float *__restrict__ sel, int row0, int inner,
-                                                            int outer_stride, int n_rows, int D,
-                                                            float *__restrict__ partial) {
-    const int nblk = gridDim.x;
+template <typename T>
+__global__ __launch_bounds__(256) void gather_rows_kernel(const float *__restrict__ src, const int32_t *__restrict__ idx,
+                                                          float *__restrict__ out, T *__restrict__ out_lp, int D) {
+    gather_row<T>(src, idx, out, out_lp, D, (int)blockIdx.x);
+}
+
+__device__ __forceinline__ void rowsum_select_block(const float *__restrict__ src, int64_t ld, const float *__restrict__ sel,
+                                                    int row0, int inner, int outer_stride, int n_rows, int D,
+                                                    float *__restrict__ partial, const int blk, const int nblk) {
     for (int d = threadIdx.x; d < D; d += 256) {
         float acc = 0.f;
-        for (int i0 = blockIdx.x; i0 < n_rows; i0 += 4 * nblk) {
+        for (int i0 = blk; i0 < n_rows; i0 += 4 * nblk) {
             float x[4];
 #pragma unroll
             for (int u = 0; u < 4; ++u) {
@@ -196,8 +242,25 @@
             for (int u = 0; u < 4; ++u)
                 if (i0 + u * nblk < n_rows && !(sel && sel[i0 + u * nblk] == 0.0f)) acc += x[u];
         }
-        partial[(int64_t)blockIdx.x * D + d] = acc;
-    }
+        partial[(int64_t)blk * D + d] = acc;
+    }
+}
+
+__global__ __launch_bounds__(256) void rowsum_select_kernel(const float *__restrict__ src, int64_t ld,
+                                                            const float *__restrict__ sel, int row0, int inner,
+                                                            int outer_stride, int n_rows, int D,
+                                                            float *__restrict__ partial) {
+    rowsum_select_block(src, ld, sel, row0, inner, outer_stride, n_rows, D, partial, (int)blockIdx.x, (int)gridDim.x);
+}
+
+template <typename T>
+__global__ __launch_bounds__(256) void rowsum_gather_kernel(const float *__restrict__ src, int64_t ld, const float *__restrict__ sel,
+                                                            int row0, int inner, int outer_stride, int n_rows, int D,
+                                                            float *__restrict__ partial, int n_sum, const int32_t *__restrict__ idx,
+                                                            float *__restrict__ out, T *__restrict__ out_lp) {
+    if ((int)blockIdx.x < n_sum)
+        return rowsum_select_block(src, ld, sel, row0, inner, outer_stride, n_rows, D, partial, (int)blockIdx.x, n_sum);
+    gather_row<T>(src, idx, out, out_lp, D, (int)blockIdx.x - n_sum);
 }
 
 template <typename T>
@@ -344,6 +407,7 @@
     hipLaunchKernelGGL(pmv_partial_kernel, dim3(B, (C * p * p + 255) / 256), dim3(256), 0, (hipStream_t)stream, imgs, ids_keep, drows, partial, C, H,
                        W, p, keep, pixel_mask);
     SKY_LAUNCH_CHECK("skyemb_patch_gather_bwd_pmv");
+    if (!dpmv) return 0;
     return skyemb_colsum(partial, SKYEMB_F32, (int64_t)C * p * p, B, C * p * p, dpmv, stream);
 }
 
@@ -383,6 +447,57 @@
                        outer_stride, n_rows, D, partial);
     SKY_LAUNCH_CHECK("skyemb_rowsum_select");
     return skyemb_colsum(partial, SKYEMB_F32, D, nblk, D, out, stream);
+}
+
+extern "C" int skyemb_rowsum_gather(const float *src, const float *sel, int row0, int inner, int outer_stride, int n_rows, int D,
+                                    float *partial, float *out_sum, const int32_t *idx, float *out, void *out_lp, int dtype,
+                                    int n_gather, void *stream) {
+    SKY_CHECK_ARG(src && partial && idx && (out || out_lp) && n_rows > 0 && n_gather > 0 && D > 0 && D % 4 == 0 && inner > 0,
+                  "skyemb_rowsum_gather: bad arguments (n_rows=%d n_gather=%d D=%d)", n_rows, n_gather, D);
+    const int nblk = 256;
+    hipStream_t st = (hipStream_t)stream;
+    const dim3 grid((unsigned)(nblk + n_gather)), block(256);
+    if (dtype == SKYEMB_BF16)
+        hipLaunchKernelGGL(rowsum_gather_kernel<bf16_t>, grid, block, 0, st, src, (int64_t)D, sel, row0, inner, outer_stride, n_rows, D,
+                           partial, nblk, idx, out, (bf16_t *)out_lp);
+    else if (dtype == SKYEMB_F16)
+        hipLaunchKernelGGL(rowsum_gather_kernel<f16_t>, grid, block, 0, st, src, (int64_t)D, sel, row0, inner, outer_stride, n_rows, D,
+                           partial, nblk, idx, out, (f16_t *)out_lp);
+    else
+        hipLaunchKernelGGL(rowsum_gather_kernel<float>, grid, block, 0, st, src, (int64_t)D, sel, row0, inner, outer_stride, n_rows, D,
+                           partial, nblk, idx, out, (float *)out_lp);
+    SKY_LAUNCH_CHECK("skyemb_rowsum_gather");
+    return out_sum ? skyemb_colsum(partial, SKYEMB_F32, D, nblk, D, out_sum, stream) : 0;
+}
+
+extern "C" int skyemb_patch_gather_seams(const float *imgs, const float *pmv, const int32_t *ids_keep, void *out, int dtype, int B,
+                                         int C, int H, int W, int p, int keep, float pixel_mean, float pixel_std, const float *cls,
+                                         const float *pos0, float *x0, int64_t x0_stride, int D, float *xd, const float *mask,
+                                         const float *mask_token, const float *dec_pos, int L, int Dd, int n_extra, void *stream) {
+    SKY_CHECK_ARG(B > 0 && C > 0 && p > 0 && p % 4 == 0 && H % p == 0 && W % p == 0 && keep > 0,
+                  "skyemb_patch_gather_seams: bad geometry C=%d H=%d W=%d p=%d keep=%d", C, H, W, p, keep);
+    SKY_CHECK_ARG(ids_keep || keep == (H / p) * (W / p), "skyemb_patch_gather_seams: ids_keep == NULL needs keep == L");
+    SKY_CHECK_ARG(!x0 || (cls && pos0 && D > 0 && D % 4 == 0 && x0_stride >= D && x0_stride % 4 == 0 && aligned16(cls) && aligned16(pos0) &&
+                          aligned16(x0)), "skyemb_patch_gather_seams: bad cls rows (D=%d)", D);
+    SKY_CHECK_ARG(!xd || (mask && mask_token && dec_pos && L > 0 && Dd > 0 && Dd % 4 == 0 && n_extra >= 1 && aligned16(mask_token) &&
+                          aligned16(dec_pos) && aligned16(xd)), "skyemb_patch_gather_seams: bad mask-token rows (L=%d Dd=%d)", L, Dd);
+    FwdSeams s;
+    s.cls = cls; s.pos0 = pos0; s.x0 = x0; s.x0_stride = x0_stride; s.D = D; s.n_cls = x0 ? B : 0;
+    s.xd = xd; s.mask = mask; s.mask_token = mask_token; s.dec_pos = dec_pos; s.L = L; s.Dd = Dd; s.E = n_extra; s.n_fill = xd ? B * L : 0;
+    hipStream_t st = (hipStream_t)stream;
+    const int n_gather = B * keep;
+    const dim3 grid((unsigned)(n_gather + s.n_cls + s.n_fill)), block(256);
+    if (dtype == SKYEMB_BF16)
+        hipLaunchKernelGGL(patch_gather_seams_kernel<bf16_t>, grid, block, 0, st, imgs, pmv, ids_keep, (bf16_t *)out, C, H, W, p, keep,
+                           pixel_mean, pixel_std, n_gather, s);
+    else if (dtype == SKYEMB_F16)
+        hipLaunchKernelGGL(patch_gather_seams_kernel<f16_t>, grid, block, 0, st, imgs, pmv, ids_keep, (f16_t *)out, C, H, W, p, keep,
+                           pixel_mean, pixel_std, n_gather, s);
+    else
+        hipLaunchKernelGGL(patch_gather_seams_kernel<float>, grid, block, 0, st, imgs, pmv, ids_keep, (float *)out, C, H, W, p, keep,
+                           pixel_mean, pixel_std, n_gather, s);
+    SKY_LAUNCH_CHECK("skyemb_patch_gather_seams");
+    return 0;
 }
 
 extern "C" int skyemb_cast(const float *src, void *dst, int dtype, int64_t n, void *stream) {
diff --git a/sky_embeddings_amd/csrc/layernorm.hip b/sky_embeddings_amd/csrc/layernorm.hip
--- a/sky_embeddings_amd/csrc/layernorm.hip
+++ b/sky_embeddings_amd/csrc/layernorm.hip
@@ -91,6 +91,20 @@
     const int2 blk = blocks[blockIdx.x];
     const skyemb_ln_reduce_item it = items[blk.x];
     const int bx = blk.y & 0xffff, by = blk.y >> 16;
+    if (by == 2) {
+        const int lane = threadIdx.x & 63, wave = threadIdx.x >> 6;
+        const int n = bx * 64 + lane;
+        float acc = 0.f;
+        if (wave < 4 && n < it.D) {
+#pragma unroll 8
+            for (int m = wave; m < it.nblk; m += 4) acc += it.part[(int64_t)m * it.D + n];
+        }
+        float *r4 = &red[0][0];
+        if (wave < 4) r4[wave * 64 + lane] = acc;
+        __syncthreads();
+        if (wave == 0 && n < it.D) it.dgamma[n] = (r4[lane] + r4[64 + lane]) + (r4[128 + lane] + r4[192 + lane]);
+        return;
+    }
     const int col = threadIdx.x & 31, rg = threadIdx.x >> 5;
     const int d = bx * 32 + col;
     const float *src = it.part + (int64_t)by * it.nblk * it.D;
diff --git a/sky_embeddings_amd/engine.py b/sky_embeddings_amd/engine.py
--- a/sky_embeddings_amd/engine.py
+++ b/sky_embeddings_amd/engine.py
@@ -147,6 +147,7 @@
         self._side, self._pending, self._group_done = None, {}, None
         self._splitk_ws_side = None
         self._ln_first = self._ln_count = 0
+        self._defer_reduces = False
         self._pf_maps = None
         self._graph_captures = 0
         self._variant_args = {"adamw": None, "g16": None}
@@ -277,8 +278,20 @@
             w["drows"] = torch.empty(B * keep, pv, **f32)
             w["pmv_part"] = torch.empty(B, pv, **f32)
             w["rs_part"] = torch.empty(256, max(D, Dd), **f32)
+            self._plan_seam_folds(w, B, D, Dd, pv)
         self._ws[key] = w
         return w
+
+    def _plan_seam_folds(self, w, B, D, Dd, pv):
+        w["fold_seams"] = bool(ops.fold_seams() and self._modes == "mae" and not self.cfg.simmim and self._side is None)
+        if not w["fold_seams"]:
+            return
+        f32, st = dict(device=self.device, dtype=torch.float32), self.store
+        w["rs_part_mask"], w["rs_part_cls"] = torch.empty(256, Dd, **f32), torch.empty(256, D, **f32)
+        tail = [(w["rs_part_mask"], st.grad("mask_token").view(Dd), None, 256, Dd, "colsum"),
+                (w["rs_part_cls"], st.grad("cls_token").view(D), None, 256, D, "colsum"),
+                (w["pmv_part"], st.grad("patch_mask_values").view(pv), None, B, pv, "colsum")]
+        w["tail_items"] = ops.ln_reduce_items(w["ln_entries"] + tail, self.device)
 
     def _block_bufs(self, M, dim):
         f32, lp = dict(device=self.device, dtype=torch.float32), dict(device=self.device, dtype=self.dtype)
@@ -329,6 +342,7 @@
             _, prefix, bufs, M_, dim = item
             ln(f"{prefix}.norm2", M_, dim)
             ln(f"{prefix}.norm1", M_, dim)
+        w["ln_entries"] = entries
         w["ln_items"] = ops.ln_reduce_items(entries, self.device)
 
     def _weight_chain(self):
@@ -364,26 +378,35 @@
         nxt = self._pf_maps[direction].get(wname)
         return None if nxt is None else self.store.lp(nxt)
 
-    def _embed(self, imgs, noise, keep, w, ra_dec=None):
+    def _embed(self, imgs, noise, keep, w, ra_dec=None, dec_fill=False):
         cfg, st = self.cfg, self.store
         B = imgs.shape[0]
         L, D, pv, E = cfg.num_patches, cfg.embed_dim, cfg.patch_dim, cfg.num_extra_tokens
         Ne = E + keep
         ops.random_mask_from_noise(noise, keep, w["ids_restore"], w["mask"], w["ids_keep"], w["dec_dst"], w["dec_tab"], n_extra=E)
-        ops.patch_gather(imgs, st.param("patch_mask_values"), w["ids_keep"], w["patches"], cfg.patch_size, keep,
-                         cfg.pixel_mean, cfg.pixel_std)
         x0 = w["xs"][0]
         pos = st.frozen["pos_embed"].view(-1, D)
+        fold = bool(w.get("fold_seams"))
+        if fold:
+            dec = dict(xd=w["xd"][0], mask=w["mask"], mask_token=st.param("mask_token"), dec_pos=st.frozen["decoder_pos_embed"],
+                       L=L, Dd=cfg.decoder_embed_dim) if dec_fill else {}
+            ops.patch_gather_seams(imgs, st.param("patch_mask_values"), w["ids_keep"], w["patches"], cfg.patch_size, keep,
+                                   cfg.pixel_mean, cfg.pixel_std, cls=st.param("cls_token"), pos0=pos[0], x0=x0, x0_stride=Ne * D, D=D,
+                                   n_extra=E, **dec)
+        else:
+            ops.patch_gather(imgs, st.param("patch_mask_values"), w["ids_keep"], w["patches"], cfg.patch_size, keep,
+                             cfg.pixel_mean, cfg.pixel_std)
         ops.gemm(w["patches"], st.lp("patch_embed.proj.weight"), M=B * keep, N=D, K=pv,
                  bias=st.param("patch_embed.proj.bias"), table=pos[E:], tab_row=w["ids_keep"], ldt=D,
                  dst_row=w["pe_dst"], out_f32=x0, ldo32=D, prefetch=self._pf("fwd", "patch_embed.proj.weight", B * keep))
-        self._extra_tokens_fwd(x0, pos, B, Ne, ra_dec, w)
+        self._extra_tokens_fwd(x0, pos, B, Ne, ra_dec, w, cls_done=fold)
         return x0
 
-    def _extra_tokens_fwd(self, x0, pos, B, Ne, ra_dec, w):
+    def _extra_tokens_fwd(self, x0, pos, B, Ne, ra_dec, w, cls_done=False):
         cfg, st = self.cfg, self.store
         D = cfg.embed_dim
-        x0.view(B, Ne, D)[:, 0, :] = st.param("cls_token").view(D) + pos[0]
+        if not cls_done:
+            x0.view(B, Ne, D)[:, 0, :] = st.param("cls_token").view(D) + pos[0]
         if cfg.ra_dec:
             P = st.param
             ops.radec_token_fwd(ra_dec, P("ra_dec_embed.neural_network.layers.0.weight"),
@@ -421,12 +444,12 @@
                 self._block_fwd(xs[i % 2], xs[(i + 1) % 2], w["enc"][0], f"blocks.{i}", M, D, cfg.num_heads, B, Ne)
         return xs[cfg.depth] if train else xs[cfg.depth % 2]
 
-    def _encoder_fwd(self, imgs, noise, keep, w, train, ra_dec=None):
+    def _encoder_fwd(self, imgs, noise, keep, w, train, ra_dec=None, dec_fill=False):
         cfg, st = self.cfg, self.store
         B = imgs.shape[0]
         D, Ne = cfg.embed_dim, cfg.num_extra_tokens + keep
         Me = B * Ne
-        self._embed(imgs, noise, keep, w, ra_dec)
+        self._embed(imgs, noise, keep, w, ra_dec, dec_fill)
         x_last = self._blocks_fwd(w, B, Ne, train)
         ops.layernorm_fwd(x_last, st.param("norm.weight"), st.param("norm.bias"), w["lat_lp"], w["lat_mean"],
                           w["lat_rstd"], Me, D, cfg.ln_eps, y32=w["latent32"])
@@ -481,13 +504,14 @@
         Me, Md = B * Ne, B * Nd
         w = self._workspace(B, keep, True)
         self.plan_loss_scale(B * (L - keep) * pv)
-        self._encoder_fwd(imgs, noise, keep, w, True, ra_dec)
+        self._encoder_fwd(imgs, noise, keep, w, True, ra_dec, dec_fill=True)
         xd = w["xd"]
         dpos = st.frozen["decoder_pos_embed"].view(-1, Dd)
         ops.gemm(w["lat_lp"], st.lp("decoder_embed.weight"), M=Me, N=Dd, K=D, bias=st.param("decoder_embed.bias"),
                  table=dpos, tab_row=w["dec_tab"], ldt=Dd, dst_row=w["dec_dst"], out_f32=xd[0], ldo32=Dd,
                  prefetch=self._pf("fwd", "decoder_embed.weight", Me))
-        ops.fill_mask_tokens(xd[0], w["mask"], st.param("mask_token"), dpos, B, L, Dd, n_extra=E)
+        if not w.get("fold_seams"):
+            ops.fill_mask_tokens(xd[0], w["mask"], st.param("mask_token"), dpos, B, L, Dd, n_extra=E)
         for i in range(cfg.decoder_depth):
             self._block_fwd(xd[i], xd[i + 1], w["dec"][i], f"decoder_blocks.{i}", Md, Dd, cfg.decoder_num_heads, B, Nd)
         ops.layernorm_fwd(xd[-1], st.param("decoder_norm.weight"), st.param("decoder_norm.bias"), w["dlat_lp"],
@@ -554,6 +578,13 @@
             torch.cuda.current_stream().wait_stream(self._side)
             self._pending.clear()
             self._group_done = None
+        if self._defer_reduces:
+            if last:
+                n_ln = len(w["ln_entries"])
+                assert self._ln_first == 0 and self._ln_count == n_ln, "backward() did not visit every LayerNorm of the reduce table"
+                ops.layernorm_bwd_reduce_batch(w["tail_items"], 0, n_ln + 3)
+                self._ln_first = self._ln_count = 0
+            return
         if self._ln_count:
             ops.layernorm_bwd_reduce_batch(w["ln_items"], self._ln_first, self._ln_count)
         self._ln_first, self._ln_count = (0, 0) if last else (self._ln_first + self._ln_count, 0)
@@ -793,8 +824,12 @@
         for i in reversed(range(cfg.decoder_depth)):
             self._block_bwd(w["xd"][i], w["dec"][i], f"decoder_blocks.{i}", Md, Dd, cfg.decoder_num_heads, B, Nd, g,
                             g_lp, w)
-        ops.rowsum_select(g, Dd, w["mask"], cfg.num_extra_tokens, L, Nd, B * L, Dd, w["rs_part"], st.grad("mask_token").view(Dd))
-        ops.gather_rows(g, w["dec_dst"], None, w["dE"], Me, Dd)
+        if w.get("fold_seams"):
+            ops.rowsum_gather(g, w["mask"], cfg.num_extra_tokens, L, Nd, B * L, Dd, w["rs_part_mask"],
+                              None if self._defer_reduces else st.grad("mask_token").view(Dd), w["dec_dst"], None, w["dE"], Me)
+        else:
+            ops.rowsum_select(g, Dd, w["mask"], cfg.num_extra_tokens, L, Nd, B * L, Dd, w["rs_part"], st.grad("mask_token").view(Dd))
+            ops.gather_rows(g, w["dec_dst"], None, w["dE"], Me, Dd)
         dln_e = w["dln"][:Me * D].view(Me, D)
         self._linear_bwd(w["dE"], w["lat_lp"], "decoder_embed.weight", "decoder_embed.bias", Me, Dd, D, w, dx_out=dln_e,
                          wgrad="decoder_embed" not in w.get("folded_wgrads", ()))
@@ -818,31 +853,41 @@
     def backward_embed(self):
         imgs, B, keep, Ne, Nd, w = self._bwd_ctx()
         self._embed_bwd(B, Ne, keep, w)
-        ops.patch_gather_bwd_pmv(imgs, w["ids_keep"], w["drows"], w["pmv_part"], self.store.grad("patch_mask_values"),
-                                 self.cfg.patch_size, keep)
+        ops.patch_gather_bwd_pmv(imgs, w["ids_keep"], w["drows"], w["pmv_part"],
+                                 None if self._defer_reduces else self.store.grad("patch_mask_values"), self.cfg.patch_size, keep)
         self._end_stage(w, last=True)
 
     def _embed_bwd(self, B, Ne, n_patch, w):
         cfg, st = self.cfg, self.store
         D, pv = cfg.embed_dim, cfg.patch_dim
         g = w["g"][:B * Ne * D].view(B * Ne, D)
-        ops.rowsum_select(g, D, None, 0, 1, Ne, B, D, w["rs_part"], st.grad("cls_token").view(D))
+        fold = bool(w.get("fold_seams"))
+        if not fold:
+            ops.rowsum_select(g, D, None, 0, 1, Ne, B, D, w["rs_part"], st.grad("cls_token").view(D))
         if cfg.ra_dec:
             G = st.grad
             ops.radec_token_bwd(g.view(-1)[D:], Ne * D, st.param("ra_dec_embed.neural_network.last_layer.weight"), w["sh"],
                                 w["z"], w["dz"], G("ra_dec_embed.neural_network.layers.0.weight"),
                                 G("ra_dec_embed.neural_network.layers.0.bias"), G("ra_dec_embed.neural_network.last_layer.weight"),
                                 G("ra_dec_embed.neural_network.last_layer.bias"), B, D)
-        ops.gather_rows(g, w["pe_dst"], None, w["dT"], B * n_patch, D)
+        if fold:
+            ops.rowsum_gather(g, None, 0, 1, Ne, B, D, w["rs_part_cls"], None if self._defer_reduces else st.grad("cls_token").view(D),
+                              w["pe_dst"], None, w["dT"], B * n_patch)
+        else:
+            ops.gather_rows(g, w["pe_dst"], None, w["dT"], B * n_patch, D)
         self._wgrad(w["dT"], w["patches"], D, pv, B * n_patch, st.grad("patch_embed.proj.weight"),
                     st.grad("patch_embed.proj.bias"), w)
         ops.gemm(w["dT"], st.lp("patch_embed.proj.weight"), M=B * n_patch, N=pv, K=D, a_layout=KC, b_layout=RC, lda=D,
                  ldb=pv, out_f32=w["drows"])
 
     def backward(self):
-        self.backward_decoder()
-        self.backward_encoder()
-        self.backward_embed()
+        self._defer_reduces = bool(self.last_workspace().get("fold_seams"))
+        try:
+            self.backward_decoder()
+            self.backward_encoder()
+            self.backward_embed()
+        finally:
+            self._defer_reduces = False
 
     def backward_stages(self, n_encoder_groups=3):
         groups, ranges = self._stage_ranges(n_encoder_groups)
diff --git a/sky_embeddings_amd/ops.py b/sky_embeddings_amd/ops.py
--- a/sky_embeddings_amd/ops.py
+++ b/sky_embeddings_amd/ops.py
@@ -37,6 +37,10 @@
 def _prefetch_on():
     import os
     return os.environ.get("SKYEMB_PREFETCH", "1") != "0"
+
+
+def fold_seams():
+    return os.environ.get("SKYEMB_FOLD_SEAMS", "1") != "0"
 
 
 def gemm_args(A, B, *, M, N, K, a_layout=KC, b_layout=KC, lda=None, ldb=None, alpha=1.0, bias=None, table=None,
@@ -177,6 +181,14 @@
                                     keep, pixel_mean, pixel_std, _stream()), "skyemb_patch_gather")
 
 
+def patch_gather_seams(imgs, pmv, ids_keep, out, p, keep, pixel_mean, pixel_std, cls=None, pos0=None, x0=None, x0_stride=0, D=0,
+                       xd=None, mask=None, mask_token=None, dec_pos=None, L=0, Dd=0, n_extra=1):
+    B, C, H, W = imgs.shape
+    check(lib().skyemb_patch_gather_seams(_p(imgs), _p(pmv), _p(ids_keep), _p(out), dtype_code(out.dtype), B, C, H, W, p, keep,
+                                          pixel_mean, pixel_std, _p(cls), _p(pos0), _p(x0), x0_stride, D, _p(xd), _p(mask),
+                                          _p(mask_token), _p(dec_pos), L, Dd, n_extra, _stream()), "skyemb_patch_gather_seams")
+
+
 def patch_gather_bwd_pmv(imgs, ids_keep, drows, partial, dpmv, p, keep):
     B, C, H, W = imgs.shape
     check(lib().skyemb_patch_gather_bwd_pmv(_p(imgs), _p(ids_keep), _p(drows), _p(partial), _p(dpmv), B, C, H, W, p,
@@ -230,11 +242,15 @@
 
 
 def ln_reduce_items(entries, device):
-    rows = [[part.data_ptr(), dg.data_ptr(), db.data_ptr() if db is not None else 0, nblk + (D << 32)] for part, dg, db, nblk, D in entries]
+    rows = [[e[0].data_ptr(), e[1].data_ptr(), e[2].data_ptr() if e[2] is not None else 0, e[3] + (e[4] << 32)] for e in entries]
     blocks, first = [], [0]
-    for k, (part, dg, db, nblk, D) in enumerate(entries):
-        for y in range(2 if db is not None else 1):
-            blocks += [[k, x | (y << 16)] for x in range((D + 31) // 32)]
+    for k, e in enumerate(entries):
+        db, D = e[2], e[4]
+        if len(e) > 5 and e[5] == "colsum":
+            blocks += [[k, x | (2 << 16)] for x in range((D + 63) // 64)]
+        else:
+            for y in range(2 if db is not None else 1):
+                blocks += [[k, x | (y << 16)] for x in range((D + 31) // 32)]
         first.append(len(blocks))
     return (torch.tensor(rows, dtype=torch.int64).to(device), torch.tensor(blocks, dtype=torch.int32).to(device), first)
 
@@ -271,6 +287,12 @@
                                      _stream()), "skyemb_rowsum_select")
 
 
+def rowsum_gather(src, sel, row0, inner, outer_stride, n_rows, D, partial, out_sum, idx, out, out_lp, n_gather):
+    code = dtype_code(out_lp.dtype) if out_lp is not None else F32
+    check(lib().skyemb_rowsum_gather(_p(src), _p(sel), row0, inner, outer_stride, n_rows, D, _p(partial), _p(out_sum), _p(idx), _p(out),
+                                     _p(out_lp), code, n_gather, _stream()), "skyemb_rowsum_gather")
+
+
 def masked_patch_loss(imgs, pred, mask, loss, dpred, dpred32, dtype, ws, p, extra, pixel_mean, pixel_std, norm_pix,
                       loss_l1, dscale=1.0):
     B, C, H, W = imgs.shape
@@ -284,6 +306,15 @@
     code = dtype_code(p_lp.dtype) if p_lp is not None else F32
     check(lib().skyemb_adamw(_p(p), _p(g), _p(m), _p(v), _p(p_lp), code, n, n_decay, _p(hyper), lr, bc1, bc2, beta1,
                              beta2, eps, wd, grad_scale, int(zero_grad), dtype_code(g.dtype), _stream()), "skyemb_adamw")
+
+
+def adamw_ranges(p, g, m, v, p_lp, ranges, n_decay, hyper, beta1, beta2, eps, wd, grad_scale=1.0):
+    n = len(ranges)
+    lo = (ctypes.c_int64 * n)(*[int(r[0]) for r in ranges])
+    hi = (ctypes.c_int64 * n)(*[int(r[1]) for r in ranges])
+    code = dtype_code(p_lp.dtype) if p_lp is not None else F32
+    check(lib().skyemb_adamw_ranges(_p(p), _p(g), _p(m), _p(v), _p(p_lp), code, ctypes.cast(lo, ctypes.c_void_p), ctypes.cast(hi, ctypes.c_void_p),
+                                    n, n_decay, _p(hyper), beta1, beta2, eps, wd, grad_scale, _stream()), "skyemb_adamw_ranges")
 
 
 def set_scalars(dst, a, b=0.0, c=0.0, d=0.0):
diff --git a/sky_embeddings_amd/optim.py b/sky_embeddings_amd/optim.py
--- a/sky_embeddings_amd/optim.py
+++ b/sky_embeddings_amd/optim.py
@@ -76,6 +76,19 @@
         ops.adamw(st.p[sl], g[sl_g], st.m[sl], st.v[sl], st.p_lp[sl], n, n_decay, self.hyper_device, b1, b2,
                   self.defaults["eps"], self.param_groups[1]["weight_decay"], grad_scale=self.grad_scale, zero_grad=False,
                   lr=self.lr, bc1=1.0 - b1 ** t, bc2=1.0 - b2 ** t)
+
+    MAX_RANGES = 8
+
+    def apply_ranges(self, ranges):
+        ranges = [(s, e) for s, e in ranges if e > s]
+        if self.hyper_device is None or self.grad_buffer is not None or not 1 < len(ranges) <= self.MAX_RANGES:
+            for s, e in ranges:
+                self.apply_range(s, e)
+            return
+        b1, b2 = self.defaults["betas"]
+        st = self.store
+        ops.adamw_ranges(st.p, st.g, st.m, st.v, st.p_lp, ranges, st.n_decay, self.hyper_device, b1, b2, self.defaults["eps"],
+                         self.param_groups[1]["weight_decay"], grad_scale=self.grad_scale)
 
     def step_scalars(self, t=None):
         b1, b2 = self.defaults["betas"]
diff --git a/sky_embeddings_amd/train_step.py b/sky_embeddings_amd/train_step.py
--- a/sky_embeddings_amd/train_step.py
+++ b/sky_embeddings_amd/train_step.py
@@ -119,12 +119,17 @@
 
             self._fused_consts = self._optimizer_consts()
 
+            fold_rest = ops.fold_seams()
+
             def owning(fn):
                 def run():
                     with engine.wgrad_variant("adamw"):
                         fn()
-                    for (s_, e_) in self._rest():
-                        optimizer.apply_range(s_, e_)
+                    if fold_rest:
+                        optimizer.apply_ranges(self._rest())
+                    else:
+                        for (s_, e_) in self._rest():
+                            optimizer.apply_range(s_, e_)
                 return run
             self.stages = [(owning(fn), ranges) for fn, ranges in self.stages]
         self.graphs = None
```
